# AlejandroSilvestri/os1

Hardware: AMD Instinct MI355X
Metric: frames/sec extract+match, 1920x1080 @ 2000 ORB feats (higher is better)
Workload: dtype u8

## Files before the change

include/orbfe.h:

```cpp
#ifndef ORBFE_H_
#define ORBFE_H_

#include <stddef.h>
#include <stdint.h>

#ifdef __cplusplus
extern "C" {
#endif

#define ORBFE_OK 0
#define ORBFE_ERR_INVALID (-1)
#define ORBFE_ERR_NO_DEVICE (-2)
#define ORBFE_ERR_HIP (-3)
#define ORBFE_ERR_TOO_SMALL (-4)
#define ORBFE_ERR_OVERFLOW (-5)

typedef struct OrbfeKeyPoint {
  float x, y;
  float size;
  float angle;
  float response;
  int32_t octave;
  int32_t class_id;
} OrbfeKeyPoint;

typedef struct orbfe_extractor orbfe_extractor;
typedef struct orbfe_matcher orbfe_matcher;
typedef struct orbfe_vocabulary orbfe_vocabulary;

const char* orbfe_last_error(void);
int orbfe_device_count(void);

int orbfe_device_malloc(int device_id, size_t bytes, void** out);
int orbfe_device_free(int device_id, void* ptr);
int orbfe_device_upload(int device_id, void* dst_device, const void* src_host, size_t bytes);
int orbfe_device_synchronize(int device_id);
int orbfe_host_alloc(size_t bytes, void** out);
int orbfe_host_free(void* ptr);
int orbfe_host_register(void* ptr, size_t bytes);
int orbfe_host_unregister(void* ptr);
int orbfe_device_numa_node(int device_id);
int orbfe_bind_thread_to_device(int device_id);
int orbfe_debug_h2d_rate(int device_id, const void* host, size_t bytes, int reps, double* gb_per_s);


int orbfe_extractor_create(int nfeatures, float scaleFactor, int nlevels, int iniThFAST, int minThFAST,
                           int device_id, orbfe_extractor** out);
void orbfe_extractor_destroy(orbfe_extractor* h);

int orbfe_extractor_levels(const orbfe_extractor* h);
int orbfe_extractor_device(const orbfe_extractor* h);
float orbfe_extractor_scale_factor(const orbfe_extractor* h);
int orbfe_extractor_scale_tables(const orbfe_extractor* h, float* scale, float* inv_scale, float* sigma2,
                                 float* inv_sigma2);
int orbfe_extractor_features_per_level(const orbfe_extractor* h, int32_t* out);
int orbfe_extractor_max_keypoints(const orbfe_extractor* h);
int orbfe_extractor_max_keypoints_for_size(const orbfe_extractor* h, int rows, int cols);

int orbfe_extractor_set_wait_mode(orbfe_extractor* h, int poll_us);

enum { ORBFE_INPUT_GRAY8 = 0, ORBFE_INPUT_RGB8 = 1, ORBFE_INPUT_BGR8 = 2, ORBFE_INPUT_RGBA8 = 3, ORBFE_INPUT_BGRA8 = 4 };
enum { ORBFE_GRAY_Q15 = 0, ORBFE_GRAY_Q14 = 1 };
int orbfe_extractor_set_input_format(orbfe_extractor* h, int format, int gray_variant);

enum { ORBFE_GAUSS_ED = 0, ORBFE_GAUSS_ROUNDED = 1 };
int orbfe_extractor_set_blur_variant(orbfe_extractor* h, int variant);

int orbfe_extract(orbfe_extractor* h, const uint8_t* gray, int rows, int cols, size_t stride_bytes,
                  OrbfeKeyPoint* kps, uint8_t* desc, int cap, int* n_out);

int orbfe_extract_batch(orbfe_extractor* h, int nframes, const uint8_t* const* gray, int in_device_memory,
                        int rows, int cols, size_t stride_bytes, OrbfeKeyPoint* kps, uint8_t* desc, int cap,
                        int* n_out);

int orbfe_extract_batch_submit(orbfe_extractor* h, int nframes, const uint8_t* const* gray, int in_device_memory,
                               int rows, int cols, size_t stride_bytes);
int orbfe_extract_batch_collect(orbfe_extractor* h, OrbfeKeyPoint* kps, uint8_t* desc, int cap, int* n_out);
int orbfe_extract_batch_wait(orbfe_extractor* h);

typedef struct orbfe_sfi_chain orbfe_sfi_chain;
int orbfe_sfi_chain_create(const orbfe_extractor* h, orbfe_sfi_chain** out);
void orbfe_sfi_chain_destroy(orbfe_sfi_chain* c);
int orbfe_sfi_chain_set_isolated(orbfe_sfi_chain* c, int isolated);
int orbfe_sfi_chain_restart(orbfe_sfi_chain* c);
int orbfe_extract_batch_submit_matched(orbfe_extractor* h, orbfe_sfi_chain* chain, int nframes, const uint8_t* const* gray,
                                       int in_device_memory, int rows, int cols, size_t stride_bytes, const float bounds[4],
                                       int window_size, float nnratio, int check_orientation);
int orbfe_extract_batch_collect_matched(orbfe_extractor* h, OrbfeKeyPoint* kps, uint8_t* desc, int cap, int* n_out,
                                        int32_t* matches12, int* nmatches);

int orbfe_debug_level_size(const orbfe_extractor* h, int level, int* w, int* hgt);
int orbfe_debug_level_copy(orbfe_extractor* h, int frame, int level, uint8_t* out );
int orbfe_debug_candidates(orbfe_extractor* h, int frame, int level, int32_t* xys, int cap, int* n_out);
int orbfe_debug_stage_ms(const orbfe_extractor* h, float out[5]);
int orbfe_debug_kernel_ms(orbfe_extractor* h, double out_ms[5], long long* batches, long long* frames, int reset);
int orbfe_debug_set_profiling(orbfe_extractor* h, int enable);
int orbfe_debug_fast_stamps(orbfe_extractor* h, unsigned long long out[8], int reset);
int orbfe_debug_sfi_records(orbfe_extractor* h, int32_t* out, int cap_records, int* n_out, int reset);
int orbfe_debug_sincos(orbfe_extractor* h, const float* angle_deg, int n, float* cos_out, float* sin_out);

int orbfe_debug_quadtree(const int16_t* x, const int16_t* y, const uint8_t* score, int n, int min_x, int max_x,
                         int min_y, int max_y, int n_target, int32_t* out_idx, int cap, int* n_out);
int orbfe_debug_sincos_host_check(uint32_t lo_bits, uint32_t hi_bits, uint32_t step, long long* mismatches);
int orbfe_debug_logf(orbfe_matcher* m, const float* x, int n, float* out);
int orbfe_debug_logf_host_check(uint32_t lo_bits, uint32_t hi_bits, uint32_t step, long long* mismatches);

typedef struct orbfe_stream orbfe_stream;
int orbfe_stream_create(int nfeatures, float scaleFactor, int nlevels, int iniThFAST, int minThFAST, int device_id,
                        int batch, int depth, orbfe_stream** out);
void orbfe_stream_destroy(orbfe_stream* s);
int orbfe_stream_set_matching(orbfe_stream* s, const float bounds[4], int window_size, float nnratio,
                              int check_orientation);
int orbfe_stream_set_isolated_batches(orbfe_stream* s, int isolated);
int orbfe_stream_batches_in_flight(const orbfe_stream* s);
int orbfe_stream_pop_hold(orbfe_stream* s, const OrbfeKeyPoint** kps, const uint8_t** desc, const int** n_kps, const int32_t** matches12,
                          const int** nmatches, int* ticket);
int orbfe_stream_release(orbfe_stream* s, int ticket);
int orbfe_stream_set_input_format(orbfe_stream* s, int format, int gray_variant);
int orbfe_stream_set_blur_variant(orbfe_stream* s, int variant);
int orbfe_stream_set_vocabulary(orbfe_stream* s, orbfe_vocabulary* v, int levelsup);
int orbfe_stream_bow_raw(orbfe_stream* s, int frame, const uint32_t** leaf_node, const uint32_t** level_node, int* n);
int orbfe_stream_capacity(const orbfe_stream* s);
int orbfe_stream_set_queue_slots(orbfe_stream* s, int nslots);
int orbfe_stream_queue_slots(const orbfe_stream* s);
int orbfe_stream_push(orbfe_stream* s, const uint8_t* const* gray, int in_device_memory, int rows, int cols,
                      size_t stride_bytes);
int orbfe_stream_pop(orbfe_stream* s, const OrbfeKeyPoint** kps, const uint8_t** desc, const int** n_kps,
                     const int32_t** matches12, const int** nmatches);
int orbfe_stream_stats(orbfe_stream* s, double out[4], int reset);
int orbfe_stream_kernel_ms(orbfe_stream* s, double out_ms[5], long long* batches, long long* frames, int reset);


int orbfe_hamming(const uint8_t a[32], const uint8_t b[32]);

int orbfe_matcher_create(int device_id, orbfe_matcher** out);
void orbfe_matcher_destroy(orbfe_matcher* m);
int orbfe_matcher_device(const orbfe_matcher* m);
int orbfe_matcher_upload_async(orbfe_matcher* m, void* dst_device, const void* src_host, size_t bytes);
int orbfe_matcher_synchronize(orbfe_matcher* m);

int orbfe_search_for_initialization(orbfe_matcher* m, const OrbfeKeyPoint* kps1, const uint8_t* desc1, int n1,
                                    const OrbfeKeyPoint* kps2, const uint8_t* desc2, int n2,
                                    const float bounds[4], float* prev_xy, int32_t* matches12, int window_size,
                                    float nnratio, int check_orientation, int* nmatches);

int orbfe_search_for_initialization_batch(orbfe_matcher* m, int npairs, const OrbfeKeyPoint* const* kps1,
                                          const uint8_t* const* desc1, const int* n1,
                                          const OrbfeKeyPoint* const* kps2, const uint8_t* const* desc2,
                                          const int* n2, const float bounds[4], float* const* prev_xy,
                                          int32_t* const* matches12, int window_size, float nnratio,
                                          int check_orientation, int* nmatches);

#define ORBFE_MP_IN_VIEW 1u
#define ORBFE_MP_BAD 2u
#define ORBFE_MP_CANDIDATO 4u
#define ORBFE_MP_OBSERVED 8u

int orbfe_search_by_projection(orbfe_matcher* m, const OrbfeKeyPoint* kps_un, const uint8_t* desc, int n,
                               const float bounds[4], const float* scale_factors, int nlevels,
                               const uint8_t* kp_occupied, const float* mp_proj_xy, const int32_t* mp_level,
                               const float* mp_viewcos, const uint8_t* mp_flags, const uint8_t* mp_desc, int n_mp,
                               float th, float nnratio, int32_t* kp_assigned, int* nmatches);

int orbfe_search_by_projection_uv(orbfe_matcher* m, const OrbfeKeyPoint* kps_un, const uint8_t* desc, int n,
                                  const float bounds[4], const float* scale_factors, int nlevels,
                                  const uint8_t* kp_occupied, const float* src_uv, const int32_t* src_level,
                                  const float* src_angle, const uint8_t* src_flags, const uint8_t* src_valid,
                                  const uint8_t* src_desc, int n_src, float th, int max_dist,
                                  int skip_any_occupied, int check_orientation, int32_t* kp_assigned,
                                  int* nmatches);

int orbfe_debug_matcher_ms(const orbfe_matcher* m, double out[3]);

int orbfe_window_candidates(orbfe_matcher* m, const OrbfeKeyPoint* kps_un, const uint8_t* desc, int n,
                            const float bounds[4], int nq, const float* qx, const float* qy, const float* qr,
                            const int32_t* qmin_level, const int32_t* qmax_level, const uint8_t* qdesc,
                            uint32_t* counts, uint32_t* offsets, uint32_t* pool, size_t pool_cap, size_t* pool_used);

int orbfe_search_projected(orbfe_matcher* m, const OrbfeKeyPoint* kps_un, const uint8_t* desc, int n, const float bounds[4],
                           int n_src, const float* src_uv, const float* src_radius, const int32_t* src_level,
                           const uint8_t* src_valid, const uint8_t* src_desc, const uint8_t* kp_skip, int claim,
                           const float* inv_level_sigma2, int nlevels, double chi2, int max_dist, int32_t* best_idx,
                           int32_t* best_dist, int* nmatches);

typedef struct orbfe_frame orbfe_frame;
int orbfe_frame_create(orbfe_matcher* m, const OrbfeKeyPoint* kps_un, const uint8_t* desc, int n, const float bounds[4],
                       orbfe_frame** out);
int orbfe_frame_create_from_extract(orbfe_extractor* h, int frame_index, const float bounds[4], const float* xy_un,
                                    orbfe_frame** out);
void orbfe_frame_destroy(orbfe_frame* f);
int orbfe_frame_size(const orbfe_frame* f);
int orbfe_frame_device(const orbfe_frame* f);
unsigned long long orbfe_resident_epoch(void);
unsigned long long orbfe_resident_invalidate(void);
const uint8_t* orbfe_frame_descriptors_device(orbfe_frame* f);
int orbfe_frame_download(orbfe_frame* f, OrbfeKeyPoint* kps_un, uint8_t* desc, int32_t* grid_order, int32_t* cell_start);

int orbfe_search_by_projection_frame(orbfe_matcher* m, orbfe_frame* f, const float* scale_factors, int nlevels,
                                     const uint8_t* kp_occupied, const float* mp_proj_xy, const int32_t* mp_level,
                                     const float* mp_viewcos, const uint8_t* mp_flags, const uint8_t* mp_desc, int n_mp,
                                     float th, float nnratio, int32_t* kp_assigned, int* nmatches);
int orbfe_search_by_projection_frame_rows(orbfe_matcher* m, orbfe_frame* f, const float* scale_factors, int nlevels,
                                          const uint8_t* kp_occupied, const float* mp_proj_xy, const int32_t* mp_level,
                                          const float* mp_viewcos, const uint8_t* mp_flags, const uint8_t* desc_table_device,
                                          const uint8_t* desc_table_host, const int32_t* mp_desc_row, int n_rows, int n_mp,
                                          float th, float nnratio, int32_t* kp_assigned, int* nmatches);
int orbfe_search_by_projection_uv_frame(orbfe_matcher* m, orbfe_frame* f, const float* scale_factors, int nlevels,
                                        const uint8_t* kp_occupied, const float* src_uv, const int32_t* src_level,
                                        const float* src_angle, const uint8_t* src_flags, const uint8_t* src_valid,
                                        const uint8_t* src_desc, int n_src, float th, int max_dist, int skip_any_occupied,
                                        int check_orientation, int32_t* kp_assigned, int* nmatches);
int orbfe_search_projected_frame(orbfe_matcher* m, orbfe_frame* f, int n_src, const float* src_uv, const float* src_radius,
                                 const int32_t* src_level, const uint8_t* src_valid, const uint8_t* src_desc,
                                 const uint8_t* kp_skip, int claim, const float* inv_level_sigma2, int nlevels, double chi2,
                                 int max_dist, int32_t* best_idx, int32_t* best_dist, int* nmatches);
typedef struct orbfe_local_map orbfe_local_map;
#define ORBFE_MP_SKIP 16u
typedef struct OrbfeCamera {
  float Rcw[9];
  float tcw[3];
  float Ow[3];
  float fx, fy, cx, cy;
  float logScaleFactor;
} OrbfeCamera;
int orbfe_local_map_create(orbfe_matcher* m, int capacity, orbfe_local_map** out);
void orbfe_local_map_destroy(orbfe_local_map* map);
int orbfe_local_map_capacity(const orbfe_local_map* map);
int orbfe_local_map_set_rows(orbfe_local_map* map, int n, const int32_t* rows, const float* pos, const float* normal,
                             const float* min_raw, const float* max_raw, const uint8_t* desc);
int orbfe_project_local_map(orbfe_matcher* m, orbfe_frame* f, orbfe_local_map* map, const OrbfeCamera* cam,
                            float view_cos_limit, const int32_t* rows, const uint8_t* flags, int n_mp, uint8_t* in_view,
                            float* proj_xy, int32_t* level, float* view_cos, int* n_in_view);
int orbfe_search_local_points_frame(orbfe_matcher* m, orbfe_frame* f, orbfe_local_map* map, const OrbfeCamera* cam,
                                    float view_cos_limit, const int32_t* rows, const uint8_t* flags, int n_mp,
                                    const float* scale_factors, int nlevels, const uint8_t* kp_occupied, float th, float nnratio,
                                    uint8_t* in_view, float* proj_xy, int32_t* level, float* view_cos, int32_t* kp_assigned,
                                    int* nmatches, int* n_in_view);
#define ORBFE_SRC_LAST_FRAME 0
#define ORBFE_SRC_KEYFRAME 1
int orbfe_project_sources(orbfe_matcher* m, orbfe_frame* cur_frame, orbfe_frame* src_frame, orbfe_local_map* map,
                          const OrbfeCamera* cam, int mode, const int32_t* rows, const uint8_t* flags, int n_src, uint8_t* valid,
                          float* uv, int32_t* level, int* n_valid);
int orbfe_search_by_projection_sources_frame(orbfe_matcher* m, orbfe_frame* cur_frame, orbfe_frame* src_frame,
// ... 82 lines not shown
```

os1_amd/api.py:

```python
import ctypes as C
import os
import subprocess

import numpy as np

_HERE = os.path.dirname(os.path.abspath(__file__))
_SO = os.environ.get('ORBFE_LIB') or os.path.join(_HERE, 'liborbfe.so')

KP_DTYPE = np.dtype([('x', 'f4'), ('y', 'f4'), ('size', 'f4'), ('angle', 'f4'), ('response', 'f4'),
                     ('octave', 'i4'), ('class_id', 'i4')])

MP_IN_VIEW, MP_BAD, MP_CANDIDATO, MP_OBSERVED = 1, 2, 4, 8


class OrbfeError(RuntimeError):
    def __init__(self, code, msg):
        super().__init__('orbfe error %d: %s' % (code, msg))
        self.code = code


def lib_path():
    return _SO


def build_library(force=False):
    args = ['make', '-s', '-C', os.path.join(_HERE, 'csrc')]
    if force:
        subprocess.check_call(args + ['clean'])
    subprocess.check_call(args)
    return _SO


_lib = None


def load_library():
    global _lib
    if _lib is not None:
        return _lib
    if not os.path.exists(_SO):
        raise OrbfeError(-2, 'liborbfe.so is not built (run __graft_entry__.build() or make -C os1_amd/csrc)')
    L = C.CDLL(_SO)
    vp, ci, cf = C.c_void_p, C.c_int, C.c_float
    L.orbfe_last_error.restype = C.c_char_p
    L.orbfe_device_count.restype = ci
    L.orbfe_extractor_create.argtypes = [ci, cf, ci, ci, ci, ci, C.POINTER(vp)]
    L.orbfe_extractor_destroy.argtypes = [vp]
    L.orbfe_extractor_destroy.restype = None
    L.orbfe_extractor_levels.argtypes = [vp]
    L.orbfe_extractor_scale_factor.argtypes = [vp]
    L.orbfe_extractor_scale_factor.restype = cf
    L.orbfe_extractor_scale_tables.argtypes = [vp, vp, vp, vp, vp]
    L.orbfe_extractor_features_per_level.argtypes = [vp, vp]
    L.orbfe_extractor_max_keypoints.argtypes = [vp]
    L.orbfe_extract.argtypes = [vp, vp, ci, ci, C.c_size_t, vp, vp, ci, C.POINTER(ci)]
    L.orbfe_extract_batch.argtypes = [vp, ci, vp, ci, ci, ci, C.c_size_t, vp, vp, ci, vp]
    L.orbfe_extract_batch_submit.argtypes = [vp, ci, vp, ci, ci, ci, C.c_size_t]
    L.orbfe_extract_batch_wait.argtypes = [vp]
    L.orbfe_extract_batch_collect.argtypes = [vp, vp, vp, ci, vp]
    L.orbfe_debug_level_size.argtypes = [vp, ci, C.POINTER(ci), C.POINTER(ci)]
    L.orbfe_debug_level_copy.argtypes = [vp, ci, ci, vp]
    L.orbfe_debug_candidates.argtypes = [vp, ci, ci, vp, ci, C.POINTER(ci)]
    L.orbfe_debug_stage_ms.argtypes = [vp, vp]
    L.orbfe_debug_sincos.argtypes = [vp, vp, ci, vp, vp]
    L.orbfe_hamming.argtypes = [vp, vp]
    L.orbfe_matcher_create.argtypes = [ci, C.POINTER(vp)]
    L.orbfe_matcher_destroy.argtypes = [vp]
    L.orbfe_matcher_destroy.restype = None
    L.orbfe_search_for_initialization.argtypes = [vp, vp, vp, ci, vp, vp, ci, vp, vp, vp, ci, cf, ci, C.POINTER(ci)]
    L.orbfe_search_for_initialization_batch.argtypes = [vp, ci, vp, vp, vp, vp, vp, vp, vp, vp, vp, ci, cf, ci, vp]
    L.orbfe_frame_create.argtypes = [vp, vp, vp, ci, vp, C.POINTER(vp)]
    L.orbfe_frame_create_from_extract.argtypes = [vp, ci, vp, vp, C.POINTER(vp)]
    L.orbfe_frame_destroy.argtypes = [vp]
    L.orbfe_frame_destroy.restype = None
    L.orbfe_frame_size.argtypes = [vp]
    L.orbfe_frame_descriptors_device.argtypes = [vp]
    L.orbfe_frame_descriptors_device.restype = vp
    L.orbfe_frame_download.argtypes = [vp, vp, vp, vp, vp]
    L.orbfe_search_by_projection_frame.argtypes = [vp, vp, vp, ci, vp, vp, vp, vp, vp, vp, ci, cf, cf, vp, C.POINTER(ci)]
    L.orbfe_search_by_projection_frame_rows.argtypes = [vp, vp, vp, ci, vp, vp, vp, vp, vp, vp, vp, vp, ci, ci, cf, cf, vp,
                                                        C.POINTER(ci)]
    L.orbfe_matcher_upload_async.argtypes = [vp, vp, vp, C.c_size_t]
    L.orbfe_matcher_synchronize.argtypes = [vp]
    L.orbfe_matcher_device.argtypes = [vp]
    L.orbfe_extractor_device.argtypes = [vp]
    L.orbfe_frame_device.argtypes = [vp]
    L.orbfe_resident_epoch.restype = C.c_ulonglong
    L.orbfe_resident_invalidate.restype = C.c_ulonglong
    L.orbfe_search_by_projection_uv_frame.argtypes = [vp, vp, vp, ci, vp, vp, vp, vp, vp, vp, vp, ci, cf, ci, ci, ci, vp,
                                                      C.POINTER(ci)]
    L.orbfe_search_projected_frame.argtypes = [vp, vp, ci, vp, vp, vp, vp, vp, vp, ci, vp, ci, C.c_double, ci, vp, vp,
                                               C.POINTER(ci)]
    L.orbfe_debug_resolve_rounds.argtypes = [vp]
    L.orbfe_debug_resolve_route.argtypes = [vp]
    L.orbfe_debug_resolve_phases.argtypes = [vp, vp]
    L.orbfe_search_by_projection.argtypes = [vp, vp, vp, ci, vp, vp, ci, vp, vp, vp, vp, vp, vp, ci, cf, cf, vp,
                                             C.POINTER(ci)]
    L.orbfe_search_by_projection_uv.argtypes = [vp, vp, vp, ci, vp, vp, ci, vp, vp, vp, vp, vp, vp, vp, ci, cf, ci,
                                                ci, ci, vp, C.POINTER(ci)]
    L.orbfe_distinctive_descriptors.argtypes = [vp, ci, vp, vp, vp]
    L.orbfe_window_candidates.argtypes = [vp, vp, vp, ci, vp, ci, vp, vp, vp, vp, vp, vp, vp, vp, vp, C.c_size_t,
                                          C.POINTER(C.c_size_t)]
    L.orbfe_undistort_equidistant.argtypes = [vp, ci, cf, cf, cf, cf]
    L.orbfe_undistort_pinhole.argtypes = [vp, ci, cf, cf, cf, cf, vp, ci]
    L.orbfe_compute_image_bounds.argtypes = [ci, ci, ci, cf, cf, cf, cf, vp, ci, vp]
    L.orbfe_search_projected.argtypes = [vp, vp, vp, ci, vp, ci, vp, vp, vp, vp, vp, vp, ci, vp, ci, C.c_double, ci, vp, vp,
                                         C.POINTER(ci)]
    L.orbfe_search_for_triangulation.argtypes = [vp, vp, vp, vp, ci, vp, vp, vp, ci, vp, vp, vp, ci, vp, vp, vp, ci, vp, cf, cf,
                                                 vp, vp, ci, ci, vp, C.POINTER(ci)]
    L.orbfe_extractor_max_keypoints_for_size.argtypes = [vp, ci, ci]
    L.orbfe_extractor_set_vocabulary.argtypes = [vp, vp, ci]
    L.orbfe_extract_bow_raw.argtypes = [vp, ci, vp, vp, ci, C.POINTER(ci)]
    L.orbfe_bow_assemble.argtypes = [vp, vp, vp, ci, vp, vp, C.POINTER(ci), vp, vp, vp, C.POINTER(ci), vp]
    L.orbfe_stream_set_vocabulary.argtypes = [vp, vp, ci]
    L.orbfe_stream_bow_raw.argtypes = [vp, ci, C.POINTER(vp), C.POINTER(vp), C.POINTER(ci)]
    L.orbfe_extract_bow.argtypes = [vp, ci, vp, vp, C.POINTER(ci), vp, vp, vp, C.POINTER(ci), vp, vp]
    L.orbfe_extractor_set_input_format.argtypes = [vp, ci, ci]
    L.orbfe_stream_set_input_format.argtypes = [vp, ci, ci]
    L.orbfe_extractor_set_blur_variant.argtypes = [vp, ci]
    L.orbfe_stream_set_blur_variant.argtypes = [vp, ci]
    L.orbfe_vocabulary_create.argtypes = [ci, ci, ci, ci, ci, vp, ci, C.POINTER(vp)]
    L.orbfe_vocabulary_create_from_image.argtypes = [ci, vp, C.c_size_t, C.POINTER(vp)]
    L.orbfe_vocabulary_destroy.argtypes = [vp]
    L.orbfe_vocabulary_destroy.restype = None
    L.orbfe_vocabulary_info.argtypes = [vp] + [C.POINTER(ci)] * 6
    L.orbfe_bow_transform.argtypes = [vp, vp, ci, ci, ci, vp, vp, C.POINTER(ci), vp, vp, vp, C.POINTER(ci), vp, vp]
    L.orbfe_search_by_bow.argtypes = [vp, vp, vp, vp, ci, vp, vp, vp, ci, vp, vp, vp, ci, vp, vp, vp, ci, cf, ci, ci, vp,
                                      C.POINTER(ci)]
    L.orbfe_search_by_bow_batch.argtypes = [vp, ci, vp, vp, vp, vp, vp, vp, vp, vp, vp, vp, vp, ci, vp, vp, vp, ci, cf, ci, ci, vp, vp]
    L.orbfe_debug_matcher_ms.argtypes = [vp, vp]
    L.orbfe_debug_features_in_area.argtypes = [vp, vp, ci, vp, cf, cf, cf, ci, ci, vp, ci, C.POINTER(ci)]
    L.orbfe_debug_kernel_ms.argtypes = [vp, vp, C.POINTER(C.c_longlong), C.POINTER(C.c_longlong), ci]
    L.orbfe_debug_set_profiling.argtypes = [vp, ci]
    L.orbfe_device_malloc.argtypes = [ci, C.c_size_t, C.POINTER(vp)]
    L.orbfe_device_free.argtypes = [ci, vp]
    L.orbfe_device_upload.argtypes = [ci, vp, vp, C.c_size_t]
    L.orbfe_host_alloc.argtypes = [C.c_size_t, C.POINTER(vp)]
    L.orbfe_host_free.argtypes = [vp]
    L.orbfe_host_register.argtypes = [vp, C.c_size_t]
    L.orbfe_host_unregister.argtypes = [vp]
    L.orbfe_device_synchronize.argtypes = [ci]
    L.orbfe_device_numa_node.argtypes = [ci]
    L.orbfe_bind_thread_to_device.argtypes = [ci]
    L.orbfe_debug_h2d_rate.argtypes = [ci, vp, C.c_size_t, ci, C.POINTER(C.c_double)]
    L.orbfe_stream_create.argtypes = [ci, cf, ci, ci, ci, ci, ci, ci, C.POINTER(vp)]
    L.orbfe_stream_destroy.argtypes = [vp]
    L.orbfe_stream_destroy.restype = None
    L.orbfe_stream_set_matching.argtypes = [vp, vp, ci, cf, ci]
    L.orbfe_stream_capacity.argtypes = [vp]
    L.orbfe_stream_set_queue_slots.argtypes = [vp, ci]
    L.orbfe_stream_queue_slots.argtypes = [vp]
    L.orbfe_stream_push.argtypes = [vp, vp, ci, ci, ci, C.c_size_t]
    L.orbfe_stream_pop.argtypes = [vp, C.POINTER(vp), C.POINTER(vp), C.POINTER(vp), C.POINTER(vp), C.POINTER(vp)]
    L.orbfe_stream_pop_hold.argtypes = [vp, C.POINTER(vp), C.POINTER(vp), C.POINTER(vp), C.POINTER(vp), C.POINTER(vp), C.POINTER(ci)]
    L.orbfe_stream_release.argtypes = [vp, ci]
    L.orbfe_stream_set_isolated_batches.argtypes = [vp, ci]
    L.orbfe_stream_batches_in_flight.argtypes = [vp]
    L.orbfe_stream_multi_create.argtypes = [ci, cf, ci, ci, ci, C.POINTER(ci), ci, ci, ci, C.POINTER(vp)]
    L.orbfe_stream_multi_destroy.argtypes = [vp]
    L.orbfe_stream_multi_destroy.restype = None
    L.orbfe_stream_multi_devices.argtypes = [vp]
    L.orbfe_stream_multi_capacity.argtypes = [vp]
    L.orbfe_stream_multi_device_of_next_push.argtypes = [vp]
    L.orbfe_stream_multi_set_matching.argtypes = [vp, vp, ci, cf, ci]
    L.orbfe_stream_multi_set_blur_variant.argtypes = [vp, ci]
    L.orbfe_stream_multi_push.argtypes = [vp, vp, ci, ci, ci, C.c_size_t]
    L.orbfe_stream_multi_pop.argtypes = [vp, C.POINTER(vp), C.POINTER(vp), C.POINTER(vp), C.POINTER(vp), C.POINTER(vp)]
    L.orbfe_stream_stats.argtypes = [vp, vp, ci]
    L.orbfe_stream_kernel_ms.argtypes = [vp, vp, C.POINTER(C.c_longlong), C.POINTER(C.c_longlong), ci]
    L.orbfe_debug_quadtree.argtypes = [vp, vp, vp, ci, ci, ci, ci, ci, ci, vp, ci, C.POINTER(ci)]
    L.orbfe_debug_sincos_host_check.argtypes = [C.c_uint32, C.c_uint32, C.c_uint32, C.POINTER(C.c_longlong)]
    L.orbfe_debug_logf.argtypes = [vp, vp, ci, vp]
    L.orbfe_debug_logf_host_check.argtypes = [C.c_uint32, C.c_uint32, C.c_uint32, C.POINTER(C.c_longlong)]
    L.orbfe_local_map_create.argtypes = [vp, ci, C.POINTER(vp)]
    L.orbfe_local_map_destroy.argtypes = [vp]
    L.orbfe_local_map_destroy.restype = None
    L.orbfe_local_map_capacity.argtypes = [vp]
    L.orbfe_local_map_set_rows.argtypes = [vp, ci, vp, vp, vp, vp, vp, vp]
    L.orbfe_project_local_map.argtypes = [vp, vp, vp, vp, cf, vp, vp, ci, vp, vp, vp, vp, C.POINTER(ci)]
    L.orbfe_search_local_points_frame.argtypes = [vp, vp, vp, vp, cf, vp, vp, ci, vp, ci, vp, cf, cf, vp, vp, vp, vp, vp,
                                                  C.POINTER(ci), C.POINTER(ci)]
    L.orbfe_project_sources.argtypes = [vp, vp, vp, vp, vp, ci, vp, vp, ci, vp, vp, vp, C.POINTER(ci)]
    L.orbfe_search_by_projection_sources_frame.argtypes = [vp, vp, vp, vp, vp, ci, vp, vp, ci, vp, ci, vp, cf, ci, ci, vp, vp, vp,
                                                           vp, C.POINTER(ci), C.POINTER(ci)]
    _lib = L
    return L


def _p(a):
    return a.ctypes.data_as(C.c_void_p)


class DeviceRows:

    def __init__(self, ptr, n):
        self.ptr, self.n = int(ptr), int(n)

    def __len__(self):
        return self.n


def _rows(a):
    if isinstance(a, DeviceRows):
        return C.c_void_p(a.ptr), a
    a = np.ascontiguousarray(a, np.uint8)
    return _p(a), a


def _check(rc):
    if rc != 0:
        raise OrbfeError(rc, load_library().orbfe_last_error().decode('utf-8', 'replace'))


def device_count():
    return load_library().orbfe_device_count()


def hamming(a, b):
    a = np.ascontiguousarray(a, np.uint8)
    b = np.ascontiguousarray(b, np.uint8)
    return load_library().orbfe_hamming(_p(a), _p(b))


class Extractor:

    def __init__(self, nfeatures=1000, scale=1.2, nlevels=8, ini_th=20, min_th=7, device=0):
        self.L = load_library()
        h = C.c_void_p()
        _check(self.L.orbfe_extractor_create(nfeatures, scale, nlevels, ini_th, min_th, device, C.byref(h)))
        self.h = h
        self.nlevels = nlevels
        self.cap = self.L.orbfe_extractor_max_keypoints(h)

    def close(self):
        if getattr(self, 'h', None):
            self.L.orbfe_extractor_destroy(self.h)
            self.h = None

    def __del__(self):
        try:
            self.close()
        except Exception:
            pass

    def tables(self):
        n = self.nlevels
        sf, isf, s2, is2 = (np.zeros(n, np.float32) for _ in range(4))
        nf = np.zeros(n, np.int32)
        _check(self.L.orbfe_extractor_scale_tables(self.h, _p(sf), _p(isf), _p(s2), _p(is2)))
        _check(self.L.orbfe_extractor_features_per_level(self.h, _p(nf)))
        return dict(sf=sf, isf=isf, s2=s2, is2=is2, nfeat=nf)

    def __call__(self, image):
        image = np.asarray(image)
        if image.size == 0:
            n = C.c_int(0)
            _check(self.L.orbfe_extract(self.h, None, 0, 0, 0, None, None, 0, C.byref(n)))
            return np.zeros(0, KP_DTYPE), np.zeros((0, 32), np.uint8)
        assert image.dtype == np.uint8 and image.ndim == 2 and image.strides[1] == 1
        cap = max(self.cap, self.L.orbfe_extractor_max_keypoints_for_size(self.h, image.shape[0], image.shape[1]))
        kps = np.zeros(cap, KP_DTYPE)
        desc = np.zeros((cap, 32), np.uint8)
        n = C.c_int(0)
        _check(self.L.orbfe_extract(self.h, _p(image), image.shape[0], image.shape[1], image.strides[0], _p(kps),
                                    _p(desc), cap, C.byref(n)))
        return kps[:n.value].copy(), desc[:n.value].copy()

    FORMATS = {'gray': 0, 'rgb': 1, 'bgr': 2, 'rgba': 3, 'bgra': 4}

    def set_blur_variant(self, variant):
        _check(self.L.orbfe_extractor_set_blur_variant(self.h, int(variant)))

    def set_input_format(self, fmt='gray', variant=0):
        _check(self.L.orbfe_extractor_set_input_format(self.h, self.FORMATS[fmt], variant))

    def extract_color(self, image):
        image = np.ascontiguousarray(image, np.uint8)
        kps = np.zeros(self.cap, KP_DTYPE)
        desc = np.zeros((self.cap, 32), np.uint8)
        n = C.c_int(0)
        _check(self.L.orbfe_extract(self.h, _p(image), image.shape[0], image.shape[1], image.strides[0], _p(kps),
                                    _p(desc), self.cap, C.byref(n)))
        return kps[:n.value].copy(), desc[:n.value].copy()

    def set_vocabulary(self, voc, levelsup=4):
        self._voc = voc
        _check(self.L.orbfe_extractor_set_vocabulary(self.h, voc.h if voc is not None else None, levelsup))

    def bow(self, frame, n):
        ids = np.zeros(max(n, 1), np.uint32)
        vals = np.zeros(max(n, 1), np.float64)
        fvn = np.zeros(max(n, 1), np.uint32)
        fvo = np.zeros(n + 1, np.uint32)
        fvf = np.zeros(max(n, 1), np.uint32)
        wof = np.zeros(max(n, 1), np.uint32)
        nof = np.zeros(max(n, 1), np.uint32)
        nw, nn = C.c_int(0), C.c_int(0)
        _check(self.L.orbfe_extract_bow(self.h, frame, _p(ids), _p(vals), C.byref(nw), _p(fvn), _p(fvo), _p(fvf), C.byref(nn),
                                        _p(wof), _p(nof)))
        nw, nn = nw.value, nn.value
        return ids[:nw], vals[:nw], (fvn[:nn], fvo[:nn + 1], fvf[:int(fvo[nn])]), wof[:n], nof[:n]

    def extract_batch_ptrs(self, ptrs, rows, cols, stride, on_device, kps=None, desc=None):
        B = len(ptrs)
        arr = (C.c_void_p * B)(*ptrs)
        if kps is None:
            kps = np.zeros((B, self.cap), KP_DTYPE)
        if desc is None:
            desc = np.zeros((B, self.cap, 32), np.uint8)
        n = np.zeros(B, np.int32)
        _check(self.L.orbfe_extract_batch(self.h, B, arr, int(on_device), rows, cols, stride, _p(kps), _p(desc),
                                          int(kps.shape[1]), _p(n)))
        return kps, desc, n

    def submit_ptrs(self, ptrs, rows, cols, stride, on_device):
        B = len(ptrs)
        self._pending = (C.c_void_p * B)(*ptrs)
        self._pendingB = B
        _check(self.L.orbfe_extract_batch_submit(self.h, B, self._pending, int(on_device), rows, cols, stride))

    def wait(self):
        _check(self.L.orbfe_extract_batch_wait(self.h))

    def collect(self, kps=None, desc=None):
        B = self._pendingB
        if kps is None:
            kps = np.zeros((B, self.cap), KP_DTYPE)
        if desc is None:
            desc = np.zeros((B, self.cap, 32), np.uint8)
        n = np.zeros(B, np.int32)
        _check(self.L.orbfe_extract_batch_collect(self.h, _p(kps), _p(desc), self.cap, _p(n)))
        return kps, desc, n

    def extract_batch(self, images):
        images = [np.ascontiguousarray(im, np.uint8) for im in images]
        rows, cols = images[0].shape
        assert all(im.shape == (rows, cols) for im in images)
        kps, desc, n = self.extract_batch_ptrs([im.ctypes.data for im in images], rows, cols, cols, False)
        return [(kps[i, :n[i]].copy(), desc[i, :n[i]].copy()) for i in range(len(images))]

    def level(self, level, frame=0):
        w, h = C.c_int(), C.c_int()
        _check(self.L.orbfe_debug_level_size(self.h, level, C.byref(w), C.byref(h)))
        out = np.zeros((h.value, w.value), np.uint8)
        _check(self.L.orbfe_debug_level_copy(self.h, frame, level, _p(out)))
        return out

    def candidates(self, level, frame=0):
        n = C.c_int(0)
        _check(self.L.orbfe_debug_candidates(self.h, frame, level, None, 0, C.byref(n)))
        out = np.zeros((max(n.value, 1), 3), np.int32)
        _check(self.L.orbfe_debug_candidates(self.h, frame, level, _p(out), n.value, C.byref(n)))
        return out[:n.value].copy()

    def stage_ms(self):
        out = np.zeros(5, np.float32)
        _check(self.L.orbfe_debug_stage_ms(self.h, _p(out)))
        return out

    def kernel_ms(self, reset=False):
        ms = np.zeros(5, np.float64)
        b, f = C.c_longlong(0), C.c_longlong(0)
        _check(self.L.orbfe_debug_kernel_ms(self.h, _p(ms), C.byref(b), C.byref(f), int(reset)))
        return ms, b.value, f.value

    def set_profiling(self, enable=True):
        _check(self.L.orbfe_debug_set_profiling(self.h, int(enable)))

    def sincos(self, angle_deg):
        a = np.ascontiguousarray(angle_deg, np.float32)
        c = np.zeros_like(a)
        s = np.zeros_like(a)
        _check(self.L.orbfe_debug_sincos(self.h, _p(a), a.size, _p(c), _p(s)))
        return c, s


class Camera(C.Structure):
    _fields_ = [('Rcw', C.c_float * 9), ('tcw', C.c_float * 3), ('Ow', C.c_float * 3), ('fx', C.c_float), ('fy', C.c_float),
                ('cx', C.c_float), ('cy', C.c_float), ('logScaleFactor', C.c_float)]

    @classmethod
    def make(cls, Rcw, tcw, Ow, fx, fy, cx, cy, log_scale_factor):
        c = cls()
        c.Rcw[:] = [float(v) for v in np.asarray(Rcw, np.float32).ravel()]
        c.tcw[:] = [float(v) for v in np.asarray(tcw, np.float32).ravel()]
        c.Ow[:] = [float(v) for v in np.asarray(Ow, np.float32).ravel()]
        c.fx, c.fy, c.cx, c.cy = float(np.float32(fx)), float(np.float32(fy)), float(np.float32(cx)), float(np.float32(cy))
        c.logScaleFactor = float(np.float32(log_scale_factor))
        return c


MP_IN_VIEW, MP_BAD, MP_CANDIDATO, MP_OBSERVED, MP_SKIP = 1, 2, 4, 8, 16
SRC_LAST_FRAME, SRC_KEYFRAME = 0, 1


class LocalMap:

    def __init__(self, matcher, capacity):
        self.L = load_library()
        self.matcher = matcher
        h = C.c_void_p()
        _check(self.L.orbfe_local_map_create(matcher.h, capacity, C.byref(h)))
        self.h = h
        self.capacity = capacity

    def set_rows(self, rows, pos=None, normal=None, min_raw=None, max_raw=None, desc=None):
        rows = np.ascontiguousarray(rows, np.int32)
        keep = []

        def arg(a, dt, shape):
            if a is None:
                return None
            a = np.ascontiguousarray(a, dt).reshape(shape)
            keep.append(a)
            return _p(a)
        n = len(rows)
        _check(self.L.orbfe_local_map_set_rows(self.h, n, _p(rows), arg(pos, np.float32, (n, 3)), arg(normal, np.float32, (n, 3)),
                                               arg(min_raw, np.float32, (n,)), arg(max_raw, np.float32, (n,)),
                                               arg(desc, np.uint8, (n, 32))))

    def close(self):
        if getattr(self, 'h', None):
            self.L.orbfe_local_map_destroy(self.h)
            self.h = None

    def __del__(self):
        try:
            self.close()
        except Exception:
            pass


class Frame:

    def __init__(self, handle, n):
        self.L = load_library()
        self.h = handle
        self.n = n

    @classmethod
    def from_host(cls, matcher, kps_un, desc, bounds):
        L = load_library()
        kps_un = np.ascontiguousarray(kps_un, KP_DTYPE)
        desc = np.ascontiguousarray(desc, np.uint8)
        b = np.asarray(bounds, np.float32)
        h = C.c_void_p()
        _check(L.orbfe_frame_create(matcher.h, _p(kps_un), _p(desc), len(kps_un), _p(b), C.byref(h)))
        return cls(h, len(kps_un))

    @classmethod
    def from_extract(cls, extractor, frame_index, bounds, xy_un=None):
        L = load_library()
        b = np.asarray(bounds, np.float32)
        xy = None if xy_un is None else np.ascontiguousarray(xy_un, np.float32)
        h = C.c_void_p()
        _check(L.orbfe_frame_create_from_extract(extractor.h, frame_index, _p(b), None if xy is None else _p(xy), C.byref(h)))
        return cls(h, L.orbfe_frame_size(h))

    def __len__(self):
        return self.n

    def descriptors_device(self):
        return DeviceRows(self.L.orbfe_frame_descriptors_device(self.h) or 0, self.n)

    def download(self):
        k = np.zeros(max(self.n, 1), KP_DTYPE)
        d = np.zeros((max(self.n, 1), 32), np.uint8)
        order = np.zeros(max(self.n, 1), np.int32)
        cs = np.zeros(64 * 48 + 1, np.int32)
        _check(self.L.orbfe_frame_download(self.h, _p(k), _p(d), _p(order), _p(cs)))
        return k[:self.n], d[:self.n], order[:int(cs[-1])], cs

    def close(self):
        if getattr(self, 'h', None):
            self.L.orbfe_frame_destroy(self.h)
            self.h = None

    def __del__(self):
        try:
            self.close()
        except Exception:
            pass


class Matcher:

    def frame(self, kps_un, desc, bounds):
        return Frame.from_host(self, kps_un, desc, bounds)

    def resolve_rounds(self):
        return int(self.L.orbfe_debug_resolve_rounds(self.h))

    def resolve_route(self):
        return int(self.L.orbfe_debug_resolve_route(self.h))

    def resolve_phases(self):
        o = np.zeros(4, np.int32)
        _check(self.L.orbfe_debug_resolve_phases(self.h, _p(o)))
        return np.diff(o.astype(np.int64)) & 0xffffffff
# ... 743 lines not shown
```

os1_amd/csrc/orbfe_extractor.hip:

```cpp
#include <hip/hip_runtime.h>
#include <unistd.h>
#include <sched.h>

#include <algorithm>
#include <cctype>
#include <chrono>
#include <cmath>
#include <cstdarg>
#include <cstdio>
#include <cstdlib>
#include <cstring>
#include <memory>
#include <mutex>
#include <string>
#include <thread>
#include <vector>

#include "../../include/orbfe.h"
#include "glibc_sincosf.h"
#include "host_pool.h"
#include "orbfe_internal.h"
#include "quadtree.h"

namespace orbfe {
int launch_pyramid(const PyramidParams& P, int nframes, hipStream_t st, const ConeParams* cone);
void launch_ingest(const uint8_t* src, long long sstride, uint8_t* dst, long long dpitch, int rowBytes, int rows, hipStream_t st);
void launch_to_gray(const uint8_t* const* raw, long long rawStride, const uint8_t* const* gray, long long grayPitch, int rows,
                    int cols, int channels, const int coef[3], int shift, bool aligned, int nframes, hipStream_t st);
void launch_fast(const PyramidParams& P, int nframes, hipStream_t st);
uint32_t fast_cell_geo(int wCell, int hCell);
void launch_compact(const PyramidParams& P, int nframes, hipStream_t st);
void launch_compact_local(const PyramidParams& P, int nframes, hipStream_t st, int level0, int level1);
void launch_describe(const PyramidParams& P, const SelKp* sel, int nsel, float* angle, uint8_t* desc,
                     hipStream_t st);
void launch_sincos(const float* deg, int n, float* c, float* s, hipStream_t st);
void launch_spin(unsigned long long ticks, hipStream_t st);
void launch_describe_slots(const PyramidParams& P, const SelKp* sel, int nslots, float* angle, uint8_t* desc,
                           const uint32_t* selCount, int selPerFrame, const int* selOff, hipStream_t st, bool fourWaves, float* angle2 = nullptr,
                           uint8_t* desc2 = nullptr);
int launch_quadtree(const QtParams& Q, int nframes, hipStream_t st, int ldsBudget);
int bow_launch_descend(orbfe_vocabulary* v, const uint8_t* d_desc, int n, int levelsup, uint2* d_out, hipStream_t st);
int bow_assemble(orbfe_vocabulary* v, const uint2* ln, int n, uint32_t* bow_ids, double* bow_values, int* n_words,
                 uint32_t* fv_nodes, uint32_t* fv_offsets, uint32_t* fv_features, int* n_fv_nodes,
                 uint32_t* word_of_feature, uint32_t* node_of_feature);
int bow_device(const orbfe_vocabulary* v);
void launch_sfi(const SfiParams& S, int nframes, hipStream_t st);
void launch_sfi_carry(const SfiParams& S, int lastFrame, SelKp* cSel, float* cAngle, uint8_t* cDesc, uint32_t* cCount,
                      hipStream_t st);

thread_local std::string g_err;
void set_err(const char* fmt, ...) {
  char buf[512];
  va_list ap;
  va_start(ap, fmt);
  vsnprintf(buf, sizeof buf, fmt, ap);
  va_end(ap);
  g_err = buf;
}
}

using namespace orbfe;

#define HIP_TRY(expr)                                                                        \
  do {                                                                                       \
    hipError_t e_ = (expr);                                                                  \
    if (e_ != hipSuccess) {                                                                  \
      set_err("%s failed: %s (%s:%d)", #expr, hipGetErrorString(e_), __FILE__, __LINE__);    \
      return ORBFE_ERR_HIP;                                                                  \
    }                                                                                        \
  } while (0)

namespace {
inline int cv_round_f(float v) { return (int)lrintf(v); }
inline int cv_floor_f(float v) { int i = (int)v; return i - (i > v); }
inline short sat_short(int v) { return (short)(v < -32768 ? -32768 : v > 32767 ? 32767 : v); }
inline long long align_up(long long v, long long a) { return (v + a - 1) / a * a; }
double now_ms() {
  return std::chrono::duration<double, std::milli>(std::chrono::steady_clock::now().time_since_epoch()).count();
}

template <class T>
struct DevBuf {
  T* p = nullptr;
  size_t n = 0;
  int ensure(size_t count) {
    if (count <= n) return ORBFE_OK;
    if (p) (void)hipFree(p);
    p = nullptr;
    n = 0;
    HIP_TRY(hipMalloc((void**)&p, count * sizeof(T)));
    n = count;
    return ORBFE_OK;
  }
  void release() { if (p) (void)hipFree(p); p = nullptr; n = 0; }
};
template <class T>
struct PinBuf {
  T* p = nullptr;
  size_t n = 0;
  int ensure(size_t count) {
    if (count <= n) return ORBFE_OK;
    if (p) (void)hipHostFree(p);
    p = nullptr;
    n = 0;
    HIP_TRY(hipHostMalloc((void**)&p, count * sizeof(T), hipHostMallocDefault));
    n = count;
    return ORBFE_OK;
  }
  void release() { if (p) (void)hipHostFree(p); p = nullptr; n = 0; }
};
}

struct orbfe_sfi_chain {
  int device = 0, n0cap = 0;
  DevBuf<SelKp> sel[2];
  DevBuf<float> angle[2];
  DevBuf<uint8_t> desc[2];
  DevBuf<uint32_t> count;
  hipEvent_t ready[2] = {};
  long long seq = 0;
  bool isolated = false;
  bool restart = false;
  orbfe_matcher* hostMatcher = nullptr;
  std::vector<OrbfeKeyPoint> hostPrevKps;
  std::vector<uint8_t> hostPrevDesc;
  bool hostPrevValid = false;
  ~orbfe_sfi_chain() {
    (void)hipSetDevice(device);
    if (hostMatcher) orbfe_matcher_destroy(hostMatcher);
    for (int i = 0; i < 2; i++) { sel[i].release(); angle[i].release(); desc[i].release(); if (ready[i]) (void)hipEventDestroy(ready[i]); }
    count.release();
  }
};

struct UploadLane {
  std::mutex mu;
  hipStream_t stream = nullptr;
};
static UploadLane* upload_lane(int device) {
  static std::mutex mu;
  static UploadLane* lanes[64] = {};
  if (device < 0 || device >= 64) return nullptr;
  std::lock_guard<std::mutex> lk(mu);
  if (!lanes[device]) {
    UploadLane* l = new UploadLane;
    if (hipStreamCreateWithFlags(&l->stream, hipStreamNonBlocking) != hipSuccess) { delete l; return nullptr; }
    lanes[device] = l;
  }
  return lanes[device];
}

struct orbfe_extractor {
  int nfeatures, nlevels, iniTh, minTh, device;
  double scaleFactor;
  std::vector<float> sf, isf, sigma2, isigma2;
  std::vector<int> nfeat;
  static constexpr int kMaxSub = 4;
  hipStream_t stream = nullptr;
  hipStream_t streams[kMaxSub] = {};
  static constexpr int subBatches = 4;
  hipEvent_t evUpload = nullptr;
  bool lastLocalCand = false, submitLocalCand = false;
  bool localLists = true;
  hipEvent_t evFrame0 = nullptr, evS1[kMaxSub] = {};
  int subSel[kMaxSub] = {};
  size_t candHostCap = 0;
  bool gpuQuadtree = true;
  orbfe_vocabulary* voc = nullptr;
  int vocLevelsup = 4;
  bool pendingBow = false;
  DevBuf<uint2> d_bow;
  PinBuf<uint2> h_bow;
  std::vector<std::vector<uint2>> bowKp;
  int kpPerFrameCap = 0;
  bool geomGpuQtOk = true;
  QtParams QP{};
  int selOff[kMaxLevels + 1] = {};
  int selPerFrame = 0;
  DevBuf<uint16_t> d_own;
  hipEvent_t evQt[2] = {};
  std::vector<int> frameKpBase, frameKpCount;

  int rows = 0, cols = 0, batchCap = 0;
  PyramidParams P{};
  DevBuf<uint8_t> d_tables, d_slab, d_in;
  DevBuf<ConeRange> d_coneTab, d_coneTailTab;
  ConeParams coneTail{};
  bool tailOk = false;
  int tailBase = 0, tailTile = 48;
  ConeParams cone{};
  bool coneOk = false;
  bool qtJump = true;
  int qtLdsBudget = 120 * 1024;
  int pollWaitUs = 0;
  bool zeroCopyOut = true;
  bool zeroCopyBatches = false;
  bool ingestKernel = true;
  int coneTile = 0;
  int coneMaxFrames = 2;
  DevBuf<FastCell> d_cells;
  DevBuf<uint8_t> d_zeros;
  DevBuf<uint32_t> d_cellCount, d_slots, d_cand;
  DevBuf<const uint8_t*> d_frame0;
  template <class T> struct View { T* p = nullptr; };
  DevBuf<uint8_t> d_outArena;
  PinBuf<uint8_t> h_outArena;
  size_t outArenaBytes = 0;
  View<uint32_t> d_levelStart, d_selCount, h_levelStart, h_selCount;
  View<SelKp> d_sel, h_sel;
  View<float> d_angle, h_angle;
  View<uint8_t> d_desc, h_desc;
  View<int32_t> d_m12, h_m12, d_nm, h_nm;
  DevBuf<uint16_t> d_sfiOrder;
  DevBuf<int> d_sfiOrderCount;
  DevBuf<uint32_t> d_sfiPool, d_sfiPcount;
  bool pendingMatched = false;
  DevBuf<float> d_f32tmp;
  bool profileKernels = false;
  PinBuf<const uint8_t*> h_frame0;
  PinBuf<uint32_t> h_cand;
  long long inPitch = 0;
  int inFormat = ORBFE_INPUT_GRAY8, grayVariant = ORBFE_GRAY_Q15;
  int gaussVariant = ORBFE_GAUSS_ED;
  long long grayPitch = 0;
  DevBuf<uint8_t> d_gray;
  bool inLinear = false;
  int lastFrames = 0;
  int deferredFrames = 0, deferredCap = 0;
  bool deferredMatched = false;
  std::vector<OrbfeKeyPoint> defKps;
  std::vector<uint8_t> defDesc;
  std::vector<int> defN, defNm;
  std::vector<int32_t> defM12;
  bool lastGpuQt = false, lastZeroCopy = false, submitZeroCopy = false;
  bool describe4 = true;
  float stageMs[5] = {0, 0, 0, 0, 0};
  hipEvent_t ev[kMaxSub][6] = {};
  double kernMs[5] = {0, 0, 0, 0, 0};
  long long kernBatches = 0, kernFrames = 0;

  struct Meta { int16_t x, y; uint8_t score, level; };
  struct Worker {
    QuadTree qt;
    std::vector<int16_t> qx, qy;
    std::vector<uint8_t> qs;
    std::vector<int> qsel;
  };
  std::unique_ptr<HostPool> pool;
  int hostThreads = 1;
  std::vector<Worker> workers;
  std::vector<std::vector<Meta>> taskOut;
  std::vector<Meta> meta;

  ~orbfe_extractor() {
    (void)hipSetDevice(device);
    for (auto& st : streams) if (st) (void)hipStreamSynchronize(st);
    d_bow.release(); h_bow.release();
    d_tables.release(); d_coneTab.release(); d_coneTailTab.release(); d_slab.release(); d_in.release(); d_cellCount.release();
    d_sfiOrder.release(); d_sfiOrderCount.release(); d_sfiPool.release(); d_sfiPcount.release();
    d_cells.release(); d_zeros.release(); d_slots.release(); d_cand.release(); d_frame0.release(); d_gray.release(); d_outArena.release(); h_outArena.release();
    d_f32tmp.release();
    h_frame0.release(); h_cand.release();
    for (auto& es : ev) for (auto& e : es) if (e) (void)hipEventDestroy(e);
    for (auto& e : evS1) if (e) (void)hipEventDestroy(e);
    for (auto& e : evQt) if (e) (void)hipEventDestroy(e);
    d_own.release();
    if (evFrame0) (void)hipEventDestroy(evFrame0);
    if (evUpload) (void)hipEventDestroy(evUpload);

    for (auto& st : streams) if (st) (void)hipStreamDestroy(st);
  }

  int setGeometry(int r, int c) {
    if (r == rows && c == cols) return ORBFE_OK;
    if (c > 4095 || r > 4095) {
      set_err("image %dx%d exceeds the 4095-pixel coordinate packing limit", c, r);
      return ORBFE_ERR_INVALID;
    }
    bool qtOk = true;
    int kpSum = 8;
    PyramidParams Q{};
    Q.nlevels = nlevels;
    Q.iniTh = iniTh;
    Q.minTh = minTh;
    long long off = 0, slot = 0;
    int cellBase = 0;
    size_t tableBytes = 0;
    for (int l = 0; l < nlevels; l++) {
      LevelGeom& L = Q.lv[l];
      L.w = cv_round_f((float)c * isf[l]);
      L.h = cv_round_f((float)r * isf[l]);
      const float width = (float)((L.w - kEdge + 3) - (kEdge - 3));
      const float height = (float)((L.h - kEdge + 3) - (kEdge - 3));
      L.nCols = (int)(width / 30.f);
      L.nRows = (int)(height / 30.f);
      if (L.nCols < 1 || L.nRows < 1) {
        set_err("image %dx%d too small: level %d (%dx%d) has no FAST cell", c, r, l, L.w, L.h);
        return ORBFE_ERR_TOO_SMALL;
      }
      L.wCell = (int)std::ceil(width / L.nCols);
      L.hCell = (int)std::ceil(height / L.nRows);
      {
        const int nIni = (int)roundf(static_cast<float>(L.w - 2 * kBorder) / (L.h - 2 * kBorder));
        if (nIni < 1 || nIni > 4) qtOk = false;
        kpSum += std::max(nfeat[l] + 4, 4 * std::max(nIni, 4));
      }
      L.cellBase = cellBase;
      cellBase += L.nCols * L.nRows;
      L.slotCap = (((L.wCell + 1) / 2) * ((L.hCell + 1) / 2) + 3) & ~3;
      L.slotBase = slot;
      slot += (long long)L.nCols * L.nRows * L.slotCap;
      if (l >= 1) {
        L.pitch = (int)align_up(L.w, 64);
        L.off = off;
        off += align_up((long long)L.pitch * L.h, 256);
        tableBytes += align_up(L.w * 4, 16) + align_up(L.w * 4, 16) + align_up(L.h * 4, 16) + align_up(L.h * 4, 16) + align_up(L.h * 4, 16);
      }
    }
    Q.ncells = cellBase;
    Q.slabBytes = off;
    Q.slotsPerFrame = slot;
    Q.candCap = slot;
    if (slot >= (1ll << 24)) qtOk = false;

    std::vector<uint8_t> tab(tableBytes);
    int rc = d_tables.ensure(tableBytes);
    if (rc) return rc;
    size_t cur = 0;
    const int* xofsH[kMaxLevels] = {};
    const int* yofsH[kMaxLevels] = {};
    for (int l = 1; l < nlevels; l++) {
      LevelGeom& L = Q.lv[l];
      const int sw = Q.lv[l - 1].w, sh = Q.lv[l - 1].h, dw = L.w, dh = L.h;
      const double scale_x = 1. / ((double)dw / sw), scale_y = 1. / ((double)dh / sh);
      int* xofs = (int*)(tab.data() + cur);
      xofsH[l] = xofs;
      L.xofs = (const int*)(d_tables.p + cur);
      cur += align_up(dw * 4, 16);
      short* xa = (short*)(tab.data() + cur);
      L.xalpha = (const short*)(d_tables.p + cur);
      cur += align_up(dw * 4, 16);
      int* yofs = (int*)(tab.data() + cur);
      yofsH[l] = yofs;
      L.yofs = (const int*)(d_tables.p + cur);
      cur += align_up(dh * 4, 16);
      short* yb = (short*)(tab.data() + cur);
      L.ybeta = (const short*)(d_tables.p + cur);
      cur += align_up(dh * 4, 16);
      unsigned* yc = (unsigned*)(tab.data() + cur);
      L.yofc = (const unsigned*)(d_tables.p + cur);
      cur += align_up(dh * 4, 16);
      for (int dx = 0; dx < dw; dx++) {
        float fx = (float)((dx + 0.5) * scale_x - 0.5);
        int sx = cv_floor_f(fx);
        fx -= sx;
        if (sx < 0) { fx = 0; sx = 0; }
        if (sx >= sw - 1) { fx = 0; sx = sw - 1; }
        xofs[dx] = sx;
        xa[2 * dx] = sat_short(cv_round_f((1.f - fx) * 2048));
        xa[2 * dx + 1] = sat_short(cv_round_f(fx * 2048));
      }
      for (int dy = 0; dy < dh; dy++) {
        float fy = (float)((dy + 0.5) * scale_y - 0.5);
        int sy = cv_floor_f(fy);
        fy -= sy;
        yofs[dy] = sy;
        yc[dy] = (unsigned)std::min(std::max(sy, 0), sh - 1) | ((unsigned)std::min(std::max(sy + 1, 0), sh - 1) << 16);
        yb[2 * dy] = sat_short(cv_round_f((1.f - fy) * 2048));
        yb[2 * dy + 1] = sat_short(cv_round_f(fy * 2048));
      }
      for (int dy = dh; dy < (int)align_up(dh, 4); dy++) {
        yc[dy] = yc[dh - 1];
        yb[2 * dy] = yb[2 * (dh - 1)];
        yb[2 * dy + 1] = yb[2 * (dh - 1) + 1];
      }
      int maxW = 1, maxH = 1;
      for (int x0 = 0; x0 < dw; x0 += 64) {
        const int x1 = std::min(x0 + 64, dw) - 1;
        maxW = std::max(maxW, std::min(xofs[x1] + 1, sw - 1) - xofs[x0] + 1);
      }
      for (int y0 = 0; y0 < dh; y0 += 64) {
        const int y1 = std::min(y0 + 64, dh) - 1;
        const int r0 = std::min(std::max(yofs[y0], 0), sh - 1), r1 = std::min(std::max(yofs[y1] + 1, 0), sh - 1);
        maxH = std::max(maxH, r1 - r0 + 1);
      }
      L.rzPitch = (maxW + 3 + 3) & ~3;
      L.rzRows = maxH;
    }
    HIP_TRY(hipMemcpyAsync(d_tables.p, tab.data(), tableBytes, hipMemcpyHostToDevice, stream));
    auto buildCone = [&](int tile, int baseMin, ConeParams& out, DevBuf<ConeRange>& tabBuf, bool& ok) -> int {
      ok = false;
      if (!(nlevels >= 3 && scaleFactor <= 1.5f)) return ORBFE_OK;
      std::vector<ConeRange> coneTab;
      const int top = nlevels - 1;
      if (tile <= 0) {
        tile = 32;
        for (int t = 16; t < 32; t += 2)
          if (((Q.lv[top].w + t - 1) / t) * ((Q.lv[top].h + t - 1) / t) <= 256) { tile = t; break; }
      }
      const int tx = (Q.lv[top].w + tile - 1) / tile, ty = (Q.lv[top].h + tile - 1) / tile;
      coneTab.assign((size_t)(tx + ty) * kMaxLevels, ConeRange{0, 0});
      int maxW[kMaxLevels] = {}, maxH[kMaxLevels] = {};
      for (int b = 0; b < tx + ty; b++) {
        const bool isX = b < tx;
        int lo = (isX ? b : b - tx) * tile, hi = std::min(lo + tile, isX ? Q.lv[top].w : Q.lv[top].h) - 1;
        ConeRange* R = coneTab.data() + (size_t)b * kMaxLevels;
        for (int l = top;; l--) {
          R[l] = ConeRange{lo, hi};
          int& m = isX ? maxW[l] : maxH[l];
          m = std::max(m, hi - lo + 1);
          if (l == 0) break;
          const int dn = isX ? Q.lv[l].w : Q.lv[l].h, sn = isX ? Q.lv[l - 1].w : Q.lv[l - 1].h;
          const int* ofs = isX ? xofsH[l] : yofsH[l];
          const int nlo = lo == 0 ? 0 : std::min(std::max(ofs[lo], 0), sn - 1);
          const int nhi = hi == dn - 1 ? sn - 1 : std::min(std::max(ofs[hi] + 1, 0), sn - 1);
          lo = nlo; hi = nhi;
        }
      }
      for (int base = std::max(0, baseMin); base < top - 1; base++) {
        auto pitchOf = [&](int l) { return (maxW[l] + 3 + 3) & ~3; };
        auto area = [&](int l) { return (size_t)align_up(pitchOf(l) * maxH[l], 16); };
        size_t hBytes = 0;
        int coefLen = 0;
        for (int l = base + 1; l <= top; l++) {
          hBytes = std::max(hBytes, (size_t)align_up(maxH[l - 1] * pitchOf(l) * 2, 16));
          coefLen = std::max(coefLen, std::max(pitchOf(l), maxH[l]));
        }
        const size_t coefBytes = (size_t)kMaxLevels * 2 * coefLen * sizeof(int2);
        const size_t total = area(base) + area(base + 1) + hBytes + coefBytes;
        if (total > 128 * 1024 || coefLen > 512) continue;
        out.base = base; out.top = top; out.tile = tile; out.tilesX = tx; out.tilesY = ty;
        out.offB = (int)area(base); out.offH = out.offB + (int)area(base + 1); out.offC = out.offH + (int)hBytes;
        out.coefLen = coefLen; out.ldsBytes = (int)total;
        ok = true;
        break;
      }
      if (ok) {
        int rc2;
        if ((rc2 = tabBuf.ensure(coneTab.size()))) return rc2;
        HIP_TRY(hipMemcpyAsync(tabBuf.p, coneTab.data(), sizeof(ConeRange) * coneTab.size(), hipMemcpyHostToDevice, stream));
        HIP_TRY(hipStreamSynchronize(stream));
        out.regX = tabBuf.p;
        out.regY = tabBuf.p + (size_t)tx * kMaxLevels;
      }
      return ORBFE_OK;
    };
    if ((rc = buildCone(coneTile, 0, cone, d_coneTab, coneOk))) return rc;
    tailOk = false;
    if (tailBase > 0 && tailBase < nlevels - 2)
      if ((rc = buildCone(tailTile, tailBase, coneTail, d_coneTailTab, tailOk))) return rc;
    if (tailOk && coneTail.base != tailBase) tailOk = false;
    std::vector<FastCell> cells(Q.ncells);
    Q.fastLean = 1;
    for (int l = 0; l < nlevels; l++) {
      const LevelGeom& L = Q.lv[l];
      const uint32_t geo = fast_cell_geo(L.wCell, L.hCell);
      if (geo == 0u && L.nRows * L.nCols > 0) Q.fastLean = 0;
      for (int i = 0; i < L.nRows; i++)
        for (int j = 0; j < L.nCols; j++) {
          const int ex0 = kEdge + j * L.wCell, ey0 = kEdge + i * L.hCell;
          const int ew = std::min(std::min(L.wCell, L.w - kEdge - ex0), 127), eh = std::min(std::min(L.hCell, L.h - kEdge - ey0), 127);
          const bool valid = ew > 0 && eh > 0;
          FastCell c{};
          c.ex0 = (uint16_t)ex0; c.ey0 = (uint16_t)ey0; c.level = (uint8_t)l;
          c.ew = valid ? (uint8_t)ew : 0;
          c.eh = valid ? (uint8_t)eh : 0;
          c.cell = (uint32_t)(L.cellBase + i * L.nCols + j);
          c.slotOff = (uint32_t)(L.slotBase + (long long)(i * L.nCols + j) * L.slotCap);
          c.roiOff = l == 0 ? 0u : (uint32_t)(L.off + (long long)(ey0 - 3) * L.pitch + (ex0 - 3));
          c.pitch = l == 0 ? 0u : (uint32_t)L.pitch;
          c.wCell = (uint8_t)L.wCell; c.hCell = (uint8_t)L.hCell;
          c.geo = geo;
          cells[c.cell] = c;
        }
    }
    if ((rc = d_cells.ensure(cells.size()))) return rc;
    if (!d_zeros.p) {
      if ((rc = d_zeros.ensure(256))) return rc;
      HIP_TRY(hipMemsetAsync(d_zeros.p, 0, 256, stream));
    }
    Q.zeros = d_zeros.p;
    HIP_TRY(hipMemcpyAsync(d_cells.p, cells.data(), sizeof(FastCell) * cells.size(), hipMemcpyHostToDevice, stream));
    HIP_TRY(hipStreamSynchronize(stream));
    Q.cells = d_cells.p;
    P = Q;
    rows = r;
    geomGpuQtOk = qtOk;
    const int kpCap = std::max(kpSum, selPerFrame);
    if (kpCap > kpPerFrameCap) {
      kpPerFrameCap = kpCap;
      batchCap = 0;
    }
    cols = c;
    batchCap = 0;
    return ORBFE_OK;
  }

  int ensureSubStreams(int nsub) {
    for (int s = 1; s < nsub; s++)
      if (!streams[s]) HIP_TRY(hipStreamCreateWithFlags(&streams[s], hipStreamNonBlocking));
    return ORBFE_OK;
  }

  int inChannels() const { return inFormat == ORBFE_INPUT_GRAY8 ? 1 : (inFormat == ORBFE_INPUT_RGB8 || inFormat == ORBFE_INPUT_BGR8) ? 3 : 4; }

  int setBatch(int nframes, bool hostInput, size_t hostStride = 0) {
    int rc;
    if (nframes > batchCap) {
      if ((rc = d_slab.ensure((size_t)P.slabBytes * nframes + 64))) return rc;
      if ((rc = d_cellCount.ensure((size_t)P.ncells * nframes))) return rc;
      if ((rc = d_slots.ensure((size_t)P.slotsPerFrame * nframes))) return rc;
      if ((rc = d_cand.ensure((size_t)P.candCap * nframes))) return rc;
      if ((rc = d_frame0.ensure(2 * (size_t)nframes))) return rc;
      if ((rc = h_frame0.ensure(2 * (size_t)nframes))) return rc;
      const size_t maxKp = (size_t)kpPerFrameCap * nframes;
      {
        auto al256 = [](size_t v) { return (v + 255) & ~(size_t)255; };
        const size_t oLs = 0, oSc = oLs + al256(sizeof(uint32_t) * (kMaxLevels + 1) * nframes),
                     oSel = oSc + al256(sizeof(uint32_t) * kMaxLevels * nframes), oAng = oSel + al256(sizeof(SelKp) * maxKp),
                     oDesc = oAng + al256(sizeof(float) * maxKp), oM12 = oDesc + al256(32 * maxKp),
                     oNm = oM12 + al256(sizeof(int32_t) * (size_t)(selOff[1] - selOff[0]) * nframes), total = oNm + al256(sizeof(int32_t) * nframes);
        if ((rc = d_outArena.ensure(total))) return rc;
        if ((rc = h_outArena.ensure(total))) return rc;
        outArenaBytes = total;
        uint8_t *D = d_outArena.p, *Hh = h_outArena.p;
        d_levelStart.p = (uint32_t*)(D + oLs); h_levelStart.p = (uint32_t*)(Hh + oLs);
        d_selCount.p = (uint32_t*)(D + oSc); h_selCount.p = (uint32_t*)(Hh + oSc);
        d_sel.p = (SelKp*)(D + oSel); h_sel.p = (SelKp*)(Hh + oSel);
        d_angle.p = (float*)(D + oAng); h_angle.p = (float*)(Hh + oAng);
        d_desc.p = D + oDesc; h_desc.p = Hh + oDesc;
        d_m12.p = (int32_t*)(D + oM12); h_m12.p = (int32_t*)(Hh + oM12);
        d_nm.p = (int32_t*)(D + oNm); h_nm.p = (int32_t*)(Hh + oNm);
      }
      if (gpuQuadtree) {
        if ((rc = d_own.ensure((size_t)P.candCap * nframes))) return rc;
      }
      batchCap = nframes;
      if (candHostCap == 0) candHostCap = 96 * 1024;
      if ((rc = h_cand.ensure(candHostCap * (size_t)batchCap))) return rc;
    }
    if (inChannels() > 1) {
      grayPitch = align_up(cols, 256);
// ... 29 lines not shown
      const uint8_t* lo = gray[f0];
      for (int f = f0 + 1; f < f0 + nf; f++) lo = std::min(lo, gray[f]);
      uint64_t seen = 0;
      bool tile = true;
      for (int f = f0; f < f0 + nf && tile; f++) {
        const size_t d = (size_t)(gray[f] - lo);
        const size_t k = d / frameBytes;
        tile = d % frameBytes == 0 && k < (size_t)nf && !(seen >> k & 1);
        seen |= (uint64_t)1 << k;
      }
      if (tile) {
        uint8_t* base = d_in.p + frameBytes * f0;
        HIP_TRY(hipMemcpyAsync(base, lo, frameBytes * (size_t)(nf - 1) + lastBytes, hipMemcpyHostToDevice, st));
        for (int f = f0; f < f0 + nf; f++) devAt[f] = base + (size_t)(gray[f] - lo);
        return ORBFE_OK;
      }
    }
    for (int f = f0; f < f0 + nf;) {
      int g = f + 1;
      while (g < f0 + nf && gray[g] == gray[g - 1] + frameBytes) g++;
      HIP_TRY(hipMemcpyAsync(d_in.p + frameBytes * f, gray[f], frameBytes * (size_t)(g - f - 1) + lastBytes, hipMemcpyHostToDevice, st));
      for (int k = f; k < g; k++) devAt[k] = d_in.p + frameBytes * k;
      f = g;
    }
    return ORBFE_OK;
  }

  int uploadSlots(int f0, int nf, const uint8_t* const* gray, size_t stride, int r, int c, hipStream_t st) {
    for (int f = f0; f < f0 + nf; f++) {
      if (inLinear)
        HIP_TRY(hipMemcpyAsync(d_in.p + (size_t)inPitch * rows * f, gray[f], stride * (size_t)(r - 1) + c, hipMemcpyHostToDevice, st));
      else
        HIP_TRY(hipMemcpy2DAsync(d_in.p + (size_t)inPitch * rows * f, inPitch, gray[f], stride, c, r, hipMemcpyHostToDevice, st));
    }
    return ORBFE_OK;
  }

  int runGpuQt(int nframes, const uint8_t* const* gray, bool onDevice, int r, int c, size_t stride, OrbfeKeyPoint* kps,
               uint8_t* desc, int cap, int* n_out) {
    int rc = submitGpuQt(nframes, gray, onDevice, r, c, stride);
    if (rc) return rc;
    return waitGpuQt(kps, desc, cap, n_out);
  }

  bool submitProfiled = false, fastTimed = false;
  std::vector<const uint8_t*> devAt;
  int pendingFrames = 0;
  double tSubmit0 = 0, tSubmit1 = 0;

  struct MatchSpec { orbfe_sfi_chain* chain; float bounds[4]; int window; float nnratio; int checkOri; };

  int submitGpuQt(int nframes, const uint8_t* const* gray, bool onDevice, int r, int c, size_t stride,
                  const MatchSpec* ms = nullptr) {
    if (pendingFrames) { set_err("a submitted batch has not been collected yet"); return ORBFE_ERR_INVALID; }
    HIP_TRY(hipSetDevice(device));
    int rc;
    if ((rc = setGeometry(r, c))) return rc;
    if (!geomGpuQtOk) {
      set_err("image %dx%d: a pyramid level has more than 4 (or no) quadtree root nodes; only the blocking "
              "orbfe_extract / orbfe_extract_batch calls (host quadtree path) handle such aspect ratios", c, r);
      return ORBFE_ERR_INVALID;
    }
    if ((rc = setBatch(nframes, !onDevice, stride))) return rc;
    const double t0 = now_ms();
    hipStream_t st = streams[0];
    const int ch = inChannels();
    const int rowBytes = c * ch;
    for (int f = 0; f < nframes; f++)
      if (!gray[f]) { set_err("frame %d is NULL", f); return ORBFE_ERR_INVALID; }
    devAt.resize(nframes);
    bool pinned = !onDevice;
    std::vector<const uint8_t*>& mappedAt = devAt;
    if (!onDevice) {
      const size_t extent = stride * (size_t)(r - 1) + (size_t)rowBytes;
      const int ncheck = nframes <= coneMaxFrames ? nframes : 1;
      for (int f = 0; f < ncheck && pinned; f++) {
        void* dp = nullptr;
        void* dpEnd = nullptr;
        const bool ok = hipHostGetDevicePointer(&dp, const_cast<uint8_t*>(gray[f]), 0) == hipSuccess && dp &&
                        hipHostGetDevicePointer(&dpEnd, const_cast<uint8_t*>(gray[f]) + extent - 1, 0) == hipSuccess &&
                        (const uint8_t*)dpEnd - (const uint8_t*)dp == (ptrdiff_t)(extent - 1);
        if (!ok) { (void)hipGetLastError(); pinned = false; break; }
        mappedAt[f] = static_cast<const uint8_t*>(dp);
      }
    }
    if (!onDevice && !pinned) {
      if ((rc = uploadFrames(0, nframes, gray, stride, r, rowBytes, st, devAt.data()))) return rc;
    } else if (!onDevice && ingestKernel && nframes <= coneMaxFrames &&
               ((((uintptr_t)gray[0] | (uintptr_t)gray[nframes - 1] | (uintptr_t)stride | (uintptr_t)rowBytes) & 3) == 0)) {
      for (int f = 0; f < nframes; f++) {
        uint8_t* d = d_in.p + (size_t)inPitch * rows * f;
        launch_ingest(mappedAt[f], (long long)stride, d, inPitch, rowBytes, r, st);
        devAt[f] = d;
      }
      HIP_TRY(hipGetLastError());
    } else if (!onDevice) {
      UploadLane* lane = upload_lane(device);
      if (!lane) { set_err("cannot create the upload stream"); return ORBFE_ERR_HIP; }
      std::lock_guard<std::mutex> lk(lane->mu);
      if ((rc = uploadFrames(0, nframes, gray, stride, r, rowBytes, lane->stream, devAt.data()))) return rc;
      HIP_TRY(hipEventRecord(evUpload, lane->stream));
      HIP_TRY(hipStreamWaitEvent(st, evUpload, 0));
    }
    bool rawAligned = ((onDevice ? (long long)stride : inPitch) & 3) == 0;
    for (int f = 0; f < nframes; f++) {
      const uint8_t* raw = onDevice ? gray[f] : devAt[f];
      rawAligned = rawAligned && ((uintptr_t)raw & (ch == 4 ? 15 : 3)) == 0;
      h_frame0.p[f] = ch == 1 ? raw : d_gray.p + (size_t)grayPitch * rows * f;
      h_frame0.p[nframes + f] = raw;
    }
    const long long rawStride = onDevice ? (long long)stride : inPitch;
    P.stride0 = ch == 1 ? rawStride : grayPitch;
    P.frameBase = 0;
    P.gaussVariant = gaussVariant;
    if (ch == 1 && nframes <= 2) {
      P.frame0 = nullptr;
      P.frameInline[0] = h_frame0.p[0];
      P.frameInline[1] = h_frame0.p[nframes - 1];
    } else {
      P.frame0 = d_frame0.p;
      HIP_TRY(hipMemcpyAsync(d_frame0.p, h_frame0.p, sizeof(void*) * nframes * (ch == 1 ? 1 : 2), hipMemcpyHostToDevice, st));
    }
    if (ch > 1) {
      const bool q15 = grayVariant == ORBFE_GRAY_Q15;
      const int cr = q15 ? 9798 : 4899, cg = q15 ? 19235 : 9617, cb = q15 ? 3735 : 1868;
      const bool rgb = inFormat == ORBFE_INPUT_RGB8 || inFormat == ORBFE_INPUT_RGBA8;
      const int coef[3] = {rgb ? cr : cb, cg, rgb ? cb : cr};
      launch_to_gray(d_frame0.p + nframes, rawStride, d_frame0.p, grayPitch, r, c, ch, coef, q15 ? 15 : 14, rawAligned, nframes, st);
    }
    const bool prof = profileKernels;
    QP.cand = d_cand.p; QP.levelStart = d_levelStart.p; QP.candCap = P.candCap; QP.nlevels = nlevels; QP.frameBase = 0;
    QP.own = d_own.p;
    QP.sel = d_sel.p; QP.selCount = d_selCount.p; QP.selPerFrame = selPerFrame;
    const bool small = nframes <= coneMaxFrames;
    const bool zeroCopy = zeroCopyOut && small && !voc && !(ms && ms->chain);
    submitZeroCopy = zeroCopy;
    QP.jump = qtJump ? 1 : 0;
    const bool kernelOut = zeroCopyBatches && !small;
    QP.selHost = (zeroCopy || kernelOut) ? h_sel.p : nullptr;
    QP.selCountHost = (zeroCopy || kernelOut) ? h_selCount.p : nullptr;
    for (int l = 0; l < nlevels; l++) {
      QP.levW[l] = P.lv[l].w; QP.levH[l] = P.lv[l].h; QP.nfeat[l] = nfeat[l]; QP.selOff[l] = selOff[l];
      QP.candBase[l] = P.lv[l].slotBase;
    }
    float* angOut = zeroCopy ? h_angle.p : d_angle.p;
    uint8_t* descOut = zeroCopy ? h_desc.p : d_desc.p;
    const int qtLds = small ? qtLdsBudget : 0;
    const bool four = describe4 && small;
    const bool localCand = small && localLists;
    submitLocalCand = localCand;
    QP.levelLocal = localCand ? 1 : 0;
    {
      if (prof) HIP_TRY(hipEventRecord(ev[0][0], st));
      if (launch_pyramid(P, nframes, st, coneOk && small ? &cone : (tailOk && !small ? &coneTail : nullptr))) { set_err("cannot configure the pyramid kernel"); return ORBFE_ERR_HIP; }
      const bool timeFast = prof || !small;
      fastTimed = timeFast;
      if (timeFast) HIP_TRY(hipEventRecord(ev[0][1], st));
      launch_fast(P, nframes, st);
      if (timeFast) HIP_TRY(hipEventRecord(ev[0][2], st));
      if (localCand) launch_compact_local(P, nframes, st, 0, nlevels);
      else launch_compact(P, nframes, st);
      if (prof) HIP_TRY(hipEventRecord(ev[0][3], st));
      if (prof) HIP_TRY(hipEventRecord(evQt[0], st));
      if (launch_quadtree(QP, nframes, st, qtLds)) { set_err("cannot configure the quadtree kernel"); return ORBFE_ERR_HIP; }
      if (prof) HIP_TRY(hipEventRecord(evQt[1], st));
      if (prof) HIP_TRY(hipEventRecord(ev[0][4], st));
      launch_describe_slots(P, d_sel.p, nframes * selPerFrame, angOut, descOut, d_selCount.p, selPerFrame, selOff, st, four,
                            kernelOut ? h_angle.p : nullptr, kernelOut ? h_desc.p : nullptr);
      if (prof) HIP_TRY(hipEventRecord(ev[0][5], st));
      HIP_TRY(hipGetLastError());
    }
    const int nslots = nframes * selPerFrame;
    pendingBow = false;
    if (voc) {
      if ((rc = d_bow.ensure(nslots)) || (rc = h_bow.ensure(nslots))) return rc;
      if ((rc = bow_launch_descend(voc, d_desc.p, nslots, vocLevelsup, d_bow.p, st))) return rc;
      HIP_TRY(hipMemcpyAsync(h_bow.p, d_bow.p, sizeof(uint2) * nslots, hipMemcpyDeviceToHost, st));
      pendingBow = true;
    }
    pendingMatched = false;
    if (ms && ms->chain) {
      orbfe_sfi_chain& ch = *ms->chain;
      const int n0cap = selOff[1] - selOff[0];
      if (ch.n0cap != n0cap || ch.device != device) { set_err("match chain belongs to a different extractor configuration"); return ORBFE_ERR_INVALID; }
      if ((rc = d_sfiOrder.ensure((size_t)batchCap * n0cap))) return rc;
      if ((rc = d_sfiOrderCount.ensure(batchCap))) return rc;
      if ((rc = d_sfiPool.ensure((size_t)batchCap * n0cap * n0cap))) return rc;
      if ((rc = d_sfiPcount.ensure((size_t)batchCap * n0cap))) return rc;
      SfiParams SP{};
      SP.sel = d_sel.p; SP.angle = d_angle.p; SP.desc = d_desc.p; SP.selCount = d_selCount.p;
      SP.selPerFrame = selPerFrame; SP.n0cap = n0cap; SP.frameBase = 0;
      const int prev = (int)((ch.seq + 1) & 1), cur = (int)(ch.seq & 1);
      SP.carrySel = ch.sel[prev].p; SP.carryAngle = ch.angle[prev].p; SP.carryDesc = ch.desc[prev].p;
      const bool iso = ch.isolated;
      SP.carryCount = ch.count.p + ((ch.seq == 0 || iso || ch.restart) ? 2 : prev);
      ch.restart = false;
      SP.minX = ms->bounds[0]; SP.minY = ms->bounds[2];
      SP.invW = static_cast<float>(64) / static_cast<float>(ms->bounds[1] - ms->bounds[0]);
      SP.invH = static_cast<float>(48) / static_cast<float>(ms->bounds[3] - ms->bounds[2]);
      SP.window = (float)ms->window; SP.nnratio = ms->nnratio; SP.checkOri = ms->checkOri;
      SP.order = d_sfiOrder.p; SP.orderCount = d_sfiOrderCount.p; SP.pool = d_sfiPool.p; SP.pcount = d_sfiPcount.p;
      SP.matches12 = kernelOut ? h_m12.p : d_m12.p; SP.nmatches = kernelOut ? h_nm.p : d_nm.p;
      if (ch.seq > 0 && !iso) HIP_TRY(hipStreamWaitEvent(st, ch.ready[prev], 0));
      launch_sfi(SP, nframes, st);
      HIP_TRY(hipGetLastError());
      if (!iso) {
        launch_sfi_carry(SP, nframes - 1, ch.sel[cur].p, ch.angle[cur].p, ch.desc[cur].p, ch.count.p + cur, st);
        HIP_TRY(hipGetLastError());
        HIP_TRY(hipEventRecord(ch.ready[cur], st));
      }
      ch.seq++;
      pendingMatched = true;
    }
    if (!zeroCopy && !kernelOut) HIP_TRY(hipMemcpyAsync(h_outArena.p, d_outArena.p, outArenaBytes, hipMemcpyDeviceToHost, st));
    submitProfiled = prof;
    tSubmit0 = t0;
    tSubmit1 = now_ms();
    pendingFrames = nframes;
    return ORBFE_OK;
  }

  int waitOnly() {
    if (!pendingFrames) return ORBFE_OK;
    HIP_TRY(hipSetDevice(device));
    hipStream_t st = streams[0];
    if (pollWaitUs > 0) {
      hipError_t q;
      while ((q = hipStreamQuery(st)) == hipErrorNotReady) usleep((useconds_t)pollWaitUs);
      if (q != hipSuccess) HIP_TRY(q);
    }
    HIP_TRY(hipStreamSynchronize(st));
    return ORBFE_OK;
  }

  int waitGpuQt(OrbfeKeyPoint* kps, uint8_t* desc, int cap, int* n_out, int32_t* matches12 = nullptr,
                int* nmatches = nullptr) {
    if (!pendingFrames) { set_err("no submitted batch to collect"); return ORBFE_ERR_INVALID; }
    HIP_TRY(hipSetDevice(device));
    const int nframes = pendingFrames;
    pendingFrames = 0;
    hipStream_t st = streams[0];
    const double t0 = tSubmit0, t1 = tSubmit1;
    const double t1b = now_ms();
    if (pollWaitUs > 0) {
      hipError_t q;
      while ((q = hipStreamQuery(st)) == hipErrorNotReady) usleep((useconds_t)pollWaitUs);
      if (q != hipSuccess) HIP_TRY(q);
    }
    HIP_TRY(hipStreamSynchronize(st));
    const double t2 = now_ms();
    {
      float ms = 0;
      if (fastTimed && hipEventElapsedTime(&ms, ev[0][1], ev[0][2]) == hipSuccess) kernMs[1] += ms;
      if (submitProfiled) {
        if (hipEventElapsedTime(&ms, ev[0][0], ev[0][1]) == hipSuccess) kernMs[0] += ms;
        if (hipEventElapsedTime(&ms, ev[0][2], ev[0][3]) == hipSuccess) kernMs[2] += ms;
        if (hipEventElapsedTime(&ms, ev[0][4], ev[0][5]) == hipSuccess) kernMs[3] += ms;
        if (hipEventElapsedTime(&ms, evQt[0], evQt[1]) == hipSuccess) kernMs[4] += ms;
      }
      if (fastTimed) {
        kernBatches++;
        kernFrames += nframes;
      }
    }
    int status = ORBFE_OK;
    if (pendingBow) bowKp.resize(nframes);
    else bowKp.clear();
    for (int f = 0; f < nframes; f++) {
      OrbfeKeyPoint* ko = kps + (size_t)f * cap;
      uint8_t* dout = desc + (size_t)f * cap * 32;
      if (pendingBow) bowKp[f].clear();
      int n = 0;
      for (int l = 0; l < nlevels; l++) {
        const int cnt = (int)h_selCount.p[(size_t)f * kMaxLevels + l];
        const size_t base = (size_t)f * selPerFrame + selOff[l];
        const float scale = sf[l];
        const float size = (float)(int)(31 * sf[l]);
        for (int i = 0; i < cnt; i++) {
          if (n >= cap) { n++; continue; }
          const SelKp s = h_sel.p[base + i];
          OrbfeKeyPoint kp;
          kp.x = (float)(s.xy & 0xffff);
          kp.y = (float)(s.xy >> 16);
          if (l != 0) { kp.x *= scale; kp.y *= scale; }
          kp.size = size;
          kp.angle = h_angle.p[base + i];
          kp.response = (float)(s.lf >> 24);
          kp.octave = l;
          kp.class_id = -1;
          ko[n] = kp;
          memcpy(dout + (size_t)n * 32, h_desc.p + (base + i) * 32, 32);
          if (pendingBow) bowKp[f].push_back(h_bow.p[base + i]);
          n++;
        }
      }
      n_out[f] = n;
      if (n > cap) {
        set_err("frame %d produced %d keypoints, cap is %d", f, n, cap);
        status = ORBFE_ERR_OVERFLOW;
      }
    }
    if (matches12 && nmatches) {
      const int n0cap = selOff[1] - selOff[0];
      for (int f = 0; f < nframes; f++) {
        int32_t* row = matches12 + (size_t)f * cap;
        const int m = std::min(cap, n0cap);
        if (pendingMatched) {
          memcpy(row, h_m12.p + (size_t)f * n0cap, sizeof(int32_t) * m);
          nmatches[f] = h_nm.p[f];
        } else {
          nmatches[f] = 0;
        }
        for (int i = pendingMatched ? m : 0; i < cap; i++) row[i] = -1;
      }
    }
    const double t3 = now_ms();
    stageMs[0] = (float)(t1 - t0);
    stageMs[1] = (float)(t2 - t1b);
    stageMs[2] = 0;
    stageMs[3] = (float)(t3 - t2);
    stageMs[4] = (float)(t3 - t0);
    lastFrames = nframes;
    lastGpuQt = true;
    lastZeroCopy = submitZeroCopy;
    lastLocalCand = submitLocalCand;
    return status;
  }

  int run(int nframes, const uint8_t* const* gray, bool onDevice, int r, int c, size_t stride, OrbfeKeyPoint* kps,
          uint8_t* desc, int cap, int* n_out) {
    if (pendingFrames) { set_err("a submitted batch has not been collected yet"); return ORBFE_ERR_INVALID; }
    HIP_TRY(hipSetDevice(device));
    int rc;
    if ((rc = setGeometry(r, c))) return rc;
    if ((rc = setBatch(nframes, !onDevice, stride))) return rc;
    const double t0 = now_ms();
    if (!pool) {
      pool.reset(new HostPool(hostThreads));
      workers.resize(hostThreads);
    }
    if (inChannels() != 1) { set_err("colour input needs the GPU quadtree path (unset ORBFE_HOST_QUADTREE)"); return ORBFE_ERR_INVALID; }
    const int nsub = std::min(nframes, std::min(kMaxSub, std::max(1, subBatches)));
    const int maxKp = kpPerFrameCap;
    if ((rc = ensureSubStreams(nsub))) return rc;
    int subF0[kMaxSub + 1];
    for (int s = 0; s <= nsub; s++) subF0[s] = (int)((long long)nframes * s / nsub);

    devAt.resize(nframes);
    for (int f = 0; f < nframes; f++) {
      if (!gray[f]) { set_err("frame %d is NULL", f); return ORBFE_ERR_INVALID; }
      h_frame0.p[f] = onDevice ? gray[f] : d_in.p + (size_t)inPitch * rows * f;
    }
    P.stride0 = onDevice ? (long long)stride : inPitch;
    P.gaussVariant = gaussVariant;
    P.frame0 = d_frame0.p;
    HIP_TRY(hipMemcpyAsync(d_frame0.p, h_frame0.p, sizeof(void*) * nframes, hipMemcpyHostToDevice, streams[0]));
    HIP_TRY(hipEventRecord(evFrame0, streams[0]));
    for (int s = 0; s < nsub; s++) {
      hipStream_t st = streams[s];
      const int f0 = subF0[s], nf = subF0[s + 1] - f0;
      if (s) HIP_TRY(hipStreamWaitEvent(st, evFrame0, 0));
      if (!onDevice && (rc = uploadSlots(f0, nf, gray, stride, r, c, st))) return rc;
      PyramidParams Q = P;
      Q.frameBase = f0;
      HIP_TRY(hipEventRecord(ev[s][0], st));
      if (launch_pyramid(Q, nf, st, coneOk && nf <= coneMaxFrames ? &cone : nullptr)) { set_err("cannot configure the pyramid kernel"); return ORBFE_ERR_HIP; }
      HIP_TRY(hipEventRecord(ev[s][1], st));
      launch_fast(Q, nf, st);
      HIP_TRY(hipEventRecord(ev[s][2], st));
      launch_compact(Q, nf, st);
      HIP_TRY(hipEventRecord(ev[s][3], st));
      HIP_TRY(hipGetLastError());
      HIP_TRY(hipMemcpyAsync(h_levelStart.p + (size_t)f0 * (kMaxLevels + 1), d_levelStart.p + (size_t)f0 * (kMaxLevels + 1),
                             sizeof(uint32_t) * (kMaxLevels + 1) * nf, hipMemcpyDeviceToHost, st));
      HIP_TRY(hipEventRecord(evS1[s], st));
    }
    double tHostQt = 0, tWait = 0;
    meta.assign((size_t)nframes * maxKp, Meta{});
    frameKpCount.assign(nframes, 0);
    frameKpBase.assign(nframes, 0);
    if ((int)taskOut.size() < nframes * nlevels) taskOut.resize((size_t)nframes * nlevels);
    for (int s = 0; s < nsub; s++) {
      hipStream_t st = streams[s];
      const int f0 = subF0[s], nf = subF0[s + 1] - f0;
      double ta = now_ms();
      HIP_TRY(hipEventSynchronize(evS1[s]));
      uint32_t need = 0;
      for (int f = f0; f < f0 + nf; f++) need = std::max(need, h_levelStart.p[(size_t)f * (kMaxLevels + 1) + nlevels]);
      if (need > candHostCap) {
        for (int q = 0; q < nsub; q++) HIP_TRY(hipStreamSynchronize(streams[q]));
        candHostCap = (size_t)need + need / 4 + 1024;
        if ((rc = h_cand.ensure(candHostCap * (size_t)batchCap))) return rc;
      }
      for (int f = f0; f < f0 + nf; f++) {
        const size_t n = h_levelStart.p[(size_t)f * (kMaxLevels + 1) + nlevels];
        if (n)
          HIP_TRY(hipMemcpyAsync(h_cand.p + candHostCap * f, d_cand.p + (size_t)P.candCap * f, n * sizeof(uint32_t),
                                 hipMemcpyDeviceToHost, st));
      }
      HIP_TRY(hipStreamSynchronize(st));
      double tb = now_ms();
      tWait += tb - ta;
      pool->parallelFor(nf * nlevels, [&](int task, int wid) {
        const int f = f0 + task / nlevels, l = task % nlevels;
        std::vector<Meta>& out = taskOut[(size_t)f * nlevels + l];
        out.clear();
        const uint32_t* ls = h_levelStart.p + (size_t)f * (kMaxLevels + 1);
        const int n = (int)(ls[l + 1] - ls[l]);
        if (n <= 0) return;
        Worker& w = workers[wid];
        const uint32_t* cd = h_cand.p + candHostCap * f + ls[l];
        w.qx.resize(n); w.qy.resize(n); w.qs.resize(n);
        for (int i = 0; i < n; i++) {
          const uint32_t v = cd[i];
          w.qx[i] = (int16_t)((int)(v & 0xfff) - kBorder);
          w.qy[i] = (int16_t)((int)((v >> 12) & 0xfff) - kBorder);
          w.qs[i] = (uint8_t)(v >> 24);
        }
        const LevelGeom& L = P.lv[l];
        w.qt.distribute(w.qx.data(), w.qy.data(), w.qs.data(), n, kBorder, L.w - kBorder, kBorder, L.h - kBorder,
                        nfeat[l], w.qsel);
        out.reserve(w.qsel.size());
        for (int k : w.qsel) {
          Meta m;
          m.x = (int16_t)(w.qx[k] + kBorder);
          m.y = (int16_t)(w.qy[k] + kBorder);
          m.score = w.qs[k];
          m.level = (uint8_t)l;
          out.push_back(m);
        }
      });
      const int selBase = f0 * maxKp;
      int nsel = 0;
      for (int f = f0; f < f0 + nf; f++) {
        frameKpBase[f] = selBase + nsel;
        for (int l = 0; l < nlevels; l++) {
          for (const Meta& m : taskOut[(size_t)f * nlevels + l]) {
            meta[selBase + nsel] = m;
            SelKp sk;
            sk.xy = (uint32_t)m.x | ((uint32_t)m.y << 16);
            sk.lf = (uint32_t)l | ((uint32_t)f << 8);
            h_sel.p[selBase + nsel++] = sk;
          }
        }
        frameKpCount[f] = selBase + nsel - frameKpBase[f];
      }
      subSel[s] = nsel;
      tHostQt += now_ms() - tb;
      if (nsel > 0) {
        HIP_TRY(hipMemcpyAsync(d_sel.p + selBase, h_sel.p + selBase, sizeof(SelKp) * nsel, hipMemcpyHostToDevice, st));
        HIP_TRY(hipEventRecord(ev[s][4], st));
        launch_describe(P, d_sel.p + selBase, nsel, d_angle.p + selBase, d_desc.p + (size_t)selBase * 32, st);
        HIP_TRY(hipEventRecord(ev[s][5], st));
        HIP_TRY(hipGetLastError());
        HIP_TRY(hipMemcpyAsync(h_angle.p + selBase, d_angle.p + selBase, sizeof(float) * nsel, hipMemcpyDeviceToHost, st));
        HIP_TRY(hipMemcpyAsync(h_desc.p + (size_t)selBase * 32, d_desc.p + (size_t)selBase * 32, (size_t)32 * nsel,
                               hipMemcpyDeviceToHost, st));
      }
    }
    const double t3 = now_ms();
    for (int s = 0; s < nsub; s++) HIP_TRY(hipStreamSynchronize(streams[s]));
    const double t4 = now_ms();
    for (int s = 0; s < nsub; s++) {
      float ms = 0;
      for (int i = 0; i < 3; i++)
        if (hipEventElapsedTime(&ms, ev[s][i], ev[s][i + 1]) == hipSuccess) kernMs[i] += ms;
      if (subSel[s] > 0 && hipEventElapsedTime(&ms, ev[s][4], ev[s][5]) == hipSuccess) kernMs[3] += ms;
      kernBatches++;
    }
    kernFrames += nframes;
    int status = ORBFE_OK;
    for (int f = 0; f < nframes; f++) {
      const int b = frameKpBase[f], n = frameKpCount[f];
      n_out[f] = n;
      if (n > cap) {
        set_err("frame %d produced %d keypoints, cap is %d", f, n, cap);
        status = ORBFE_ERR_OVERFLOW;
      }
      const int m = n < cap ? n : cap;
      OrbfeKeyPoint* ko = kps + (size_t)f * cap;
      for (int i = 0; i < m; i++) {
        const Meta& mt = meta[b + i];
        OrbfeKeyPoint kp;
        kp.x = (float)mt.x;
        kp.y = (float)mt.y;
        if (mt.level != 0) {
          const float scale = sf[mt.level];
          kp.x *= scale;
          kp.y *= scale;
        }
        kp.size = (float)(int)(31 * sf[mt.level]);
        kp.angle = h_angle.p[b + i];
        kp.response = (float)mt.score;
        kp.octave = mt.level;
        kp.class_id = -1;
        ko[i] = kp;
      }
      if (m > 0) memcpy(desc + (size_t)f * cap * 32, h_desc.p + (size_t)b * 32, (size_t)m * 32);
    }
    const double t5 = now_ms();
    stageMs[0] = (float)tWait;
    stageMs[1] = (float)tHostQt;
    stageMs[2] = (float)(t4 - t3);
    stageMs[3] = (float)(t5 - t4);
    stageMs[4] = (float)(t5 - t0);
    lastFrames = nframes;
    lastGpuQt = false;
    lastLocalCand = false;
    return status;
  }
};

extern "C" {

const char* orbfe_last_error(void) { return g_err.c_str(); }

}

namespace orbfe {
// ... 97 lines not shown
  char list[4096] = {0};
  const bool ok = fgets(list, sizeof list, f) != nullptr;
  fclose(f);
  if (!ok) return 0;
  cpu_set_t cur, want;
  CPU_ZERO(&want);
  if (sched_getaffinity(0, sizeof cur, &cur) != 0) return 0;
  int ncpu = 0;
  for (char* p = list; *p;) {
    char* e;
    long a = strtol(p, &e, 10);
    if (e == p) break;
    long b = a;
    if (*e == '-') { p = e + 1; b = strtol(p, &e, 10); }
    for (long c = a; c <= b && c < CPU_SETSIZE; c++)
      if (CPU_ISSET(c, &cur)) { CPU_SET(c, &want); ncpu++; }
    p = (*e == ',') ? e + 1 : e;
    if (*e != ',' ) break;
  }
  if (ncpu == 0) return 0;
  if (sched_setaffinity(0, sizeof want, &want) != 0) return 0;
  return ncpu;
}

int orbfe_debug_h2d_rate(int device_id, const void* host, size_t bytes, int reps, double* gb_per_s) {
  if (!host || !bytes || reps < 1 || !gb_per_s) { set_err("bad argument"); return ORBFE_ERR_INVALID; }
  HIP_TRY(hipSetDevice(device_id));
  void* d = nullptr;
  HIP_TRY(hipMalloc(&d, bytes));
  hipStream_t st = nullptr;
  hipEvent_t e0 = nullptr, e1 = nullptr;
  int rc = ORBFE_OK;
  float ms = 0;
  if (hipStreamCreateWithFlags(&st, hipStreamNonBlocking) != hipSuccess || hipEventCreate(&e0) != hipSuccess ||
      hipEventCreate(&e1) != hipSuccess) { set_err("stream/event creation failed"); rc = ORBFE_ERR_HIP; }
  if (rc == ORBFE_OK) {
    bool ok = hipMemcpyAsync(d, host, bytes, hipMemcpyHostToDevice, st) == hipSuccess && hipStreamSynchronize(st) == hipSuccess;
    ok = ok && hipEventRecord(e0, st) == hipSuccess;
    for (int i = 0; i < reps && ok; i++) ok = hipMemcpyAsync(d, host, bytes, hipMemcpyHostToDevice, st) == hipSuccess;
    ok = ok && hipEventRecord(e1, st) == hipSuccess && hipStreamSynchronize(st) == hipSuccess &&
         hipEventElapsedTime(&ms, e0, e1) == hipSuccess;
    if (!ok) { set_err("h2d probe failed: %s", hipGetErrorString(hipGetLastError())); rc = ORBFE_ERR_HIP; }
  }
  if (e0) (void)hipEventDestroy(e0);
  if (e1) (void)hipEventDestroy(e1);
  if (st) (void)hipStreamDestroy(st);
  (void)hipFree(d);
  if (rc == ORBFE_OK) *gb_per_s = ms > 0 ? (double)bytes * reps / (ms * 1e-3) / 1e9 : 0.0;
  return rc;
}

int orbfe_extractor_set_wait_mode(orbfe_extractor* h, int poll_us) {
  if (!h || poll_us < 0) { set_err("bad wait mode"); return ORBFE_ERR_INVALID; }
  if (h->pendingFrames) { set_err("a submitted batch has not been collected yet"); return ORBFE_ERR_INVALID; }
  h->pollWaitUs = poll_us;
  return ORBFE_OK;
}

int orbfe_extractor_set_blur_variant(orbfe_extractor* h, int variant) {
  if (!h || (variant != ORBFE_GAUSS_ED && variant != ORBFE_GAUSS_ROUNDED)) { set_err("bad blur variant"); return ORBFE_ERR_INVALID; }
  if (h->pendingFrames) { set_err("a submitted batch has not been collected yet"); return ORBFE_ERR_INVALID; }
  h->gaussVariant = variant;
  return ORBFE_OK;
}

int orbfe_extractor_set_input_format(orbfe_extractor* h, int format, int gray_variant) {
  if (!h || format < ORBFE_INPUT_GRAY8 || format > ORBFE_INPUT_BGRA8 || (gray_variant != ORBFE_GRAY_Q15 && gray_variant != ORBFE_GRAY_Q14)) {
    set_err("bad input format");
    return ORBFE_ERR_INVALID;
  }
  if (h->pendingFrames) { set_err("a submitted batch has not been collected yet"); return ORBFE_ERR_INVALID; }
  h->inFormat = format;
  h->grayVariant = gray_variant;
  h->batchCap = 0;
  return ORBFE_OK;
}

int orbfe_extractor_create(int nfeatures, float scaleFactor, int nlevels, int iniThFAST, int minThFAST, int device_id,
                           orbfe_extractor** out) {
  if (!out) { set_err("out is NULL"); return ORBFE_ERR_INVALID; }
  *out = nullptr;
  if (nfeatures <= 0 || nlevels < 1 || nlevels > kMaxLevels || !(scaleFactor > 1.0f) || iniThFAST < 1 ||
      minThFAST < 1 || iniThFAST > 255 || minThFAST > 255) {
    set_err("invalid extractor parameters (nfeatures=%d scale=%g nlevels=%d ini=%d min=%d; nlevels<=%d)", nfeatures,
            scaleFactor, nlevels, iniThFAST, minThFAST, kMaxLevels);
    return ORBFE_ERR_INVALID;
  }
  int ndev = 0;
  if (hipGetDeviceCount(&ndev) != hipSuccess || ndev <= 0 || device_id < 0 || device_id >= ndev) {
    set_err("no usable HIP device (count=%d, requested %d): this library has no CPU fallback", ndev, device_id);
    return ORBFE_ERR_NO_DEVICE;
  }
  HIP_TRY(hipSetDevice(device_id));
  orbfe_extractor* h = new orbfe_extractor();
  h->nfeatures = nfeatures;
  h->scaleFactor = scaleFactor;
  h->nlevels = nlevels;
  h->iniTh = iniThFAST;
  h->minTh = minThFAST;
  h->device = device_id;
  h->sf.resize(nlevels);
  h->sigma2.resize(nlevels);
  h->sf[0] = 1.0f;
  h->sigma2[0] = 1.0f;
  for (int i = 1; i < nlevels; i++) {
    h->sf[i] = (float)(h->sf[i - 1] * h->scaleFactor);
    h->sigma2[i] = h->sf[i] * h->sf[i];
  }
  h->isf.resize(nlevels);
  h->isigma2.resize(nlevels);
  for (int i = 0; i < nlevels; i++) {
    h->isf[i] = 1.0f / h->sf[i];
    h->isigma2[i] = 1.0f / h->sigma2[i];
  }
  h->nfeat.resize(nlevels);
  const float factor = (float)(1.0f / h->scaleFactor);
  float nDesired = nfeatures * (1 - factor) / (1 - (float)pow((double)factor, (double)nlevels));
  int sum = 0;
  for (int l = 0; l < nlevels - 1; l++) {
    h->nfeat[l] = cv_round_f(nDesired);
    sum += h->nfeat[l];
    nDesired *= factor;
  }
  h->nfeat[nlevels - 1] = nfeatures - sum > 0 ? nfeatures - sum : 0;
  {
    hipError_t e = hipStreamCreateWithFlags(&h->streams[0], hipStreamNonBlocking);
    if (e != hipSuccess) {
      set_err("hipStreamCreate failed: %s", hipGetErrorString(e));
      delete h;
      return ORBFE_ERR_HIP;
    }
  }
  h->stream = h->streams[0];
  bool evOk = hipEventCreate(&h->evFrame0) == hipSuccess &&
              hipEventCreateWithFlags(&h->evUpload, hipEventDisableTiming) == hipSuccess;
  for (auto& e : h->evS1) evOk = evOk && hipEventCreateWithFlags(&e, hipEventDisableTiming) == hipSuccess;
  for (auto& es : h->ev) for (auto& e : es) evOk = evOk && hipEventCreate(&e) == hipSuccess;
  if (!evOk) { set_err("hipEventCreate failed"); delete h; return ORBFE_ERR_HIP; }
  for (auto& e : h->evQt) evOk = evOk && hipEventCreate(&e) == hipSuccess;
  if (!evOk) { set_err("hipEventCreate failed"); delete h; return ORBFE_ERR_HIP; }
  if (const char* hv = getenv("ORBFE_HOST_QUADTREE")) h->gpuQuadtree = atoi(hv) == 0;
  if (const char* cv = getenv("ORBFE_CONE_MAX_FRAMES")) h->coneMaxFrames = atoi(cv);
  if (const char* pv = getenv("ORBFE_POLL_WAIT_US")) h->pollWaitUs = atoi(pv);
  if (const char* dw = ORBFE_EXP_ENV("ORBFE_DESCRIBE_WAVES")) h->describe4 = atoi(dw) != 1;
  if (const char* zv = getenv("ORBFE_ZERO_COPY")) { h->zeroCopyOut = atoi(zv) != 0; h->zeroCopyBatches = atoi(zv) == 2; }
  if (const char* iv = getenv("ORBFE_INGEST_KERNEL")) h->ingestKernel = atoi(iv) != 0;
  if (const char* gv = ORBFE_EXP_ENV("ORBFE_LOCAL_LISTS")) h->localLists = atoi(gv) != 0;
  if (const char* qv = getenv("ORBFE_QT_LDS_BYTES")) h->qtLdsBudget = atoi(qv);
  if (const char* qj = getenv("ORBFE_QT_JUMP")) h->qtJump = atoi(qj) != 0;
  if (const char* tb = ORBFE_EXP_ENV("ORBFE_TAIL_CONE_BASE")) h->tailBase = atoi(tb);
  if (const char* tt = ORBFE_EXP_ENV("ORBFE_TAIL_CONE_TILE")) h->tailTile = std::max(8, atoi(tt)) & ~3;
  if (const char* cv = ORBFE_EXP_ENV("ORBFE_CONE_TILE")) h->coneTile = atoi(cv) <= 0 ? 0 : std::max(8, atoi(cv));
  if (const char* pv = ORBFE_EXP_ENV("ORBFE_PROFILE_KERNELS")) h->profileKernels = atoi(pv) != 0;
  if (const char* gv = getenv("ORBFE_GAUSS_VARIANT")) h->gaussVariant = atoi(gv) == ORBFE_GAUSS_ROUNDED ? ORBFE_GAUSS_ROUNDED : ORBFE_GAUSS_ED;
  h->selPerFrame = 0;
  for (int l = 0; l < nlevels; l++) {
    h->selOff[l] = h->selPerFrame;
    h->selPerFrame += std::max(h->nfeat[l] + 4, 16);
    if (h->nfeat[l] + 4 > kQtNodeCap) h->gpuQuadtree = false;
  }
  h->selOff[nlevels] = h->selPerFrame;
  int nthreads = (int)std::thread::hardware_concurrency();
  if (nthreads > 16) nthreads = 16;
  if (const char* ev = getenv("ORBFE_HOST_THREADS")) nthreads = atoi(ev);
  if (nthreads < 1) nthreads = 1;
  h->hostThreads = nthreads;
  *out = h;
  return ORBFE_OK;
}

void orbfe_extractor_destroy(orbfe_extractor* h) { delete h; }
int orbfe_extractor_levels(const orbfe_extractor* h) { return h ? h->nlevels : 0; }
int orbfe_extractor_device(const orbfe_extractor* h) { return h ? h->device : -1; }

extern "C++" int orbfe_concurrent_streams(orbfe_extractor* const* hs, int n) {
  if (!hs || n < 1) return ORBFE_ERR_INVALID;
  HIP_TRY(hipSetDevice(hs[0]->device));
  constexpr unsigned long long kTicks = 20000;
  for (int i = 0; i < n; i++) launch_spin(100, hs[i]->streams[0]);
  for (int i = 0; i < n; i++) HIP_TRY(hipStreamSynchronize(hs[i]->streams[0]));
  auto overlap = [&](int k, bool& yes) -> int {
    double best = 1e30;
    for (int rep = 0; rep < 3 && best >= 0.2 * 1.6; rep++) {
      const double t0 = now_ms();
      for (int i = 0; i < k; i++) launch_spin(kTicks, hs[i]->streams[0]);
      HIP_TRY(hipGetLastError());
      for (int i = 0; i < k; i++) HIP_TRY(hipStreamSynchronize(hs[i]->streams[0]));
      best = std::min(best, now_ms() - t0);
    }
    yes = best < 0.2 * 1.6;
    return ORBFE_OK;
  };
  int k = 1;
  while (k < n) {
    bool yes = false;
    int rc = overlap(k + 1, yes);
    if (rc) return rc;
    for (int attempt = 0; !yes && attempt < 6; attempt++) {
      orbfe_extractor* h = hs[k];
      hipStream_t fresh = nullptr;
      HIP_TRY(hipStreamCreateWithFlags(&fresh, hipStreamNonBlocking));
      HIP_TRY(hipStreamSynchronize(h->streams[0]));
      (void)hipStreamDestroy(h->streams[0]);
      h->streams[0] = fresh;
      h->stream = fresh;
      launch_spin(100, fresh);
      HIP_TRY(hipStreamSynchronize(fresh));
      if ((rc = overlap(k + 1, yes))) return rc;
    }
    if (!yes) break;
    k++;
  }
  return k;
}
extern "C++" { namespace orbfe { int fast_stamps(unsigned long long out[8], int reset); } }
int orbfe_debug_fast_stamps(orbfe_extractor* h, unsigned long long out[8], int reset) {
  if (!h || !out) { set_err("NULL argument"); return ORBFE_ERR_INVALID; }
  HIP_TRY(hipSetDevice(h->device));
  HIP_TRY(hipDeviceSynchronize());
#ifndef ORBFE_EXPERIMENTS
  set_err("orbfe_debug_fast_stamps needs a library built with make EXPERIMENTS=1");
  return ORBFE_ERR_INVALID;
#endif
  if (orbfe::fast_stamps(out, reset)) { set_err("reading the stamp counters failed"); return ORBFE_ERR_HIP; }
  return ORBFE_OK;
}
extern "C++" { namespace orbfe { int sfi_debug_read(int* out, int capRecords, int reset); } }
int orbfe_debug_sfi_records(orbfe_extractor* h, int32_t* out, int cap_records, int* n_out, int reset) {
  if (!h || !out || !n_out || cap_records < 0) { set_err("NULL argument"); return ORBFE_ERR_INVALID; }
  HIP_TRY(hipSetDevice(h->device));
  HIP_TRY(hipDeviceSynchronize());
  const int n = orbfe::sfi_debug_read(out, cap_records, reset);
  if (n < 0) { set_err("reading the SearchForInitialization records failed"); return ORBFE_ERR_HIP; }
  *n_out = n;
  return ORBFE_OK;
}
float orbfe_extractor_scale_factor(const orbfe_extractor* h) { return h ? (float)h->scaleFactor : 0.f; }
int orbfe_extractor_scale_tables(const orbfe_extractor* h, float* a, float* b, float* c, float* d) {
  if (!h) { set_err("handle is NULL"); return ORBFE_ERR_INVALID; }
  for (int i = 0; i < h->nlevels; i++) {
    if (a) a[i] = h->sf[i];
    if (b) b[i] = h->isf[i];
    if (c) c[i] = h->sigma2[i];
    if (d) d[i] = h->isigma2[i];
  }
  return ORBFE_OK;
}
int orbfe_extractor_features_per_level(const orbfe_extractor* h, int32_t* out) {
  if (!h || !out) { set_err("NULL argument"); return ORBFE_ERR_INVALID; }
  for (int i = 0; i < h->nlevels; i++) out[i] = h->nfeat[i];
  return ORBFE_OK;
}
int orbfe_extractor_max_keypoints(const orbfe_extractor* h) {
  if (!h) return 0;
  int n = 0;
  for (int l = 0; l < h->nlevels; l++) n += std::max(h->nfeat[l] + 2, 16);
  return n;
}

int orbfe_extractor_set_vocabulary(orbfe_extractor* h, orbfe_vocabulary* v, int levelsup) {
  if (!h) { set_err("extractor is NULL"); return ORBFE_ERR_INVALID; }
  if (h->pendingFrames) { set_err("a submitted batch has not been collected yet"); return ORBFE_ERR_INVALID; }
  if (v && bow_device(v) != h->device) { set_err("vocabulary lives on device %d, extractor on %d", bow_device(v), h->device); return ORBFE_ERR_INVALID; }
  if (v && !h->gpuQuadtree) { set_err("the fused bag-of-words path needs the GPU quadtree path"); return ORBFE_ERR_INVALID; }
  h->voc = v;
  h->vocLevelsup = levelsup;
  return ORBFE_OK;
}

int orbfe_extract_bow(orbfe_extractor* h, int frame, uint32_t* bow_ids, double* bow_values, int* n_words, uint32_t* fv_nodes,
                      uint32_t* fv_offsets, uint32_t* fv_features, int* n_fv_nodes, uint32_t* word_of_feature,
                      uint32_t* node_of_feature) {
  if (!h || !bow_ids || !bow_values || !n_words || !fv_nodes || !fv_offsets || !fv_features || !n_fv_nodes) {
    set_err("bad argument");
    return ORBFE_ERR_INVALID;
  }
  if (!h->voc || frame < 0 || frame >= (int)h->bowKp.size()) {
    set_err("no bag-of-words result for frame %d (set a vocabulary before extracting)", frame);
    return ORBFE_ERR_INVALID;
  }
  const std::vector<uint2>& ln = h->bowKp[frame];
  return bow_assemble(h->voc, ln.data(), (int)ln.size(), bow_ids, bow_values, n_words, fv_nodes, fv_offsets, fv_features,
                      n_fv_nodes, word_of_feature, node_of_feature);
}

int orbfe_extract_bow_raw(orbfe_extractor* h, int frame, uint32_t* leaf_node, uint32_t* level_node, int cap, int* n_out) {
  if (!h || !leaf_node || !level_node || !n_out || cap < 0) { set_err("bad argument"); return ORBFE_ERR_INVALID; }
  if (!h->voc || frame < 0 || frame >= (int)h->bowKp.size()) {
    set_err("no bag-of-words result for frame %d (set a vocabulary before extracting)", frame);
    return ORBFE_ERR_INVALID;
  }
  const std::vector<uint2>& ln = h->bowKp[frame];
  *n_out = (int)ln.size();
  const int m = std::min(cap, (int)ln.size());
  for (int i = 0; i < m; i++) { leaf_node[i] = ln[i].x; level_node[i] = ln[i].y; }
  return ORBFE_OK;
}

int orbfe_extractor_max_keypoints_for_size(const orbfe_extractor* h, int rows, int cols) {
  if (!h || rows <= 0 || cols <= 0) return 0;
  int n = 0;
  for (int l = 0; l < h->nlevels; l++) {
    const int w = cv_round_f((float)cols * h->isf[l]), hh = cv_round_f((float)rows * h->isf[l]);
    int roots = hh > 2 * kBorder ? (int)roundf(static_cast<float>(w - 2 * kBorder) / (hh - 2 * kBorder)) : 0;
    if (roots < 0) roots = 0;
    n += std::max(h->nfeat[l] + 2, 4 * roots);
// ... 72 lines not shown
  return status;
}

int orbfe_extract_batch_submit(orbfe_extractor* h, int nframes, const uint8_t* const* gray, int in_device_memory,
                               int rows, int cols, size_t stride_bytes) {
  if (!h || !gray || nframes <= 0 || rows <= 0 || cols <= 0 || stride_bytes < (size_t)cols * h->inChannels()) {
    set_err("invalid arguments");
    return ORBFE_ERR_INVALID;
  }
  int rc;
  if (!gpu_route_ok(h, rows, cols, &rc)) {
    if (rc) return rc;
    return deferred_extract(h, nframes, gray, in_device_memory, rows, cols, stride_bytes);
  }
  if (h->deferredFrames) { set_err("a submitted batch has not been collected yet"); return ORBFE_ERR_INVALID; }
  return h->submitGpuQt(nframes, gray, in_device_memory != 0, rows, cols, stride_bytes);
}

int orbfe_extract_batch_wait(orbfe_extractor* h) {
  if (!h) { set_err("invalid arguments"); return ORBFE_ERR_INVALID; }
  if (h->deferredFrames) return ORBFE_OK;
  return h->waitOnly();
}

int orbfe_extract_batch_collect(orbfe_extractor* h, OrbfeKeyPoint* kps, uint8_t* desc, int cap, int* n_out) {
  if (!h || !kps || !desc || !n_out || cap <= 0) { set_err("invalid arguments"); return ORBFE_ERR_INVALID; }
  if (h->deferredFrames) return deferred_collect(h, kps, desc, cap, n_out, nullptr, nullptr);
  return h->waitGpuQt(kps, desc, cap, n_out);
}

int orbfe_sfi_chain_create(const orbfe_extractor* h, orbfe_sfi_chain** out) {
  if (!h || !out) { set_err("NULL argument"); return ORBFE_ERR_INVALID; }
  *out = nullptr;
  HIP_TRY(hipSetDevice(h->device));
  orbfe_sfi_chain* c = new orbfe_sfi_chain();
  c->device = h->device;
  c->n0cap = h->selOff[1] - h->selOff[0];
  int rc = ORBFE_OK;
  for (int i = 0; i < 2 && rc == ORBFE_OK; i++) {
    if ((rc = c->sel[i].ensure(c->n0cap))) break;
    if ((rc = c->angle[i].ensure(c->n0cap))) break;
    if ((rc = c->desc[i].ensure((size_t)c->n0cap * 32))) break;
    if (hipEventCreateWithFlags(&c->ready[i], hipEventDisableTiming) != hipSuccess) { set_err("hipEventCreate failed"); rc = ORBFE_ERR_HIP; }
  }
  if (rc == ORBFE_OK) rc = c->count.ensure(4);
  if (rc == ORBFE_OK) {
    const uint32_t init[4] = {0xffffffffu, 0xffffffffu, 0xffffffffu, 0xffffffffu};
    if (hipMemcpy(c->count.p, init, sizeof init, hipMemcpyHostToDevice) != hipSuccess) { set_err("hipMemcpy failed"); rc = ORBFE_ERR_HIP; }
  }
  if (rc != ORBFE_OK) { delete c; return rc; }
  *out = c;
  return ORBFE_OK;
}

void orbfe_sfi_chain_destroy(orbfe_sfi_chain* c) { delete c; }

int orbfe_sfi_chain_set_isolated(orbfe_sfi_chain* c, int isolated) {
  if (!c) { set_err("chain is NULL"); return ORBFE_ERR_INVALID; }
  if (c->isolated != (isolated != 0)) {
    c->seq = 0;
    c->hostPrevValid = false;
  }
  c->isolated = isolated != 0;
  return ORBFE_OK;
}

int orbfe_sfi_chain_restart(orbfe_sfi_chain* c) {
  if (!c) { set_err("chain is NULL"); return ORBFE_ERR_INVALID; }
  c->restart = true;
  return ORBFE_OK;
}

int orbfe_extract_batch_submit_matched(orbfe_extractor* h, orbfe_sfi_chain* chain, int nframes, const uint8_t* const* gray,
                                       int in_device_memory, int rows, int cols, size_t stride_bytes, const float bounds[4],
                                       int window_size, float nnratio, int check_orientation) {
  if (!h || !chain || !gray || !bounds || nframes <= 0 || rows <= 0 || cols <= 0 || stride_bytes < (size_t)cols * h->inChannels() || window_size <= 0) {
    set_err("invalid arguments");
    return ORBFE_ERR_INVALID;
  }
  int rc;
  if (!gpu_route_ok(h, rows, cols, &rc)) {
    if (rc) return rc;
    if ((rc = deferred_extract(h, nframes, gray, in_device_memory, rows, cols, stride_bytes))) return rc;
    if (!chain->hostMatcher && (rc = orbfe_matcher_create(h->device, &chain->hostMatcher))) { h->deferredFrames = 0; return rc; }
    const int cap = h->deferredCap;
    h->defM12.assign((size_t)nframes * cap, -1);
    h->defNm.assign(nframes, 0);
    std::vector<const OrbfeKeyPoint*> k1, k2;
    std::vector<const uint8_t*> d1, d2;
    std::vector<int> n1, n2, frameOf, nm;
    std::vector<std::vector<float>> pxy;
    std::vector<float*> prev;
    std::vector<int32_t*> m12;
    for (int f = 0; f < nframes; f++) {
      const OrbfeKeyPoint* pk;
      const uint8_t* pd;
      int pn;
      if (f == 0) {
        if (!chain->hostPrevValid || chain->isolated || chain->restart) continue;
        pk = chain->hostPrevKps.data(); pd = chain->hostPrevDesc.data(); pn = (int)chain->hostPrevKps.size();
      } else {
        pk = h->defKps.data() + (size_t)(f - 1) * cap; pd = h->defDesc.data() + (size_t)(f - 1) * cap * 32; pn = h->defN[f - 1];
      }
      pxy.emplace_back((size_t)std::max(pn, 1) * 2);
      for (int j = 0; j < pn; j++) { pxy.back()[2 * j] = pk[j].x; pxy.back()[2 * j + 1] = pk[j].y; }
      k1.push_back(pk); d1.push_back(pd); n1.push_back(pn);
      k2.push_back(h->defKps.data() + (size_t)f * cap); d2.push_back(h->defDesc.data() + (size_t)f * cap * 32); n2.push_back(h->defN[f]);
      m12.push_back(h->defM12.data() + (size_t)f * cap);
      frameOf.push_back(f);
    }
    for (auto& v : pxy) prev.push_back(v.data());
    nm.assign(k1.size(), 0);
    if (!k1.empty()) {
      rc = orbfe_search_for_initialization_batch(chain->hostMatcher, (int)k1.size(), k1.data(), d1.data(), n1.data(), k2.data(), d2.data(),
                                                 n2.data(), bounds, prev.data(), m12.data(), window_size, nnratio, check_orientation,
                                                 nm.data());
      if (rc) { h->deferredFrames = 0; return rc; }
      for (size_t p = 0; p < frameOf.size(); p++) h->defNm[frameOf[p]] = nm[p];
    }
    const int last = nframes - 1, ln = h->defN[last];
    chain->hostPrevKps.assign(h->defKps.begin() + (size_t)last * cap, h->defKps.begin() + (size_t)last * cap + ln);
    chain->hostPrevDesc.assign(h->defDesc.begin() + (size_t)last * cap * 32, h->defDesc.begin() + ((size_t)last * cap + ln) * 32);
    chain->hostPrevValid = !chain->isolated;
    chain->restart = false;
    h->deferredMatched = true;
    return ORBFE_OK;
  }
  if (h->deferredFrames) { set_err("a submitted batch has not been collected yet"); return ORBFE_ERR_INVALID; }
  orbfe_extractor::MatchSpec ms;
  ms.chain = chain;
  memcpy(ms.bounds, bounds, sizeof ms.bounds);
  ms.window = window_size;
  ms.nnratio = nnratio;
  ms.checkOri = check_orientation;
  return h->submitGpuQt(nframes, gray, in_device_memory != 0, rows, cols, stride_bytes, &ms);
}

int orbfe_extract_batch_collect_matched(orbfe_extractor* h, OrbfeKeyPoint* kps, uint8_t* desc, int cap, int* n_out,
                                        int32_t* matches12, int* nmatches) {
  if (!h || !kps || !desc || !n_out || !matches12 || !nmatches || cap <= 0) { set_err("invalid arguments"); return ORBFE_ERR_INVALID; }
  if (h->deferredFrames) return deferred_collect(h, kps, desc, cap, n_out, matches12, nmatches);
  return h->waitGpuQt(kps, desc, cap, n_out, matches12, nmatches);
}

int orbfe_extract(orbfe_extractor* h, const uint8_t* gray, int rows, int cols, size_t stride_bytes, OrbfeKeyPoint* kps,
                  uint8_t* desc, int cap, int* n_out) {
  if (!n_out) { set_err("n_out is NULL"); return ORBFE_ERR_INVALID; }
  *n_out = 0;
  if (!gray || rows == 0 || cols == 0) return ORBFE_OK;
  const uint8_t* frames[1] = {gray};
  return orbfe_extract_batch(h, 1, frames, 0, rows, cols, stride_bytes, kps, desc, cap, n_out);
}

int orbfe_debug_level_size(const orbfe_extractor* h, int level, int* w, int* hgt) {
  if (!h || level < 0 || level >= h->nlevels || h->rows == 0) { set_err("bad level / no frame yet"); return ORBFE_ERR_INVALID; }
  *w = h->P.lv[level].w;
  *hgt = h->P.lv[level].h;
  return ORBFE_OK;
}

int orbfe_debug_level_copy(orbfe_extractor* h, int frame, int level, uint8_t* out) {
  if (!h || level < 0 || level >= h->nlevels || frame < 0 || frame >= h->lastFrames) {
    set_err("bad frame/level");
    return ORBFE_ERR_INVALID;
  }
  HIP_TRY(hipSetDevice(h->device));
  const LevelGeom& L = h->P.lv[level];
  const uint8_t* src;
  size_t pitch;
  if (level == 0) {
    src = h->h_frame0.p[frame];
    pitch = (size_t)h->P.stride0;
  } else {
    src = h->d_slab.p + (size_t)h->P.slabBytes * frame + L.off;
    pitch = L.pitch;
  }
  HIP_TRY(hipMemcpy2D(out, L.w, src, pitch, L.w, L.h, hipMemcpyDeviceToHost));
  return ORBFE_OK;
}

int orbfe_debug_candidates(orbfe_extractor* h, int frame, int level, int32_t* xys, int cap, int* n_out) {
  if (!h || !n_out || level < 0 || level >= h->nlevels || frame < 0 || frame >= h->lastFrames) {
    set_err("bad frame/level");
    return ORBFE_ERR_INVALID;
  }
  HIP_TRY(hipSetDevice(h->device));
  uint32_t ls[kMaxLevels + 1];
  HIP_TRY(hipMemcpy(ls, h->d_levelStart.p + (size_t)frame * (kMaxLevels + 1), sizeof(ls), hipMemcpyDeviceToHost));
  const size_t start = h->lastLocalCand ? (size_t)h->P.lv[level].slotBase : (size_t)ls[level];
  const int n = h->lastLocalCand ? (int)ls[level] : (int)(ls[level + 1] - ls[level]);
  *n_out = n;
  if (n <= 0 || !xys) return ORBFE_OK;
  std::vector<uint32_t> tmp(n);
  HIP_TRY(hipMemcpy(tmp.data(), h->d_cand.p + (size_t)h->P.candCap * frame + start, sizeof(uint32_t) * n,
                    hipMemcpyDeviceToHost));
  for (int i = 0; i < n && i < cap; i++) {
    xys[3 * i] = (int)(tmp[i] & 0xfff) - kBorder;
    xys[3 * i + 1] = (int)((tmp[i] >> 12) & 0xfff) - kBorder;
    xys[3 * i + 2] = (int)(tmp[i] >> 24);
  }
  return ORBFE_OK;
}

int orbfe_debug_stage_ms(const orbfe_extractor* h, float out[5]) {
  if (!h || !out) { set_err("NULL argument"); return ORBFE_ERR_INVALID; }
  for (int i = 0; i < 5; i++) out[i] = h->stageMs[i];
  return ORBFE_OK;
}

int orbfe_debug_kernel_ms(orbfe_extractor* h, double out_ms[5], long long* batches, long long* frames, int reset) {
  if (!h) { set_err("handle is NULL"); return ORBFE_ERR_INVALID; }
  for (int i = 0; i < 5; i++) if (out_ms) out_ms[i] = h->kernMs[i];
  if (batches) *batches = h->kernBatches;
  if (frames) *frames = h->kernFrames;
  if (reset) {
    for (double& v : h->kernMs) v = 0;
    h->kernBatches = h->kernFrames = 0;
  }
  return ORBFE_OK;
}

int orbfe_debug_set_profiling(orbfe_extractor* h, int enable) {
  if (!h) { set_err("handle is NULL"); return ORBFE_ERR_INVALID; }
  h->profileKernels = enable != 0;
  return ORBFE_OK;
}

int orbfe_debug_sincos(orbfe_extractor* h, const float* angle_deg, int n, float* cos_out, float* sin_out) {
  if (!h || !angle_deg || !cos_out || !sin_out || n < 0) { set_err("bad argument"); return ORBFE_ERR_INVALID; }
  if (n == 0) return ORBFE_OK;
  HIP_TRY(hipSetDevice(h->device));
  int rc;
  if ((rc = h->d_f32tmp.ensure((size_t)3 * n))) return rc;
  float* d = h->d_f32tmp.p;
  HIP_TRY(hipMemcpyAsync(d, angle_deg, sizeof(float) * n, hipMemcpyHostToDevice, h->stream));
  launch_sincos(d, n, d + n, d + 2 * (size_t)n, h->stream);
  HIP_TRY(hipGetLastError());
  HIP_TRY(hipMemcpyAsync(cos_out, d + n, sizeof(float) * n, hipMemcpyDeviceToHost, h->stream));
  HIP_TRY(hipMemcpyAsync(sin_out, d + 2 * (size_t)n, sizeof(float) * n, hipMemcpyDeviceToHost, h->stream));
  HIP_TRY(hipStreamSynchronize(h->stream));
  return ORBFE_OK;
}

int orbfe_debug_quadtree(const int16_t* x, const int16_t* y, const uint8_t* score, int n, int min_x, int max_x,
                         int min_y, int max_y, int n_target, int32_t* out_idx, int cap, int* n_out) {
  if (!n_out || n < 0 || (n && (!x || !y || !score))) { set_err("bad argument"); return ORBFE_ERR_INVALID; }
  QuadTree qt;
  std::vector<int> sel;
  qt.distribute(x, y, score, n, min_x, max_x, min_y, max_y, n_target, sel);
  *n_out = (int)sel.size();
  for (int i = 0; i < (int)sel.size() && i < cap; i++) out_idx[i] = sel[i];
  return ORBFE_OK;
}

int orbfe_debug_sincos_host_check(uint32_t lo_bits, uint32_t hi_bits, uint32_t step, long long* mismatches) {
  if (!mismatches || step == 0) { set_err("bad argument"); return ORBFE_ERR_INVALID; }
  long long bad = 0;
  for (uint64_t u = lo_bits; u <= hi_bits; u += step) {
    const uint32_t b = (uint32_t)u;
    float f;
    memcpy(&f, &b, 4);
    volatile float vf = f;
    float s, c;
    sincosf_glibc(f, &s, &c);
    const float s0 = sinf(vf), c0 = cosf(vf);
    if (memcmp(&s, &s0, 4) || memcmp(&c, &c0, 4)) bad++;
  }
  *mismatches = bad;
  return ORBFE_OK;
}

}
```

os1_amd/csrc/orbfe_internal.h:

```cpp
#pragma once
#include <cstddef>
#include <cstdint>

namespace orbfe {

constexpr int kMaxLevels = 12;
constexpr int kEdge = 19;
constexpr int kBorder = 16;
constexpr int kHalfPatch = 15;
constexpr int kBlurRad = 18;
constexpr int kRawRad = kBlurRad + 3;

struct LevelGeom {
  int w, h;
  int pitch;
  long long off;
  int nCols, nRows;
  int wCell, hCell;
  int cellBase;
  int slotCap;
  long long slotBase;
  const int* xofs;
  const short* xalpha;
  const int* yofs;
  const short* ybeta;
  const unsigned* yofc;
  int rzPitch, rzRows;
};

struct FastCell {
  uint16_t ex0, ey0;
  uint8_t ew, pad0;
  uint8_t eh, level;
  uint32_t cell;
  uint32_t slotOff;
  uint32_t roiOff;
  uint32_t pitch;
  uint8_t wCell, hCell;
  uint16_t pad1;
  uint32_t geo;
};
static_assert(sizeof(FastCell) == 32, "one s_load_dwordx8 per FAST wave");

struct PyramidParams {
  LevelGeom lv[kMaxLevels];
  int nlevels;
  int ncells;
  long long slabBytes;
  long long slotsPerFrame;
  long long candCap;
  const uint8_t* const* frame0;
  const uint8_t* frameInline[2];
  long long stride0;
  uint8_t* slab;
  uint32_t* cellCount;
  uint32_t* slots;
  uint32_t* cand;
  uint32_t* levelStart;
  const FastCell* cells;
  const uint8_t* zeros;
  int iniTh, minTh;
  int frameBase;
  int gaussVariant;
  int fastLean;
};

struct ConeRange { int lo, hi; };
struct ConeParams {
  int base, top;
  int tile, tilesX, tilesY;
  int offB, offH, offC, coefLen;
  int ldsBytes;
  const ConeRange* regX;
  const ConeRange* regY;
};

#ifdef ORBFE_EXPERIMENTS
#define ORBFE_EXP_ENV(name) getenv(name)
#else
#define ORBFE_EXP_ENV(name) (static_cast<const char*>(nullptr))
#endif
#ifdef __HIPCC__
__device__ __forceinline__ const uint8_t* level0_of(const PyramidParams& P, int f) {
  const uint8_t* p = P.frame0 ? P.frame0[f] : P.frameInline[f & 1];
  const unsigned long long v = reinterpret_cast<unsigned long long>(p);
  const unsigned lo = __builtin_amdgcn_readfirstlane((unsigned)v), hi = __builtin_amdgcn_readfirstlane((unsigned)(v >> 32));
  return reinterpret_cast<const uint8_t*>(((unsigned long long)hi << 32) | lo);
}
#endif

struct SelKp {
  uint32_t xy;
  uint32_t lf;
};

struct ExtractView {
  const SelKp* sel;
  const float* angle;
  const uint8_t* desc;
  int selOff[kMaxLevels + 1];
  int count[kMaxLevels];
  float sf[kMaxLevels];
  int nlevels, n, device;
  void* stream;
};

struct SfiParams {
  const SelKp* sel;
  const float* angle;
  const uint8_t* desc;
  const uint32_t* selCount;
  int selPerFrame, n0cap, frameBase;
  const SelKp* carrySel;
  const float* carryAngle;
  const uint8_t* carryDesc;
  const uint32_t* carryCount;
  float minX, minY, invW, invH;
  float window, nnratio;
  int checkOri;
  uint16_t* order;
  int* orderCount;
  uint32_t* pool;
  uint32_t* pcount;
  int32_t* matches12;
  int32_t* nmatches;
};

constexpr int kQtNodeCap = 2048;

struct QtParams {
  const uint32_t* cand;
  const uint32_t* levelStart;
  long long candCap;
  int nlevels, frameBase;
  int levW[kMaxLevels], levH[kMaxLevels], nfeat[kMaxLevels];
  int selOff[kMaxLevels];
  int selPerFrame;
  uint16_t* own;
  SelKp* sel;
  uint32_t* selCount;
  SelKp* selHost;
  uint32_t* selCountHost;
  int jump;
  int levelLocal;
  long long candBase[kMaxLevels];
};


}
```

os1_amd/csrc/orbfe_kernels.hip:

```cpp
#include <mutex>
#include <hip/hip_runtime.h>

#include <type_traits>

#include "glibc_sincosf.h"
#include "orbfe_internal.h"

namespace orbfe {

__device__ __forceinline__ int m24(int a, int b) { return __mul24(a, b); }
__device__ __forceinline__ unsigned mulu24(unsigned a, unsigned b) {
  unsigned r;
  asm("v_mul_u32_u24 %0, %1, %2" : "=v"(r) : "v"(a), "v"(b));
  return r;
}

constexpr int kRzTile = 64;

__global__ __launch_bounds__(256) void k_resize(PyramidParams P, int level) {
  extern __shared__ __align__(16) uint8_t rz[];
  const LevelGeom& D = P.lv[level];
  const LevelGeom& S = P.lv[level - 1];
  const int f = P.frameBase + blockIdx.z;
  const int tx0 = blockIdx.x * kRzTile, ty0 = blockIdx.y * kRzTile;
  const int tx1 = min(tx0 + kRzTile, D.w) - 1, ty1 = min(ty0 + kRzTile, D.h) - 1;
  const uint8_t* src;
  long long sstride;
  if (level == 1) {
    src = level0_of(P, f);
    sstride = P.stride0;
  } else {
    src = P.slab + (long long)f * P.slabBytes + S.off;
    sstride = S.pitch;
  }
  const int tid = threadIdx.x;
  const int hc = tid & 63;
  const int hx = min(tx0 + hc, D.w - 1);
  const int hsx = D.xofs[hx];
  const int hal = reinterpret_cast<const int*>(D.xalpha)[hx];
  const int cx = tx0 + (tid & 15) * 4, cy = ty0 + (tid >> 4) * 4;
  int syv[4], be[4];
#pragma unroll
  for (int i = 0; i < 4; i++) {
    const int y = min(cy + i, D.h - 1);
    syv[i] = D.yofs[y];
    be[i] = reinterpret_cast<const int*>(D.ybeta)[y];
  }
  const int rx0 = D.xofs[tx0], rx1 = min(D.xofs[tx1] + 1, S.w - 1);
  const int ry0 = min(max(D.yofs[ty0], 0), S.h - 1), ry1 = min(max(D.yofs[ty1] + 1, 0), S.h - 1);
  const int rw = rx1 - rx0 + 1, rh = ry1 - ry0 + 1;
  const int LP = D.rzPitch;
  const int istr = (int)sstride;
  const uint8_t* rbase = src + (long long)ry0 * sstride + rx0;
  const int a = (int)(reinterpret_cast<uintptr_t>(rbase) & 3);
  uint16_t* H = reinterpret_cast<uint16_t*>(rz + ((m24(LP, D.rzRows) + 15) & ~15));
  if ((sstride & 3) == 0) {
    const int ndw = (a + rw + 3) >> 2;
    const int r0 = tid >> 5;
    for (int c = tid & 31; c < ndw; c += 32) {
      const uint8_t* g = rbase - a + 4 * c + m24(r0, istr);
      uint8_t* l = rz + 4 * c + m24(r0, LP);
      const int gstep = 8 * istr, lstep = 8 * LP;
      for (int r = r0; r < rh; r += 32, g += 4 * gstep, l += 4 * lstep) {
        uint32_t v[4];
#pragma unroll
        for (int u = 0; u < 4; u++) v[u] = (r + 8 * u < rh) ? *reinterpret_cast<const uint32_t*>(g + u * gstep) : 0u;
#pragma unroll
        for (int u = 0; u < 4; u++)
          if (r + 8 * u < rh) *reinterpret_cast<uint32_t*>(l + u * lstep) = v[u];
      }
    }
  } else {
    const float rcp = 1.0f / (float)rw;
    const int total = rw * rh;
    for (int i = tid; i < total; i += 256) {
      const int y = (int)(((float)i + 0.5f) * rcp), x = i - m24(y, rw);
      rz[m24(y, LP) + a + x] = rbase[m24(y, istr) + x];
    }
  }
  __syncthreads();
  {
    const int a0 = (short)hal, a1 = hal >> 16;
    const int o0 = a + hsx - rx0, o1 = a + min(hsx + 1, S.w - 1) - rx0;
    const uint8_t* p = rz + m24(tid >> 6, LP);
    uint16_t* h = H + (tid >> 6) * 64 + hc;
    for (int r = tid >> 6; r < rh; r += 4, p += 4 * LP, h += 4 * 64)
      *h = (uint16_t)((m24(p[o0], a0) + m24(p[o1], a1)) >> 4);
  }
  __syncthreads();
  if (cx > tx1 || cy > ty1) return;
  uint8_t* dst = P.slab + (long long)f * P.slabBytes + D.off;
  const uint16_t* hcol = H + (cx - tx0);
#pragma unroll
  for (int j = 0; j < 4; j++) {
    const int y = cy + j;
    if (y > ty1) break;
    const int sy = syv[j];
    const int sy0 = min(max(sy, 0), S.h - 1) - ry0, sy1 = min(max(sy + 1, 0), S.h - 1) - ry0;
    const unsigned b0 = (unsigned)(int)(short)be[j], b1 = (unsigned)(be[j] >> 16);
    const uint2 q0 = *reinterpret_cast<const uint2*>(hcol + sy0 * 64), q1 = *reinterpret_cast<const uint2*>(hcol + sy1 * 64);
    const unsigned h0[4] = {q0.x & 0xffffu, q0.x >> 16, q0.y & 0xffffu, q0.y >> 16};
    const unsigned h1[4] = {q1.x & 0xffffu, q1.x >> 16, q1.y & 0xffffu, q1.y >> 16};
    uint32_t packed = 0;
#pragma unroll
    for (int i = 0; i < 4; i++) {
      const unsigned v = ((mulu24(b0, h0[i]) >> 16) + (mulu24(b1, h1[i]) >> 16) + 2) >> 2;
      packed |= v << (8 * i);
    }
    *reinterpret_cast<uint32_t*>(dst + m24(y, D.pitch) + cx) = packed;
  }
}

__device__ __forceinline__ unsigned mulu24_w0(unsigned b, unsigned hh) {
  unsigned r;
  asm("v_mul_u32_u24_sdwa %0, %1, %2 dst_sel:DWORD dst_unused:UNUSED_PAD src0_sel:DWORD src1_sel:WORD_0" : "=v"(r) : "v"(b), "v"(hh));
  return r;
}
__device__ __forceinline__ unsigned mulu24_w1(unsigned b, unsigned hh) {
  unsigned r;
  asm("v_mul_u32_u24_sdwa %0, %1, %2 dst_sel:DWORD dst_unused:UNUSED_PAD src0_sel:DWORD src1_sel:WORD_1" : "=v"(r) : "v"(b), "v"(hh));
  return r;
}

template <int WA, int WB>
__device__ __forceinline__ unsigned mulu24_hh(unsigned a, unsigned b) {
  unsigned r;
  if (WA == 0 && WB == 0) asm("v_mul_u32_u24_sdwa %0, %1, %2 dst_sel:DWORD dst_unused:UNUSED_PAD src0_sel:WORD_0 src1_sel:WORD_0" : "=v"(r) : "v"(a), "v"(b));
  if (WA == 0 && WB == 1) asm("v_mul_u32_u24_sdwa %0, %1, %2 dst_sel:DWORD dst_unused:UNUSED_PAD src0_sel:WORD_0 src1_sel:WORD_1" : "=v"(r) : "v"(a), "v"(b));
  if (WA == 1 && WB == 0) asm("v_mul_u32_u24_sdwa %0, %1, %2 dst_sel:DWORD dst_unused:UNUSED_PAD src0_sel:WORD_1 src1_sel:WORD_0" : "=v"(r) : "v"(a), "v"(b));
  if (WA == 1 && WB == 1) asm("v_mul_u32_u24_sdwa %0, %1, %2 dst_sel:DWORD dst_unused:UNUSED_PAD src0_sel:WORD_1 src1_sel:WORD_1" : "=v"(r) : "v"(a), "v"(b));
  return r;
}

__device__ __forceinline__ int ld32(const void* base, unsigned byteOff) {
  return *reinterpret_cast<const int*>(reinterpret_cast<const char*>(base) + byteOff);
}

__device__ __forceinline__ const uint8_t* uniform_ptr(const uint8_t* p) {
  const uintptr_t v = reinterpret_cast<uintptr_t>(p);
  const unsigned lo = __builtin_amdgcn_readfirstlane((unsigned)v), hi = __builtin_amdgcn_readfirstlane((unsigned)(v >> 32));
  return reinterpret_cast<const uint8_t*>(((uintptr_t)hi << 32) | lo);
}

__device__ __forceinline__ unsigned pk_round2(unsigned x, unsigned y) {
  unsigned t;
  asm("v_pk_add_u16 %0, %1, %2\n\tv_pk_add_u16 %0, %0, 2 op_sel_hi:[1,0]\n\tv_pk_lshrrev_b16 %0, 2, %0 op_sel_hi:[0,1]" : "=&v"(t) : "v"(x), "v"(y));
  return t;
}

struct ResizeLevel {
  int dw, dh, dpitch;
  int sw, sh;
  long long sstride;
  long long doff, soff;
  const int* xofs;
  const short* xalpha;
  const unsigned* yofc;
  const short* ybeta;
  const uint8_t* const* frame0;
  const uint8_t* frameInline[2];
  uint8_t* slab;
  long long slabBytes;
  int frameBase;
  int fromLevel0;
};

template <int LP, int RH>
__global__ __launch_bounds__(256) void k_resize_fixed(ResizeLevel R, int tilesX, int ntiles, unsigned rcpTilesX, int dma) {
  __shared__ __align__(16) uint8_t rz[LP * RH];
  __shared__ __align__(16) uint16_t H[RH * 64];
  struct { int w, h, pitch; const int* xofs; const short* xalpha; const unsigned* yofc; const short* ybeta; } D = {R.dw, R.dh, R.dpitch, R.xofs, R.xalpha, R.yofc, R.ybeta};
  struct { int w, h; } S = {R.sw, R.sh};
  const int f = R.frameBase + blockIdx.y;
  const int chunk = (ntiles + 7) >> 3;
  const int tileIx = (blockIdx.x & 7) * chunk + (blockIdx.x >> 3);
  if (tileIx >= ntiles) return;
  const int tyI = (int)(((unsigned long long)(unsigned)tileIx * rcpTilesX) >> 32);
  const int tx0 = (tileIx - tyI * tilesX) * kRzTile, ty0 = tyI * kRzTile;
  const int tx1 = min(tx0 + kRzTile, D.w) - 1, ty1 = min(ty0 + kRzTile, D.h) - 1;
  const int level = R.fromLevel0 ? 1 : 2;
  typedef uint32_t u32x2 __attribute__((ext_vector_type(2)));
  u32x2 fpw = {0u, 0u};
  if (R.fromLevel0) {
    if (R.frame0) {
      fpw = *reinterpret_cast<const u32x2 __attribute__((address_space(4)))*>(reinterpret_cast<uintptr_t>(R.frame0 + f));
    } else {
      const unsigned long long v = reinterpret_cast<unsigned long long>((f & 1) ? R.frameInline[1] : R.frameInline[0]);
      fpw.x = (uint32_t)v;
      fpw.y = (uint32_t)(v >> 32);
    }
  }
  const int cxa = *reinterpret_cast<const int __attribute__((address_space(4)))*>(reinterpret_cast<uintptr_t>(D.xofs + tx0));
  const int cxb = *reinterpret_cast<const int __attribute__((address_space(4)))*>(reinterpret_cast<uintptr_t>(D.xofs + tx1));
  const unsigned cya = *reinterpret_cast<const unsigned __attribute__((address_space(4)))*>(reinterpret_cast<uintptr_t>(D.yofc + ty0));
  const unsigned cyb = *reinterpret_cast<const unsigned __attribute__((address_space(4)))*>(reinterpret_cast<uintptr_t>(D.yofc + ty1));
  const int tid = threadIdx.x;
  const int hc = tid & 63;
  const int hx = min(tx0 + hc, D.w - 1);
  const int hsx = ld32(D.xofs, (unsigned)hx << 2);
  const int hal = ld32(D.xalpha, (unsigned)hx << 2);
  const int cx = tx0 + (tid & 15) * 4, cy = ty0 + (tid >> 4) * 4;
  const int4 syq = *reinterpret_cast<const int4*>(reinterpret_cast<const char*>(D.yofc) + ((unsigned)cy << 2));
  const int4 beq = *reinterpret_cast<const int4*>(reinterpret_cast<const char*>(D.ybeta) + ((unsigned)cy << 2));
  const int syv[4] = {syq.x, syq.y, syq.z, syq.w}, be[4] = {beq.x, beq.y, beq.z, beq.w};
  asm volatile("" ::"s"(cxa), "s"(cxb), "s"(cya), "s"(cyb), "s"(fpw.x), "s"(fpw.y));
  const uint8_t* src;
  const long long sstride = R.sstride;
  if (R.fromLevel0) {
    src = reinterpret_cast<const uint8_t*>(((unsigned long long)fpw.y << 32) | fpw.x);
  } else {
    src = R.slab + (long long)f * R.slabBytes + R.soff;
  }
  const int rx0 = cxa, rx1 = min(cxb + 1, S.w - 1);
  const int ry0 = (int)(cya & 0xffffu), ry1 = (int)(cyb >> 16);
  const int rw = rx1 - rx0 + 1, rh = ry1 - ry0 + 1;
  const int istr = (int)sstride;
  const uint8_t* rbase = uniform_ptr(src + (long long)ry0 * sstride + rx0);
  const int a = (int)(reinterpret_cast<uintptr_t>(rbase) & 3);
  if ((sstride & 3) == 0 && dma) {
    static_assert(LP == 96 && RH % 10 == 0, "LDS-DMA staging layout");
    const uint8_t* gb = rbase - a;
    const int lane = tid & 63, wave = __builtin_amdgcn_readfirstlane(tid >> 6);
    const int lrow = (int)(((unsigned)lane * 43u) >> 8), lcol = lane - lrow * 6;
    const bool lastSpecial = level == 1 && ry1 == S.h - 1;
    const int rhDma = lastSpecial ? rh - 1 : rh;
    const bool on = lrow < 10 && 16 * lcol < a + rw;
    const unsigned voff = (unsigned)(m24(lrow, istr) + 16 * lcol);
#pragma unroll
    for (int u = 0; u < RH / 40; u++) {
      const int r = (wave * (RH / 40) + u) * 10;
      const uint8_t* gbr = gb + (long long)r * sstride;
      unsigned vo = voff;
      asm volatile("" : "+s"(gbr), "+v"(vo));
      if (on && r + lrow < rhDma)
        __builtin_amdgcn_global_load_lds((const __attribute__((address_space(1))) void*)(gbr + vo),
                                         (__attribute__((address_space(3))) void*)(rz + r * LP), 16, 0, 0);
    }
    if (lastSpecial && tid < ((a + rw + 3) >> 2))
      *reinterpret_cast<uint32_t*>(rz + (rh - 1) * LP + 4 * tid) = (uint32_t)ld32(gb, (unsigned)(4 * tid + m24(rh - 1, istr)));
    asm volatile("s_waitcnt vmcnt(0)" ::: "memory");
  } else if ((sstride & 3) == 0) {
    static_assert(LP <= 128 && RH % 8 == 0, "staging layout");
    const int ndw = (a + rw + 3) >> 2;
    const int c = tid & 31, r0 = tid >> 5;
    if (c < ndw) {
      const uint8_t* gb = rbase - a;
      uint32_t v[RH / 8];
#pragma unroll
      for (int u = 0; u < RH / 8; u++) v[u] = (uint32_t)ld32(gb, (unsigned)(4 * c + m24(min(r0 + 8 * u, rh - 1), istr)));
      uint8_t* l = rz + 4 * c + r0 * LP;
#pragma unroll
      for (int u = 0; u < RH / 8; u++) *reinterpret_cast<uint32_t*>(l + u * 8 * LP) = v[u];
    }
  } else {
    const float rcp = 1.0f / (float)rw;
    const int total = rw * rh;
    for (int i = tid; i < total; i += 256) {
      const int y = (int)(((float)i + 0.5f) * rcp), x = i - m24(y, rw);
      rz[y * LP + a + x] = rbase[m24(y, istr) + x];
    }
  }
  __syncthreads();
  {
    const unsigned a0 = (unsigned)(int)(short)hal << 12, a1 = (unsigned)(hal >> 16) << 12;
    const int o0 = a + hsx - rx0, o1 = a + min(hsx + 1, S.w - 1) - rx0;
    const uint8_t* p0 = rz + (tid >> 6) * LP + o0;
    const uint8_t* p1 = rz + (tid >> 6) * LP + o1;
    uint16_t* h = H + (tid >> 6) * 64 + hc;
#pragma unroll
    for (int i = 0; i < RH / 4; i++)
      h[i * 4 * 64] = (uint16_t)((__umul24(p0[i * 4 * LP], a0) + __umul24(p1[i * 4 * LP], a1)) >> 16);
  }
  __syncthreads();
  if (cx > tx1 || cy > ty1) return;
  uint8_t* dst = R.slab + (long long)f * R.slabBytes + R.doff;
  unsigned doffs = (unsigned)(m24(cy, D.pitch) + cx);
  const unsigned hx2 = (unsigned)(cx - tx0) * 2u, ry0s = (unsigned)ry0 << 7;
#pragma unroll
  for (int j = 0; j < 4; j++) {
    const int y = cy + j;
    if (y > ty1) break;
    const unsigned r0 = ((unsigned)syv[j] & 0xffffu) << 7, r1 = ((unsigned)syv[j] >> 16) << 7;
    const uint8_t* hb = reinterpret_cast<const uint8_t*>(H) + hx2 - ry0s;
    const uint2 q0 = *reinterpret_cast<const uint2*>(hb + r0), q1 = *reinterpret_cast<const uint2*>(hb + r1);
    const unsigned bw = (unsigned)be[j];
    const unsigned x01 = __builtin_amdgcn_perm(mulu24_hh<0, 1>(bw, q0.x), mulu24_hh<0, 0>(bw, q0.x), 0x07060302u);
    const unsigned y01 = __builtin_amdgcn_perm(mulu24_hh<1, 1>(bw, q1.x), mulu24_hh<1, 0>(bw, q1.x), 0x07060302u);
    const unsigned x23 = __builtin_amdgcn_perm(mulu24_hh<0, 1>(bw, q0.y), mulu24_hh<0, 0>(bw, q0.y), 0x07060302u);
    const unsigned y23 = __builtin_amdgcn_perm(mulu24_hh<1, 1>(bw, q1.y), mulu24_hh<1, 0>(bw, q1.y), 0x07060302u);
    const unsigned v01 = pk_round2(x01, y01), v23 = pk_round2(x23, y23);
    *reinterpret_cast<uint32_t*>(dst + doffs) = __builtin_amdgcn_perm(v23, v01, 0x06040200u);
    doffs += (unsigned)D.pitch;
  }
}

constexpr int kConeThreads = 1024;
#ifdef ORBFE_EXPERIMENTS
__device__ unsigned long long g_coneStamps[32];
#define CONE_STAMP(i)                                                                                                              \
  do {                                                                                                                             \
    if (threadIdx.x == 0 && blockIdx.z == 0 && blockIdx.x == gridDim.x / 2 && blockIdx.y == gridDim.y / 2)                         \
      g_coneStamps[i] = __builtin_amdgcn_s_memrealtime();                                                                          \
  } while (0)
#else
#define CONE_STAMP(i) ((void)0)
#endif

__global__ __launch_bounds__(kConeThreads) void k_pyramid_cone(PyramidParams P, ConeParams C) {
  extern __shared__ __align__(16) uint8_t cone[];
  const int tid = threadIdx.x, f = P.frameBase + blockIdx.z;
  CONE_STAMP(0);
  ConeRange rx[kMaxLevels], ry[kMaxLevels];
#pragma unroll
  for (int l = 0; l < kMaxLevels; l++) {
    rx[l] = C.regX[blockIdx.x * kMaxLevels + l];
    ry[l] = C.regY[blockIdx.y * kMaxLevels + l];
  }
  uint8_t* A = cone;
  uint8_t* B = cone + C.offB;
  uint16_t* H = reinterpret_cast<uint16_t*>(cone + C.offH);
  int2* coef = reinterpret_cast<int2*>(cone + C.offC);
  ConeRange bx = rx[0], by = ry[0];
#pragma unroll
  for (int l = 1; l < kMaxLevels; l++)
    if (l == C.base) { bx = rx[l]; by = ry[l]; }
  const uint8_t* src;
  int sstride;
  if (C.base == 0) {
    src = level0_of(P, f);
    sstride = (int)P.stride0;
  } else {
    src = P.slab + (long long)f * P.slabBytes + P.lv[C.base].off;
    sstride = P.lv[C.base].pitch;
  }
  src += (long long)by.lo * sstride + bx.lo;
  const bool dwordRows = (sstride & 3) == 0;
  int padA = dwordRows ? (int)(reinterpret_cast<uintptr_t>(src) & 3) : 0;
  int pitchA = (padA + (bx.hi - bx.lo + 1) + 3) & ~3;
  {
    int cofs[kMaxLevels], cwgt[kMaxLevels];
#pragma unroll
    for (int l = 1; l < kMaxLevels; l++) {
      cofs[l] = 0; cwgt[l] = 0;
      if (l <= C.base || l > C.top) continue;
      const LevelGeom& D = P.lv[l];
      const int pad = rx[l].lo & 3;
      if (tid < 512) {
        const int c = tid - pad;
        if (c >= 0 && c <= rx[l].hi - rx[l].lo) {
          cofs[l] = D.xofs[rx[l].lo + c];
          cwgt[l] = reinterpret_cast<const int*>(D.xalpha)[rx[l].lo + c];
        }
      } else if (tid - 512 <= ry[l].hi - ry[l].lo) {
        cofs[l] = D.yofs[ry[l].lo + tid - 512];
        cwgt[l] = reinterpret_cast<const int*>(D.ybeta)[ry[l].lo + tid - 512];
      }
    }
    const int w = bx.hi - bx.lo + 1, h = by.hi - by.lo + 1;
    if (dwordRows) {
      const int ndw = pitchA >> 2;
      const int cw = ndw <= 32 ? 32 : ndw <= 64 ? 64 : 128;
      const int c = tid & (cw - 1), rstep = kConeThreads / cw;
      if (c < ndw) {
        const uint8_t* g = src - padA + 4 * c;
        for (int r = tid / cw; r < h; r += 4 * rstep) {
          uint32_t v[4];
#pragma unroll
          for (int u = 0; u < 4; u++) v[u] = r + u * rstep < h ? *reinterpret_cast<const uint32_t*>(g + m24(r + u * rstep, sstride)) : 0u;
#pragma unroll
          for (int u = 0; u < 4; u++)
            if (r + u * rstep < h) reinterpret_cast<uint32_t*>(A)[m24(r + u * rstep, ndw) + c] = v[u];
        }
      }
    } else {
      const float rcp = 1.0f / (float)w;
      const int total = m24(w, h);
      for (int i = tid; i < total; i += kConeThreads) {
        const int r = (int)(((float)i + 0.5f) * rcp), c = i - m24(r, w);
        A[m24(r, pitchA) + c] = src[m24(r, sstride) + c];
      }
    }
    int prevPad = padA;
#pragma unroll
    for (int l = 1; l < kMaxLevels; l++) {
      if (l <= C.base || l > C.top) continue;
      const LevelGeom& S = P.lv[l - 1];
      const int dw = rx[l].hi - rx[l].lo + 1, dh = ry[l].hi - ry[l].lo + 1, pad = rx[l].lo & 3, pitch = (pad + dw + 3) & ~3;
      int2* cx = coef + (l * 2) * C.coefLen;
      int2* cy = cx + C.coefLen;
      if (tid < pitch) {
        int2 v = make_int2(0, 0);
        const int c = tid - pad;
        if (c >= 0 && c < dw) {
          const int x = cofs[l];
          v.x = (x - rx[l - 1].lo + prevPad) | ((min(x + 1, S.w - 1) - rx[l - 1].lo + prevPad) << 16);
          v.y = cwgt[l];
        }
        cx[tid] = v;
      } else if (tid >= 512 && tid - 512 < dh) {
        const int y = cofs[l];
        cy[tid - 512] = make_int2((min(max(y, 0), S.h - 1) - ry[l - 1].lo) | ((min(max(y + 1, 0), S.h - 1) - ry[l - 1].lo) << 16), cwgt[l]);
      }
      prevPad = pad;
    }
  }
  __syncthreads();
  CONE_STAMP(1);
#pragma unroll
  for (int l = 1; l < kMaxLevels; l++) {
    if (l <= C.base || l > C.top) continue;
    const LevelGeom& D = P.lv[l];
    const ConeRange sy = ry[l - 1], dx = rx[l], dy = ry[l];
    const int sh = sy.hi - sy.lo + 1, dw = dx.hi - dx.lo + 1, dh = dy.hi - dy.lo + 1;
    const int pad = dx.lo & 3, pitch = (pad + dw + 3) & ~3;
    const int2* cx = coef + (l * 2) * C.coefLen;
    const int2* cy = cx + C.coefLen;
    {
      const int cw = pitch <= 32 ? 32 : pitch <= 64 ? 64 : pitch <= 128 ? 128 : pitch <= 256 ? 256 : 512;
      const int j = tid & (cw - 1), r0 = tid / cw, rstep = kConeThreads / cw;
      if (j < pitch) {
        const int2 k = cx[j];
        const int a0 = (short)k.y, a1 = k.y >> 16;
        const uint8_t* p0 = A + (k.x & 0xffff);
        const uint8_t* p1 = A + (k.x >> 16);
        uint16_t* h = H + j;
        for (int r = r0; r < sh; r += 4 * rstep) {
          int v0[4], v1[4];
#pragma unroll
          for (int u = 0; u < 4; u++) {
            const int rr = min(r + u * rstep, sh - 1);
            v0[u] = p0[m24(rr, pitchA)];
            v1[u] = p1[m24(rr, pitchA)];
          }
#pragma unroll
          for (int u = 0; u < 4; u++)
            if (r + u * rstep < sh) h[m24(r + u * rstep, pitch)] = (uint16_t)((m24(v0[u], a0) + m24(v1[u], a1)) >> 4);
        }
      }
    }
    __syncthreads();
    CONE_STAMP(16 + l);
    {
      uint8_t* dst = P.slab + (long long)f * P.slabBytes + D.off + (long long)dy.lo * D.pitch + (dx.lo - pad);
      const int ng = pitch >> 2;
      const int gw = ng <= 8 ? 8 : ng <= 16 ? 16 : ng <= 32 ? 32 : ng <= 64 ? 64 : 128;
      const int j = (tid & (gw - 1)) * 4, y0 = tid / gw, ystep = kConeThreads / gw;
// ... 560 lines not shown
        r4[2 * h + 1] = o;
      }
      const unsigned packed = __builtin_amdgcn_perm(r4[1], r4[0], 0x0c0c0602u) | __builtin_amdgcn_perm(r4[3], r4[2], 0x06020c0cu);
      *reinterpret_cast<uint32_t*>(blT + (bv[it] >> 16)) = packed;
    }
  }
  __syncthreads();

  const float factorPI = (float)(3.1415926535897932384626433832795 / 180.f);
  float a, b;
  const float rad = __builtin_bit_cast(float, __builtin_amdgcn_readfirstlane(__builtin_bit_cast(int, angle * factorPI)));
  sincosf_glibc(rad, &b, &a);
  const uint8_t* center = blT + kBlurRad * kBPT + kBlurRad;
  typedef float f32x2 __attribute__((ext_vector_type(2)));
  const f32x2 AB = {a, b}, NBA = {-b, a}, kRoundMagic = {12582912.0f, 12582912.0f};
  unsigned long long words[4] = {0ull, 0ull, 0ull, 0ull};
#pragma unroll
  for (int j = 0; j < 4; j++) {
    if (WAVES == 4 && j != wave) continue;
    const int bit = j * 64 + lane;
    const float4 p = *reinterpret_cast<const float4*>(&c_patternF.v[4 * bit]);
    const f32x2 c1 = (f32x2){p.x, p.x} * AB + (f32x2){p.y, p.y} * NBA + kRoundMagic;
    const f32x2 c2 = (f32x2){p.z, p.z} * AB + (f32x2){p.w, p.w} * NBA + kRoundMagic;
    constexpr unsigned K = 0x400000u * (unsigned)kBPT + 0x4B400000u;
    const float c1x = c1.x, c1y = c1.y, c2x = c2.x, c2y = c2.y;
    const int i1 = (int)(__umul24(__float_as_uint(c1x), (unsigned)kBPT) + __float_as_uint(c1y) - K);
    const int i2 = (int)(__umul24(__float_as_uint(c2x), (unsigned)kBPT) + __float_as_uint(c2y) - K);
    const int t0 = center[i1], t1 = center[i2];
    words[j] = __ballot(t0 < t1);
  }
  uint8_t* descOut2 = A.descOut2;
  if (WAVES == 4) {
    if (lane == 0) {
      reinterpret_cast<unsigned long long*>(descOut + (long long)k * 32)[wave] = words[wave];
      if (descOut2) reinterpret_cast<unsigned long long*>(descOut2 + (long long)k * 32)[wave] = words[wave];
    }
  } else if (lane < 4) {
    reinterpret_cast<unsigned long long*>(descOut + (long long)k * 32)[lane] = words[lane];
    if (descOut2) reinterpret_cast<unsigned long long*>(descOut2 + (long long)k * 32)[lane] = words[lane];
  }
  if (tid == 0) {
    angleOut[k] = angle;
    if (A.angleOut2) A.angleOut2[k] = angle;
  }
}

__global__ void k_sincos(const float* deg, int n, float* c, float* s) {
  const int i = blockIdx.x * blockDim.x + threadIdx.x;
  if (i >= n) return;
  const float factorPI = (float)(3.1415926535897932384626433832795 / 180.f);
  sincosf_glibc(deg[i] * factorPI, &s[i], &c[i]);
}

template <int CH>
__global__ void __launch_bounds__(256) k_to_gray(const uint8_t* const* __restrict__ raw, long long rawStride,
                                                 const uint8_t* const* __restrict__ gray, long long grayPitch, int cols,
                                                 int c0, int c1, int c2, int shift, int aligned) {
  const int x = (int)(blockIdx.x * 256 + threadIdx.x) * 4;
  if (x >= cols) return;
  const int y = blockIdx.y, f = blockIdx.z;
  const uint8_t* src = raw[f] + (long long)y * rawStride + (long long)x * CH;
  uint8_t* dst = const_cast<uint8_t*>(gray[f]) + (long long)y * grayPitch + x;
  const int rnd = 1 << (shift - 1);
  if (aligned && x + 4 <= cols) {
    uint32_t w[CH];
    if (CH == 3) {
      const uint32_t* s32 = (const uint32_t*)src;
      w[0] = s32[0]; w[1] = s32[1]; w[2] = s32[2];
    } else {
      const uint4 q = *(const uint4*)src;
      w[0] = q.x; w[1] = q.y; w[2] = q.z; w[CH - 1] = q.w;
    }
    uint32_t out = 0;
#pragma unroll
    for (int i = 0; i < 4; i++) {
      uint32_t a, b, c;
      if (CH == 3) {
        a = (w[(3 * i) >> 2] >> (((3 * i) & 3) * 8)) & 255u;
        b = (w[(3 * i + 1) >> 2] >> (((3 * i + 1) & 3) * 8)) & 255u;
        c = (w[(3 * i + 2) >> 2] >> (((3 * i + 2) & 3) * 8)) & 255u;
      } else {
        a = w[i] & 255u; b = (w[i] >> 8) & 255u; c = (w[i] >> 16) & 255u;
      }
      out |= ((uint32_t)(m24((int)a, c0) + m24((int)b, c1) + m24((int)c, c2) + rnd) >> shift) << (8 * i);
    }
    *(uint32_t*)dst = out;
  } else {
    for (int i = 0; i < 4 && x + i < cols; i++)
      dst[i] = (uint8_t)((m24(src[CH * i], c0) + m24(src[CH * i + 1], c1) + m24(src[CH * i + 2], c2) + rnd) >> shift);
  }
}

void launch_to_gray(const uint8_t* const* raw, long long rawStride, const uint8_t* const* gray, long long grayPitch, int rows,
                    int cols, int channels, const int coef[3], int shift, bool aligned, int nframes, hipStream_t st) {
  dim3 grid((cols + 1023) / 1024, rows, nframes);
  if (channels == 3)
    hipLaunchKernelGGL(k_to_gray<3>, grid, dim3(256), 0, st, raw, rawStride, gray, grayPitch, cols, coef[0], coef[1], coef[2],
                       shift, aligned ? 1 : 0);
  else
    hipLaunchKernelGGL(k_to_gray<4>, grid, dim3(256), 0, st, raw, rawStride, gray, grayPitch, cols, coef[0], coef[1], coef[2],
                       shift, aligned ? 1 : 0);
}

static int lds_dma_enabled() {
  static const int v = [] { const char* e = getenv("ORBFE_LDS_DMA"); return e ? (atoi(e) != 0 ? 1 : 0) : 1; }();
  return v;
}

template <int V, int U>
__global__ __launch_bounds__(256) void k_ingest(const uint8_t* __restrict__ src, long long sstride, uint8_t* __restrict__ dst, long long dpitch,
                                                int rowBytes, int rows) {
  typedef uint32_t u32x4 __attribute__((ext_vector_type(4)));
  typedef typename std::conditional<V == 16, u32x4, typename std::conditional<V == 4, uint32_t, uint8_t>::type>::type T;
  const int perRow = (rowBytes + V - 1) / V;
  const int total = perRow * rows;
  const float rcpRow = 1.0f / (float)perRow;
  const int i0 = blockIdx.x * 256 + threadIdx.x, step = gridDim.x * 256;
  long long so[U], dof[U];
  bool ok[U];
  T v[U];
#pragma unroll
  for (int u = 0; u < U; u++) {
    const int i = i0 + u * step;
    ok[u] = i < total;
    const int ii = ok[u] ? i : 0;
    int yy = (int)(((float)ii + 0.5f) * rcpRow);
    int xx = ii - yy * perRow;
    if (xx < 0) { yy--; xx += perRow; }
    if (xx >= perRow) { yy++; xx -= perRow; }
    so[u] = (long long)yy * sstride + (long long)V * xx;
    dof[u] = (long long)yy * dpitch + (long long)V * xx;
  }
#pragma unroll
  for (int u = 0; u < U; u++)
    if (ok[u]) v[u] = __builtin_nontemporal_load(reinterpret_cast<const T*>(src + so[u]));
#pragma unroll
  for (int u = 0; u < U; u++)
    if (ok[u]) *reinterpret_cast<T*>(dst + dof[u]) = v[u];
}

void launch_ingest(const uint8_t* src, long long sstride, uint8_t* dst, long long dpitch, int rowBytes, int rows, hipStream_t st) {
  const uintptr_t all = (uintptr_t)src | (uintptr_t)dst | (uintptr_t)sstride | (uintptr_t)dpitch | (uintptr_t)rowBytes;
  const int V = (all & 15) == 0 ? 16 : (all & 3) == 0 ? 4 : 1;
  constexpr int U = 4;
  const long long total = (long long)((rowBytes + V - 1) / V) * rows;
  const int blocks = (int)std::max<long long>(1, (total + 256 * U - 1) / (256 * U));
#define ORBFE_INGEST(VV, UU) hipLaunchKernelGGL((k_ingest<VV, UU>), dim3(blocks), dim3(256), 0, st, src, sstride, dst, dpitch, rowBytes, rows)
  if (V == 16) ORBFE_INGEST(16, 4);
  else if (V == 4) ORBFE_INGEST(4, 4);
  else ORBFE_INGEST(1, 4);
#undef ORBFE_INGEST
}

int launch_pyramid(const PyramidParams& P, int nframes, hipStream_t st, const ConeParams* cone) {
  const int last = cone ? cone->base : P.nlevels - 1;
  if (cone) {
    static std::mutex mu;
    static int attrBytes[64] = {};
    int dev = 0;
    if (hipGetDevice(&dev) != hipSuccess || dev < 0 || dev >= 64) return 1;
    std::lock_guard<std::mutex> lk(mu);
    if (cone->ldsBytes > attrBytes[dev]) {
      if (hipFuncSetAttribute(reinterpret_cast<const void*>(k_pyramid_cone), hipFuncAttributeMaxDynamicSharedMemorySize,
                              cone->ldsBytes) != hipSuccess)
        return 1;
      attrBytes[dev] = cone->ldsBytes;
    }
  }
  for (int l = 1; l <= last; l++) {
    dim3 grid((P.lv[l].w + kRzTile - 1) / kRzTile, (P.lv[l].h + kRzTile - 1) / kRzTile, nframes);
    if (P.lv[l].rzPitch <= 96 && P.lv[l].rzRows <= 80 && grid.x >= 2) {
      const int tilesX = (int)grid.x, ntiles = (int)(grid.x * grid.y);
      const unsigned rcp = (unsigned)(0x100000000ull / (unsigned)tilesX) + 1u;
      if ((unsigned long long)ntiles * tilesX < (1ull << 31)) {
        const int dma = lds_dma_enabled();
        ResizeLevel R{};
        R.dw = P.lv[l].w; R.dh = P.lv[l].h; R.dpitch = P.lv[l].pitch;
        R.sw = P.lv[l - 1].w; R.sh = P.lv[l - 1].h;
        R.sstride = l == 1 ? P.stride0 : (long long)P.lv[l - 1].pitch;
        R.doff = P.lv[l].off; R.soff = P.lv[l - 1].off;
        R.xofs = P.lv[l].xofs; R.xalpha = P.lv[l].xalpha; R.yofc = P.lv[l].yofc; R.ybeta = P.lv[l].ybeta;
        R.frame0 = P.frame0; R.frameInline[0] = P.frameInline[0]; R.frameInline[1] = P.frameInline[1];
        R.slab = P.slab; R.slabBytes = P.slabBytes; R.frameBase = P.frameBase; R.fromLevel0 = l == 1;
        hipLaunchKernelGGL((k_resize_fixed<96, 80>), dim3(8 * ((ntiles + 7) / 8), nframes), dim3(256), 0, st, R, tilesX, ntiles, rcp, dma);
        continue;
      }
    }
    hipLaunchKernelGGL(k_resize, grid, dim3(256), (((size_t)P.lv[l].rzPitch * P.lv[l].rzRows + 15) & ~(size_t)15) + (size_t)P.lv[l].rzRows * 64 * 2, st,
                       P, l);
  }
  if (cone)
    hipLaunchKernelGGL(k_pyramid_cone, dim3(cone->tilesX, cone->tilesY, nframes), dim3(kConeThreads), cone->ldsBytes, st, P, *cone);
  return 0;
}

void launch_compact(const PyramidParams& P, int nframes, hipStream_t st) {
  hipLaunchKernelGGL(k_compact, dim3((P.ncells + 63) / 64, nframes), dim3(64), 0, st, P);
}
void launch_compact_local(const PyramidParams& P, int nframes, hipStream_t st, int level0, int level1) {
  if (level1 > P.nlevels) level1 = P.nlevels;
  int maxCells = 0;
  for (int l = level0; l < level1; l++) maxCells = std::max(maxCells, P.lv[l].nCols * P.lv[l].nRows);
  if (maxCells <= 0) return;
  hipLaunchKernelGGL(k_compact_local, dim3((maxCells + 63) / 64, level1 - level0, nframes), dim3(64), 0, st, P, level0);
}

static DescribeArgs describe_args(const PyramidParams& P, const SelKp* sel, int nsel, float* angle, uint8_t* desc) {
  DescribeArgs A{};
  for (int l = 0; l < kMaxLevels; l++) {
    A.lv[l].w = P.lv[l].w; A.lv[l].h = P.lv[l].h; A.lv[l].pitch = P.lv[l].pitch; A.lv[l].off = P.lv[l].off;
  }
  A.sel = sel; A.selCount = nullptr; A.angleOut = angle; A.descOut = desc; A.angleOut2 = nullptr; A.descOut2 = nullptr;
  A.frame0 = P.frame0; A.frameInline[0] = P.frameInline[0]; A.frameInline[1] = P.frameInline[1];
  A.stride0 = P.stride0; A.slab = P.slab; A.slabBytes = P.slabBytes;
  A.nsel = nsel; A.selPerFrame = 1; A.nlevels = P.nlevels; A.frameBase = P.frameBase; A.dma = lds_dma_enabled();
  A.gauss = P.gaussVariant;
  return A;
}

void launch_describe(const PyramidParams& P, const SelKp* sel, int nsel, float* angle, uint8_t* desc,
                     hipStream_t st) {
  if (nsel <= 0) return;
  const DescribeArgs A = describe_args(P, sel, nsel, angle, desc);
  if (A.gauss == 1) hipLaunchKernelGGL((k_describe<1, 1>), dim3(8 * ((nsel + 7) / 8)), dim3(64), 0, st, A);
  else hipLaunchKernelGGL((k_describe<1, 0>), dim3(8 * ((nsel + 7) / 8)), dim3(64), 0, st, A);
}

void launch_describe_slots(const PyramidParams& P, const SelKp* sel, int nslots, float* angle, uint8_t* desc,
                           const uint32_t* selCount, int selPerFrame, const int* selOff, hipStream_t st, bool fourWaves, float* angle2,
                           uint8_t* desc2) {
  if (nslots <= 0) return;
  DescribeArgs A = describe_args(P, sel, nslots, angle, desc);
  A.angleOut2 = angle2;
  A.descOut2 = desc2;
  A.selCount = selCount;
  A.selPerFrame = selPerFrame;
  for (int l = 0; l <= P.nlevels; l++) A.selOff[l] = selOff[l];
  const dim3 grid(8 * ((nslots + 7) / 8));
  if (fourWaves) {
    if (A.gauss == 1) hipLaunchKernelGGL((k_describe<4, 1>), grid, dim3(256), 0, st, A);
    else hipLaunchKernelGGL((k_describe<4, 0>), grid, dim3(256), 0, st, A);
  } else {
    if (A.gauss == 1) hipLaunchKernelGGL((k_describe<1, 1>), grid, dim3(64), 0, st, A);
    else hipLaunchKernelGGL((k_describe<1, 0>), grid, dim3(64), 0, st, A);
  }
}

__global__ void k_spin(unsigned long long ticks, unsigned* sink) {
  const unsigned long long t0 = __builtin_amdgcn_s_memrealtime();
  unsigned n = 0;
  while (__builtin_amdgcn_s_memrealtime() - t0 < ticks) { __builtin_amdgcn_s_sleep(32); n++; }
  if (sink && n == 0xffffffffu) *sink = n;
}
void launch_spin(unsigned long long ticks, hipStream_t st) {
  hipLaunchKernelGGL(k_spin, dim3(1), dim3(64), 0, st, ticks, (unsigned*)nullptr);
}

void launch_sincos(const float* deg, int n, float* c, float* s, hipStream_t st) {
  if (n <= 0) return;
  hipLaunchKernelGGL(k_sincos, dim3((n + 255) / 256), dim3(256), 0, st, deg, n, c, s);
}

}

#ifdef ORBFE_EXPERIMENTS
extern "C" int orbfe_exp_cone_stamps(unsigned long long* out ) {
  if (hipDeviceSynchronize() != hipSuccess) return 1;
  return hipMemcpyFromSymbol(out, HIP_SYMBOL(orbfe::g_coneStamps), sizeof(unsigned long long) * 32) == hipSuccess ? 0 : 1;
}
#endif
```

Baseline: 89330.

## Fuse pairs of pyramid resize levels into one kernel with LDS-resident middle level

Adds a k_resize_fixed2 kernel that computes two consecutive pyramid levels per tile. The intermediate level is kept in LDS and also written out, then resized again to the next level. Host code precomputes per-tile footprint ranges so each tile is self-contained, and launch_pyramid uses the fused kernel for even/odd level pairs when no cone path is active. The aim is to halve resize launches and avoid re-reading the middle level from global memory, at the cost of overlapping footprint loads and more LDS per block.

```diff
diff --git a/include/orbfe.h b/include/orbfe.h
--- a/include/orbfe.h
+++ b/include/orbfe.h
@@ -89,6 +89,9 @@
 int orbfe_extract_batch_collect_matched(orbfe_extractor* h, OrbfeKeyPoint* kps, uint8_t* desc, int cap, int* n_out,
                                         int32_t* matches12, int* nmatches);
 
+int orbfe_debug_set_pyramid_pairs(orbfe_extractor* h, int enable);
+int orbfe_debug_pyramid_pair_launches(const orbfe_extractor* h);
+int orbfe_debug_pair_partition(int cols, int rows, int nlevels, float scale, int tile_h, long long out[4]);
 int orbfe_debug_level_size(const orbfe_extractor* h, int level, int* w, int* hgt);
 int orbfe_debug_level_copy(orbfe_extractor* h, int frame, int level, uint8_t* out );
 int orbfe_debug_candidates(orbfe_extractor* h, int frame, int level, int32_t* xys, int cap, int* n_out);
diff --git a/os1_amd/api.py b/os1_amd/api.py
--- a/os1_amd/api.py
+++ b/os1_amd/api.py
@@ -60,6 +60,9 @@
     L.orbfe_extract_batch_collect.argtypes = [vp, vp, vp, ci, vp]
     L.orbfe_debug_level_size.argtypes = [vp, ci, C.POINTER(ci), C.POINTER(ci)]
     L.orbfe_debug_level_copy.argtypes = [vp, ci, ci, vp]
+    L.orbfe_debug_set_pyramid_pairs.argtypes = [vp, ci]
+    L.orbfe_debug_pyramid_pair_launches.argtypes = [vp]
+    L.orbfe_debug_pair_partition.argtypes = [ci, ci, ci, cf, ci, vp]
     L.orbfe_debug_candidates.argtypes = [vp, ci, ci, vp, ci, C.POINTER(ci)]
     L.orbfe_debug_stage_ms.argtypes = [vp, vp]
     L.orbfe_debug_sincos.argtypes = [vp, vp, ci, vp, vp]
@@ -216,6 +219,12 @@
     return load_library().orbfe_device_count()
 
 
+def pair_partition(cols, rows, nlevels=8, scale=1.2, tile_h=64):
+    out = np.zeros(4, np.int64)
+    _check(load_library().orbfe_debug_pair_partition(cols, rows, nlevels, scale, tile_h, _p(out)))
+    return tuple(int(v) for v in out)
+
+
 def hamming(a, b):
     a = np.ascontiguousarray(a, np.uint8)
     b = np.ascontiguousarray(b, np.uint8)
@@ -345,6 +354,12 @@
         out = np.zeros((h.value, w.value), np.uint8)
         _check(self.L.orbfe_debug_level_copy(self.h, frame, level, _p(out)))
         return out
+
+    def set_pyramid_pairs(self, enable=True):
+        _check(self.L.orbfe_debug_set_pyramid_pairs(self.h, int(enable)))
+
+    def pyramid_pair_launches(self):
+        return int(self.L.orbfe_debug_pyramid_pair_launches(self.h))
 
     def candidates(self, level, frame=0):
         n = C.c_int(0)
diff --git a/os1_amd/csrc/orbfe_extractor.hip b/os1_amd/csrc/orbfe_extractor.hip
--- a/os1_amd/csrc/orbfe_extractor.hip
+++ b/os1_amd/csrc/orbfe_extractor.hip
@@ -20,10 +20,11 @@
 #include "glibc_sincosf.h"
 #include "host_pool.h"
 #include "orbfe_internal.h"
+#include "pyramid_pairs.h"
 #include "quadtree.h"
 
 namespace orbfe {
-int launch_pyramid(const PyramidParams& P, int nframes, hipStream_t st, const ConeParams* cone);
+int launch_pyramid(const PyramidParams& P, int nframes, hipStream_t st, const ConeParams* cone, const PairGeom* pairs, int* pairLaunches);
 void launch_ingest(const uint8_t* src, long long sstride, uint8_t* dst, long long dpitch, int rowBytes, int rows, hipStream_t st);
 void launch_to_gray(const uint8_t* const* raw, long long rawStride, const uint8_t* const* gray, long long grayPitch, int rows,
                     int cols, int channels, const int coef[3], int shift, bool aligned, int nframes, hipStream_t st);
@@ -190,6 +191,11 @@
   int tailBase = 0, tailTile = 48;
   ConeParams cone{};
   bool coneOk = false;
+  DevBuf<PairRange> d_pairTab;
+  PairGeom pairGeom[kMaxLevels] = {};
+  bool pyramidPairs = true;
+  int pairTileH = kPairTileH;
+  int lastPairLaunches = 0;
   bool qtJump = true;
   int qtLdsBudget = 120 * 1024;
   int pollWaitUs = 0;
@@ -256,7 +262,7 @@
     (void)hipSetDevice(device);
     for (auto& st : streams) if (st) (void)hipStreamSynchronize(st);
     d_bow.release(); h_bow.release();
-    d_tables.release(); d_coneTab.release(); d_coneTailTab.release(); d_slab.release(); d_in.release(); d_cellCount.release();
+    d_tables.release(); d_pairTab.release(); d_coneTab.release(); d_coneTailTab.release(); d_slab.release(); d_in.release(); d_cellCount.release();
     d_sfiOrder.release(); d_sfiOrderCount.release(); d_sfiPool.release(); d_sfiPcount.release();
     d_cells.release(); d_zeros.release(); d_slots.release(); d_cand.release(); d_frame0.release(); d_gray.release(); d_outArena.release(); h_outArena.release();
     d_f32tmp.release();
@@ -388,6 +394,29 @@
       L.rzRows = maxH;
     }
     HIP_TRY(hipMemcpyAsync(d_tables.p, tab.data(), tableBytes, hipMemcpyHostToDevice, stream));
+    std::vector<PairRange> pairTab;
+    size_t pairAt[kMaxLevels] = {};
+    for (int u = 0; u < kMaxLevels; u++) pairGeom[u] = PairGeom{};
+    for (int u = 3; u < nlevels; u += 2) {
+      std::vector<PairRange> px, py;
+      const LevelGeom &L0 = Q.lv[u - 2], &L1 = Q.lv[u - 1], &L2 = Q.lv[u];
+      if (!pair_axis_ranges(xofsH[u - 1], L0.w, L1.w, xofsH[u], L2.w, kPairTileW, px) || !pair_axis_fits(px, true, pairTileH)) continue;
+      if (!pair_axis_ranges(yofsH[u - 1], L0.h, L1.h, yofsH[u], L2.h, pairTileH, py) || !pair_axis_fits(py, false, pairTileH)) continue;
+      pairGeom[u].tilesX = (int)px.size(); pairGeom[u].tilesY = (int)py.size(); pairGeom[u].tileH = pairTileH;
+      pairAt[u] = pairTab.size() + 1;
+      pairTab.insert(pairTab.end(), px.begin(), px.end());
+      pairTab.insert(pairTab.end(), py.begin(), py.end());
+    }
+    if (!pairTab.empty()) {
+      if ((rc = d_pairTab.ensure(pairTab.size()))) return rc;
+      HIP_TRY(hipMemcpyAsync(d_pairTab.p, pairTab.data(), sizeof(PairRange) * pairTab.size(), hipMemcpyHostToDevice, stream));
+      HIP_TRY(hipStreamSynchronize(stream));
+      for (int u = 3; u < nlevels; u += 2)
+        if (pairAt[u]) {
+          pairGeom[u].rx = d_pairTab.p + (pairAt[u] - 1);
+          pairGeom[u].ry = pairGeom[u].rx + pairGeom[u].tilesX;
+        }
+    }
     auto buildCone = [&](int tile, int baseMin, ConeParams& out, DevBuf<ConeRange>& tabBuf, bool& ok) -> int {
       ok = false;
       if (!(nlevels >= 3 && scaleFactor <= 1.5f)) return ORBFE_OK;
@@ -723,7 +752,9 @@
     QP.levelLocal = localCand ? 1 : 0;
     {
       if (prof) HIP_TRY(hipEventRecord(ev[0][0], st));
-      if (launch_pyramid(P, nframes, st, coneOk && small ? &cone : (tailOk && !small ? &coneTail : nullptr))) { set_err("cannot configure the pyramid kernel"); return ORBFE_ERR_HIP; }
+      lastPairLaunches = 0;
+      if (launch_pyramid(P, nframes, st, coneOk && small ? &cone : (tailOk && !small ? &coneTail : nullptr), !small && pyramidPairs ? pairGeom : nullptr,
+                         &lastPairLaunches)) { set_err("cannot configure the pyramid kernel"); return ORBFE_ERR_HIP; }
       const bool timeFast = prof || !small;
       fastTimed = timeFast;
       if (timeFast) HIP_TRY(hipEventRecord(ev[0][1], st));
@@ -935,7 +966,9 @@
       PyramidParams Q = P;
       Q.frameBase = f0;
       HIP_TRY(hipEventRecord(ev[s][0], st));
-      if (launch_pyramid(Q, nf, st, coneOk && nf <= coneMaxFrames ? &cone : nullptr)) { set_err("cannot configure the pyramid kernel"); return ORBFE_ERR_HIP; }
+      int np = 0;
+      if (launch_pyramid(Q, nf, st, coneOk && nf <= coneMaxFrames ? &cone : nullptr, nf > coneMaxFrames && pyramidPairs ? pairGeom : nullptr, &np)) { set_err("cannot configure the pyramid kernel"); return ORBFE_ERR_HIP; }
+      lastPairLaunches = s ? std::max(lastPairLaunches, np) : np;
       HIP_TRY(hipEventRecord(ev[s][1], st));
       launch_fast(Q, nf, st);
       HIP_TRY(hipEventRecord(ev[s][2], st));
@@ -1339,6 +1372,8 @@
   if (const char* tt = ORBFE_EXP_ENV("ORBFE_TAIL_CONE_TILE")) h->tailTile = std::max(8, atoi(tt)) & ~3;
   if (const char* cv = ORBFE_EXP_ENV("ORBFE_CONE_TILE")) h->coneTile = atoi(cv) <= 0 ? 0 : std::max(8, atoi(cv));
   if (const char* pv = ORBFE_EXP_ENV("ORBFE_PROFILE_KERNELS")) h->profileKernels = atoi(pv) != 0;
+  if (const char* pp = ORBFE_EXP_ENV("ORBFE_PYRAMID_PAIRS")) h->pyramidPairs = atoi(pp) != 0;
+  if (const char* ph = ORBFE_EXP_ENV("ORBFE_PAIR_TILE_H")) h->pairTileH = atoi(ph) == 32 ? 32 : 64;
   if (const char* gv = getenv("ORBFE_GAUSS_VARIANT")) h->gaussVariant = atoi(gv) == ORBFE_GAUSS_ROUNDED ? ORBFE_GAUSS_ROUNDED : ORBFE_GAUSS_ED;
   h->selPerFrame = 0;
   for (int l = 0; l < nlevels; l++) {
@@ -1717,6 +1752,58 @@
   return orbfe_extract_batch(h, 1, frames, 0, rows, cols, stride_bytes, kps, desc, cap, n_out);
 }
 
+int orbfe_debug_set_pyramid_pairs(orbfe_extractor* h, int enable) {
+  if (!h) return ORBFE_ERR_INVALID;
+  h->pyramidPairs = enable != 0;
+  return ORBFE_OK;
+}
+int orbfe_debug_pyramid_pair_launches(const orbfe_extractor* h) { return h ? h->lastPairLaunches : 0; }
+
+int orbfe_debug_pair_partition(int cols, int rows, int nlevels, float scale, int tile_h, long long out[4]) {
+  if (cols < 1 || rows < 1 || nlevels < 1 || nlevels > kMaxLevels || !(scale > 1.f) || (tile_h != 64 && tile_h != 32) || !out) return ORBFE_ERR_INVALID;
+  out[0] = out[1] = out[2] = out[3] = 0;
+  int w[kMaxLevels], hh[kMaxLevels];
+  float sf = 1.f;
+  for (int l = 0; l < nlevels; l++) {
+    if (l) sf = sf * scale;
+    w[l] = cv_round_f((float)cols * (1.0f / sf));
+    hh[l] = cv_round_f((float)rows * (1.0f / sf));
+    if (w[l] < 1 || hh[l] < 1) return ORBFE_ERR_TOO_SMALL;
+  }
+  for (int u = 3; u < nlevels; u += 2) {
+    out[0]++;
+    bool part = true, fit = true;
+    for (int axis = 0; axis < 2; axis++) {
+      const int* n = axis ? hh : w;
+      std::vector<int> o1, o2;
+      pair_resize_ofs(n[u - 1], n[u - 2], o1);
+      pair_resize_ofs(n[u], n[u - 1], o2);
+      std::vector<PairRange> r;
+      if (!pair_axis_ranges(o1.data(), n[u - 2], n[u - 1], o2.data(), n[u], axis ? tile_h : kPairTileW, r)) { part = false; continue; }
+      std::vector<int> owners(n[u - 1], 0);
+      for (const PairRange& q : r) {
+        for (int i = q.o0; i < q.o1; i++) {
+          owners[i]++;
+          if (i < q.m0 || i > q.m1) part = false;
+        }
+        for (int i = q.m0; i <= q.m1; i++)
+          if (o1[i] < q.f0 || std::min(o1[i] + 1, n[u - 2] - 1) > q.f1) part = false;
+      }
+      for (int i = 0; i < n[u - 1]; i++)
+        if (owners[i] != 1) { part = false; out[3]++; }
+      const int tile = axis ? tile_h : kPairTileW;
+      for (int i = 0; i < n[u]; i++) {
+        const PairRange& q = r[i / tile];
+        if (o2[i] < q.m0 || std::min(o2[i] + 1, n[u - 1] - 1) > q.m1) part = false;
+      }
+      if (!pair_axis_fits(r, axis == 0, tile_h)) fit = false;
+    }
+    if (part) out[1]++;
+    if (part && fit) out[2]++;
+  }
+  return ORBFE_OK;
+}
+
 int orbfe_debug_level_size(const orbfe_extractor* h, int level, int* w, int* hgt) {
   if (!h || level < 0 || level >= h->nlevels || h->rows == 0) { set_err("bad level / no frame yet"); return ORBFE_ERR_INVALID; }
   *w = h->P.lv[level].w;
diff --git a/os1_amd/csrc/orbfe_internal.h b/os1_amd/csrc/orbfe_internal.h
--- a/os1_amd/csrc/orbfe_internal.h
+++ b/os1_amd/csrc/orbfe_internal.h
@@ -75,6 +75,25 @@
   const ConeRange* regY;
 };
 
+struct PairRange {
+  uint16_t m0, m1;
+  uint16_t f0, f1;
+  uint16_t o0, o1;
+  uint16_t pad0, pad1;
+};
+static_assert(sizeof(PairRange) == 16, "one s_load_dwordx4 per axis");
+struct PairGeom {
+  const PairRange* rx;
+  const PairRange* ry;
+  int tilesX, tilesY, tileH;
+};
+constexpr int kPairTileW = 64;
+constexpr int kPairTileH = 64;
+constexpr int kPairFootPitch = 112;
+constexpr int kPairMidPitch = 84;
+constexpr int kPairFootRows(int tileH) { return tileH == 64 ? 99 : 54; }
+constexpr int kPairMidRows(int tileH) { return tileH == 64 ? 80 : 44; }
+
 #ifdef ORBFE_EXPERIMENTS
 #define ORBFE_EXP_ENV(name) getenv(name)
 #else
diff --git a/os1_amd/csrc/orbfe_kernels.hip b/os1_amd/csrc/orbfe_kernels.hip
--- a/os1_amd/csrc/orbfe_kernels.hip
+++ b/os1_amd/csrc/orbfe_kernels.hip
@@ -146,6 +146,37 @@
   unsigned t;
   asm("v_pk_add_u16 %0, %1, %2\n\tv_pk_add_u16 %0, %0, 2 op_sel_hi:[1,0]\n\tv_pk_lshrrev_b16 %0, 2, %0 op_sel_hi:[0,1]" : "=&v"(t) : "v"(x), "v"(y));
   return t;
+}
+
+template <int LP, int HP, int N, int RSTEP>
+__device__ __forceinline__ void rz_row_pass(const uint8_t* p0, const uint8_t* p1, uint16_t* h, int hal) {
+  const unsigned a0 = (unsigned)(int)(short)hal << 12, a1 = (unsigned)(hal >> 16) << 12;
+#pragma unroll
+  for (int i = 0; i < N; i++)
+    h[i * RSTEP * HP] = (uint16_t)((__umul24(p0[i * RSTEP * LP], a0) + __umul24(p1[i * RSTEP * LP], a1)) >> 16);
+}
+
+__device__ __forceinline__ uint32_t rz_col4(const uint8_t* h0, const uint8_t* h1, unsigned bw) {
+  const uint2 q0 = *reinterpret_cast<const uint2*>(h0), q1 = *reinterpret_cast<const uint2*>(h1);
+  const unsigned x01 = __builtin_amdgcn_perm(mulu24_hh<0, 1>(bw, q0.x), mulu24_hh<0, 0>(bw, q0.x), 0x07060302u);
+  const unsigned y01 = __builtin_amdgcn_perm(mulu24_hh<1, 1>(bw, q1.x), mulu24_hh<1, 0>(bw, q1.x), 0x07060302u);
+  const unsigned x23 = __builtin_amdgcn_perm(mulu24_hh<0, 1>(bw, q0.y), mulu24_hh<0, 0>(bw, q0.y), 0x07060302u);
+  const unsigned y23 = __builtin_amdgcn_perm(mulu24_hh<1, 1>(bw, q1.y), mulu24_hh<1, 0>(bw, q1.y), 0x07060302u);
+  const unsigned v01 = pk_round2(x01, y01), v23 = pk_round2(x23, y23);
+  return __builtin_amdgcn_perm(v23, v01, 0x06040200u);
+}
+
+template <int ROWS>
+__device__ __forceinline__ void rz_col_pass(const uint8_t* hb, const int* syv, const int* be, uint8_t* dst, unsigned doffs, unsigned pitch,
+                                            int cy, int ty1) {
+#pragma unroll
+  for (int j = 0; j < ROWS; j++) {
+    const int y = cy + j;
+    if (y > ty1) break;
+    const unsigned r0 = ((unsigned)syv[j] & 0xffffu) << 7, r1 = ((unsigned)syv[j] >> 16) << 7;
+    *reinterpret_cast<uint32_t*>(dst + doffs) = rz_col4(hb + r0, hb + r1, (unsigned)be[j]);
+    doffs += pitch;
+  }
 }
 
 struct ResizeLevel {
@@ -262,36 +293,169 @@
   }
   __syncthreads();
   {
-    const unsigned a0 = (unsigned)(int)(short)hal << 12, a1 = (unsigned)(hal >> 16) << 12;
     const int o0 = a + hsx - rx0, o1 = a + min(hsx + 1, S.w - 1) - rx0;
-    const uint8_t* p0 = rz + (tid >> 6) * LP + o0;
-    const uint8_t* p1 = rz + (tid >> 6) * LP + o1;
-    uint16_t* h = H + (tid >> 6) * 64 + hc;
-#pragma unroll
-    for (int i = 0; i < RH / 4; i++)
-      h[i * 4 * 64] = (uint16_t)((__umul24(p0[i * 4 * LP], a0) + __umul24(p1[i * 4 * LP], a1)) >> 16);
+    rz_row_pass<LP, 64, RH / 4, 4>(rz + (tid >> 6) * LP + o0, rz + (tid >> 6) * LP + o1, H + (tid >> 6) * 64 + hc, hal);
   }
   __syncthreads();
   if (cx > tx1 || cy > ty1) return;
   uint8_t* dst = R.slab + (long long)f * R.slabBytes + R.doff;
-  unsigned doffs = (unsigned)(m24(cy, D.pitch) + cx);
-  const unsigned hx2 = (unsigned)(cx - tx0) * 2u, ry0s = (unsigned)ry0 << 7;
-#pragma unroll
-  for (int j = 0; j < 4; j++) {
-    const int y = cy + j;
-    if (y > ty1) break;
-    const unsigned r0 = ((unsigned)syv[j] & 0xffffu) << 7, r1 = ((unsigned)syv[j] >> 16) << 7;
-    const uint8_t* hb = reinterpret_cast<const uint8_t*>(H) + hx2 - ry0s;
-    const uint2 q0 = *reinterpret_cast<const uint2*>(hb + r0), q1 = *reinterpret_cast<const uint2*>(hb + r1);
-    const unsigned bw = (unsigned)be[j];
-    const unsigned x01 = __builtin_amdgcn_perm(mulu24_hh<0, 1>(bw, q0.x), mulu24_hh<0, 0>(bw, q0.x), 0x07060302u);
-    const unsigned y01 = __builtin_amdgcn_perm(mulu24_hh<1, 1>(bw, q1.x), mulu24_hh<1, 0>(bw, q1.x), 0x07060302u);
-    const unsigned x23 = __builtin_amdgcn_perm(mulu24_hh<0, 1>(bw, q0.y), mulu24_hh<0, 0>(bw, q0.y), 0x07060302u);
-    const unsigned y23 = __builtin_amdgcn_perm(mulu24_hh<1, 1>(bw, q1.y), mulu24_hh<1, 0>(bw, q1.y), 0x07060302u);
-    const unsigned v01 = pk_round2(x01, y01), v23 = pk_round2(x23, y23);
-    *reinterpret_cast<uint32_t*>(dst + doffs) = __builtin_amdgcn_perm(v23, v01, 0x06040200u);
-    doffs += (unsigned)D.pitch;
-  }
+  rz_col_pass<4>(reinterpret_cast<const uint8_t*>(H) + (unsigned)(cx - tx0) * 2u - ((unsigned)ry0 << 7), syv, be, dst,
+                 (unsigned)(m24(cy, D.pitch) + cx), (unsigned)D.pitch, cy, ty1);
+}
+
+struct ResizePair {
+  int w0, h0;
+  int w1, h1, pitch1;
+  int w2, h2, pitch2;
+  int sstride;
+  long long off0, off1, off2;
+  const int* xofs1; const short* xalpha1; const unsigned* yofc1; const short* ybeta1;
+  const int* xofs2; const short* xalpha2; const unsigned* yofc2; const short* ybeta2;
+  const PairRange* rx; const PairRange* ry;
+  uint8_t* slab;
+  long long slabBytes;
+  int frameBase;
+};
+
+template <int TH>
+__global__ __launch_bounds__(256) void k_resize_fixed2(ResizePair R, int tilesX, int ntiles, unsigned rcpTilesX, int dma) {
+  constexpr int LP = kPairFootPitch, MP = kPairMidPitch, RH = kPairFootRows(TH), RHM = kPairMidRows(TH);
+  constexpr int NG = RH / 9;
+  constexpr int MDW = MP / 4, MRG = 12;
+  constexpr int NI1 = (RHM + MRG - 1) / MRG;
+  constexpr int RPT = TH / 16;
+  constexpr int FB = LP * RH;
+  static_assert(LP == 112 && RH % 9 == 0 && RH % 3 == 0 && RHM % 4 == 0 && FB % 16 == 0, "staging and row-pass layout");
+  static_assert(MP * 3 <= 256 && MDW * MRG <= 256 && (MP * 2) % 8 == 0, "thread maps of the middle region");
+  static_assert(MP * RHM <= FB && RHM * 64 <= RH * MP, "the middle region reuses the footprint, H2 reuses H1");
+  static_assert(RPT == 4 || RPT == 2, "tile height");
+  __shared__ __align__(16) uint8_t lds[FB + RH * MP * 2];
+  uint8_t* const F = lds;
+  uint8_t* const M = lds;
+  uint16_t* const H1 = reinterpret_cast<uint16_t*>(lds + FB);
+  uint16_t* const H2 = H1;
+  const int f = R.frameBase + blockIdx.y;
+  const int chunk = (ntiles + 7) >> 3;
+  const int tileIx = (blockIdx.x & 7) * chunk + (blockIdx.x >> 3);
+  if (tileIx >= ntiles) return;
+  const int tyI = (int)(((unsigned long long)(unsigned)tileIx * rcpTilesX) >> 32);
+  const int txI = tileIx - tyI * tilesX;
+  const int tx0 = txI * kPairTileW, ty0 = tyI * TH;
+  const int tx1 = min(tx0 + kPairTileW, R.w2) - 1, ty1 = min(ty0 + TH, R.h2) - 1;
+  typedef uint32_t u32x4 __attribute__((ext_vector_type(4)));
+  const u32x4 qx = *reinterpret_cast<const u32x4 __attribute__((address_space(4)))*>(reinterpret_cast<uintptr_t>(R.rx + txI));
+  const u32x4 qy = *reinterpret_cast<const u32x4 __attribute__((address_space(4)))*>(reinterpret_cast<uintptr_t>(R.ry + tyI));
+  const int tid = threadIdx.x;
+  const int hc = tid & 63;
+  const int hx = min(tx0 + hc, R.w2 - 1);
+  const int hsx = ld32(R.xofs2, (unsigned)hx << 2);
+  const int hal = ld32(R.xalpha2, (unsigned)hx << 2);
+  const int cx = tx0 + (tid & 15) * 4, cy = ty0 + (tid >> 4) * RPT;
+  int syv[RPT], be[RPT];
+  if constexpr (RPT == 4) {
+    const int4 syq = *reinterpret_cast<const int4*>(reinterpret_cast<const char*>(R.yofc2) + ((unsigned)cy << 2));
+    const int4 beq = *reinterpret_cast<const int4*>(reinterpret_cast<const char*>(R.ybeta2) + ((unsigned)cy << 2));
+    syv[0] = syq.x; syv[1] = syq.y; syv[2] = syq.z; syv[3] = syq.w;
+    be[0] = beq.x; be[1] = beq.y; be[2] = beq.z; be[3] = beq.w;
+  } else {
+    const int2 syq = *reinterpret_cast<const int2*>(reinterpret_cast<const char*>(R.yofc2) + ((unsigned)cy << 2));
+    const int2 beq = *reinterpret_cast<const int2*>(reinterpret_cast<const char*>(R.ybeta2) + ((unsigned)cy << 2));
+    syv[0] = syq.x; syv[1] = syq.y;
+    be[0] = beq.x; be[1] = beq.y;
+  }
+  asm volatile("" ::"s"(qx.x), "s"(qx.y), "s"(qx.z), "s"(qy.x), "s"(qy.y), "s"(qy.z));
+  const int mx0 = (int)(qx.x & 0xffffu), mx1 = (int)(qx.x >> 16), fx0 = (int)(qx.y & 0xffffu), fx1 = (int)(qx.y >> 16);
+  const int ox1 = (int)(qx.z >> 16);
+  const int my0 = (int)(qy.x & 0xffffu), my1 = (int)(qy.x >> 16), fy0 = (int)(qy.y & 0xffffu), fy1 = (int)(qy.y >> 16);
+  const int oy1 = (int)(qy.z >> 16);
+  const int gx0 = mx0 & ~3;
+  const int fw = fx1 - fx0 + 1, fh = fy1 - fy0 + 1, mh = my1 - my0 + 1;
+  uint8_t* const frame = R.slab + (long long)f * R.slabBytes;
+  const int istr = R.sstride;
+  const uint8_t* rbase = uniform_ptr(frame + R.off0 + (long long)fy0 * istr + fx0);
+  const int a = (int)(reinterpret_cast<uintptr_t>(rbase) & 3);
+  const uint8_t* gb = rbase - a;
+  uint32_t sv[(RH + 7) / 8];
+  const int sc = tid & 31, sr0 = tid >> 5;
+  if (dma) {
+    const int lane = tid & 63, wave = __builtin_amdgcn_readfirstlane(tid >> 6);
+    const int lrow = lane / 7, lcol = lane - lrow * 7;
+    const bool on = lrow < 9 && 16 * lcol < a + fw;
+    const unsigned voff = (unsigned)(m24(lrow, istr) + 16 * lcol);
+#pragma unroll
+    for (int u = 0; u < (NG + 3) / 4; u++) {
+      const int g = wave + 4 * u;
+      const int r = g * 9;
+      const uint8_t* gbr = gb + (long long)r * istr;
+      unsigned vo = voff;
+      asm volatile("" : "+s"(gbr), "+v"(vo));
+      if (g < NG && on && r + lrow < fh)
+        __builtin_amdgcn_global_load_lds((const __attribute__((address_space(1))) void*)(gbr + vo),
+                                         (__attribute__((address_space(3))) void*)(F + r * LP), 16, 0, 0);
+    }
+  } else if (sc < ((a + fw + 3) >> 2)) {
+#pragma unroll
+    for (int u = 0; u < (RH + 7) / 8; u++) sv[u] = (uint32_t)ld32(gb, (unsigned)(4 * sc + m24(min(sr0 + 8 * u, fh - 1), istr)));
+  }
+  const int rg = (tid >= MP) + (tid >= 2 * MP), j1 = tid - rg * MP;
+  const int mx = min(max(gx0 + j1, mx0), mx1);
+  const int msx = ld32(R.xofs1, (unsigned)mx << 2);
+  const int mal = ld32(R.xalpha1, (unsigned)mx << 2);
+  const int rgp = tid / MDW, cg = tid - rgp * MDW;
+  int yc1[NI1], yb1[NI1];
+#pragma unroll
+  for (int i = 0; i < NI1; i++) {
+    const int y = min(my0 + rgp + MRG * i, my1);
+    yc1[i] = ld32(R.yofc1, (unsigned)y << 2);
+    yb1[i] = ld32(R.ybeta1, (unsigned)y << 2);
+  }
+  if (dma) {
+    asm volatile("s_waitcnt vmcnt(0)" ::: "memory");
+  } else if (sc < ((a + fw + 3) >> 2)) {
+#pragma unroll
+    for (int u = 0; u < (RH + 7) / 8; u++)
+      if (sr0 + 8 * u < RH) *reinterpret_cast<uint32_t*>(F + 4 * sc + (sr0 + 8 * u) * LP) = sv[u];
+  }
+  __syncthreads();
+  if (tid < 3 * MP) {
+    const int o0 = a + msx - fx0, o1 = a + min(msx + 1, R.w0 - 1) - fx0;
+    rz_row_pass<LP, MP, RH / 3, 3>(F + rg * LP + o0, F + rg * LP + o1, H1 + rg * MP + j1, mal);
+  }
+  __syncthreads();
+  if (tid < MDW * MRG) {
+    const uint8_t* hb = reinterpret_cast<const uint8_t*>(H1) + cg * 8 - m24(fy0, MP * 2);
+    uint8_t* d1 = frame + R.off1;
+    const int x = gx0 + 4 * cg;
+    const bool whole = x >= mx0 && x + 4 <= ox1;
+#pragma unroll
+    for (int i = 0; i < NI1; i++) {
+      const int r = rgp + MRG * i;
+      if (r >= mh) break;
+      const unsigned r0 = mulu24((unsigned)yc1[i] & 0xffffu, MP * 2), r1 = mulu24((unsigned)yc1[i] >> 16, MP * 2);
+      const uint32_t v = rz_col4(hb + r0, hb + r1, (unsigned)yb1[i]);
+      *reinterpret_cast<uint32_t*>(M + r * MP + 4 * cg) = v;
+      const int y = my0 + r;
+      if (y < oy1) {
+        const unsigned o = (unsigned)(m24(y, R.pitch1) + x);
+        if (whole) {
+          *reinterpret_cast<uint32_t*>(d1 + o) = v;
+        } else {
+#pragma unroll
+          for (int k = 0; k < 4; k++)
+            if (x + k >= mx0 && x + k < ox1) d1[o + k] = (uint8_t)(v >> (8 * k));
+        }
+      }
+    }
+  }
+  __syncthreads();
+  {
+    const int o0 = hsx - gx0, o1 = min(hsx + 1, R.w1 - 1) - gx0;
+    rz_row_pass<MP, 64, RHM / 4, 4>(M + (tid >> 6) * MP + o0, M + (tid >> 6) * MP + o1, H2 + (tid >> 6) * 64 + hc, hal);
+  }
+  __syncthreads();
+  if (cx > tx1 || cy > ty1) return;
+  rz_col_pass<RPT>(reinterpret_cast<const uint8_t*>(H2) + (unsigned)(cx - tx0) * 2u - ((unsigned)my0 << 7), syv, be, frame + R.off2,
+                   (unsigned)(m24(cy, R.pitch2) + cx), (unsigned)R.pitch2, cy, ty1);
 }
 
 constexpr int kConeThreads = 1024;
@@ -1158,7 +1322,7 @@
 #undef ORBFE_INGEST
 }
 
-int launch_pyramid(const PyramidParams& P, int nframes, hipStream_t st, const ConeParams* cone) {
+int launch_pyramid(const PyramidParams& P, int nframes, hipStream_t st, const ConeParams* cone, const PairGeom* pairs, int* pairLaunches) {
   const int last = cone ? cone->base : P.nlevels - 1;
   if (cone) {
     static std::mutex mu;
@@ -1173,7 +1337,34 @@
       attrBytes[dev] = cone->ldsBytes;
     }
   }
+  int npairs = 0;
   for (int l = 1; l <= last; l++) {
+    if (pairs && !cone && (l & 1) == 0 && l + 1 <= last && pairs[l + 1].rx) {
+      const PairGeom& G = pairs[l + 1];
+      const int ntiles = G.tilesX * G.tilesY;
+      if (G.tilesX >= 2 && (P.lv[l - 1].pitch & 3) == 0 && (unsigned long long)ntiles * G.tilesX < (1ull << 31)) {
+        const unsigned rcp = (unsigned)(0x100000000ull / (unsigned)G.tilesX) + 1u;
+        ResizePair R{};
+        R.w0 = P.lv[l - 1].w; R.h0 = P.lv[l - 1].h; R.sstride = P.lv[l - 1].pitch;
+        R.w1 = P.lv[l].w; R.h1 = P.lv[l].h; R.pitch1 = P.lv[l].pitch;
+        R.w2 = P.lv[l + 1].w; R.h2 = P.lv[l + 1].h; R.pitch2 = P.lv[l + 1].pitch;
+        R.off0 = P.lv[l - 1].off; R.off1 = P.lv[l].off; R.off2 = P.lv[l + 1].off;
+        R.xofs1 = P.lv[l].xofs; R.xalpha1 = P.lv[l].xalpha; R.yofc1 = P.lv[l].yofc; R.ybeta1 = P.lv[l].ybeta;
+        R.xofs2 = P.lv[l + 1].xofs; R.xalpha2 = P.lv[l + 1].xalpha; R.yofc2 = P.lv[l + 1].yofc; R.ybeta2 = P.lv[l + 1].ybeta;
+        R.rx = G.rx; R.ry = G.ry;
+        R.slab = P.slab; R.slabBytes = P.slabBytes; R.frameBase = P.frameBase;
+        const dim3 pgrid(8 * ((ntiles + 7) / 8), nframes);
+        const int dma = lds_dma_enabled();
+#ifdef ORBFE_EXPERIMENTS
+        if (G.tileH != kPairTileH) hipLaunchKernelGGL((k_resize_fixed2<kPairTileH == 64 ? 32 : 64>), pgrid, dim3(256), 0, st, R, G.tilesX, ntiles, rcp, dma);
+        else
+#endif
+          hipLaunchKernelGGL((k_resize_fixed2<kPairTileH>), pgrid, dim3(256), 0, st, R, G.tilesX, ntiles, rcp, dma);
+        npairs++;
+        l++;
+        continue;
+      }
+    }
     dim3 grid((P.lv[l].w + kRzTile - 1) / kRzTile, (P.lv[l].h + kRzTile - 1) / kRzTile, nframes);
     if (P.lv[l].rzPitch <= 96 && P.lv[l].rzRows <= 80 && grid.x >= 2) {
       const int tilesX = (int)grid.x, ntiles = (int)(grid.x * grid.y);
@@ -1197,6 +1388,7 @@
   }
   if (cone)
     hipLaunchKernelGGL(k_pyramid_cone, dim3(cone->tilesX, cone->tilesY, nframes), dim3(kConeThreads), cone->ldsBytes, st, P, *cone);
+  if (pairLaunches) *pairLaunches = npairs;
   return 0;
 }
 
diff --git a/os1_amd/csrc/pyramid_pairs.h b/os1_amd/csrc/pyramid_pairs.h
--- /dev/null
+++ b/os1_amd/csrc/pyramid_pairs.h
@@ -0,0 +1,61 @@
+#pragma once
+#include <algorithm>
+#include <vector>
+
+#include "orbfe_internal.h"
+
+namespace orbfe {
+
+inline bool pair_axis_ranges(const int* ofs1, int n0, int n1, const int* ofs2, int n2, int tile, std::vector<PairRange>& out) {
+  out.clear();
+  if (n0 < 1 || n1 < 1 || n2 < 1 || tile < 1 || n0 > 65535 || n1 > 65535) return false;
+  auto c1 = [&](int i) { return std::min(std::max(ofs1[i], 0), n0 - 1); };
+  auto c2 = [&](int i) { return std::min(std::max(ofs2[i], 0), n1 - 1); };
+  for (int i = 1; i < n1; i++)
+    if (c1(i) < c1(i - 1)) return false;
+  for (int i = 1; i < n2; i++)
+    if (c2(i) < c2(i - 1)) return false;
+  const int ntiles = (n2 + tile - 1) / tile;
+  for (int t = 0; t < ntiles; t++) {
+    const int d0 = t * tile, d1 = std::min(d0 + tile, n2) - 1;
+    const bool lastTile = t == ntiles - 1;
+    const int m0 = c2(d0), m1 = lastTile ? n1 - 1 : std::min(c2(d1) + 1, n1 - 1);
+    const int f0 = c1(m0), f1 = std::min(c1(m1) + 1, n0 - 1);
+    const int o1 = lastTile ? n1 : c2(d0 + tile);
+    PairRange r{};
+    r.m0 = (uint16_t)m0; r.m1 = (uint16_t)m1; r.f0 = (uint16_t)f0; r.f1 = (uint16_t)f1; r.o0 = (uint16_t)m0; r.o1 = (uint16_t)o1;
+    out.push_back(r);
+  }
+  int next = 0;
+  for (const PairRange& r : out) {
+    if (r.o0 != next || r.o1 <= r.o0) return false;
+    if (r.o0 < r.m0 || r.o1 - 1 > r.m1) return false;
+    next = r.o1;
+  }
+  return next == n1;
+}
+
+inline bool pair_axis_fits(const std::vector<PairRange>& r, bool columns, int tileH) {
+  for (const PairRange& q : r) {
+    const int mid = q.m1 - q.m0 + 1, foot = q.f1 - q.f0 + 1;
+    if (columns) {
+      if ((q.m0 & 3) + mid > kPairMidPitch || (q.f0 & 3) + foot > kPairFootPitch) return false;
+    } else {
+      if (mid > kPairMidRows(tileH) || foot > kPairFootRows(tileH)) return false;
+    }
+  }
+  return true;
+}
+
+inline void pair_resize_ofs(int dn, int sn, std::vector<int>& ofs) {
+  ofs.resize(dn);
+  const double scale = 1. / ((double)dn / sn);
+  for (int d = 0; d < dn; d++) {
+    const float f = (float)((d + 0.5) * scale - 0.5);
+    int s = (int)f;
+    if ((float)s > f) s--;
+    ofs[d] = std::min(std::max(s, 0), sn - 1);
+  }
+}
+
+}
```

Result: slower. 86440 (-3.2%).
